# twmitchel/FieldConv

Measured on AMD Instinct MI355X. Metric: FieldConv fwd+bwd Medges/s (20k verts, k=32, C=48, M=2), higher is better.
Workload: dtype f32 (complex64 in/out; contractions on f16 MFMA with every operand split into two halves, fp32 accumulate)

## Files before the change

fieldconv_amd/_env.py:

```python
import os

SWITCHES = {
    'FC_MFMA': 'f32: fp32-MFMA contractions throughout; f16: single halves (reduced precision); default: split halves',
    'FC_RING': '0: frequency-major forward kernels for every mesh size; 2: ring-major ones for every size',
    'FC_GROUP_SPLIT': '0: the backward data kernel never runs the two frequency groups of a tile as separate work items; 2 (development): wherever legal',
    'FC_RING_COMPACT': '0: no compact LDS plans (aliased partials, half-size record chunks) for the ring-major forward kernel',
    'FC_RING_HALVES': '0: no half tiles in the last round of the ring-major forward kernel',
    'FC_HALF_TILES': '0: no half tiles in the frequency-major kernels; 2: half tiles in the backward kernels too',
    'FC_BWD_STREAM': '0: the data / filter kernel pair on large meshes too, instead of the H-streaming arrangement (gather + stream + gx kernels)',
    'FC_GATHER_WPG': '16 / 4: the gather kernel of the H-streaming arrangement as one 16-wavefront workgroup per CU / as five 4-wavefront ones, whatever its registers say',
    'FC_FILTER2': '0: the LDS-staged half-precision filter-gradient kernel instead of the register-fed one',
    'FC_SPLIT_FINISH': '1: partial sums and parameter-gradient chain as two launches',
    'FC_EDGE_PARTS_MAX': 'cap (log2) on the number of workgroups that share a tile on small meshes',
    'FC_ECHO_WPV': 'wavefronts per vertex in the ECHO descriptor kernels (1, 2 or 4)',
    'FC_STAMP_KERNEL': 'data | filter | stream: which backward kernel writes in-kernel time stamps (tools/stamps.py); waits: the walk kernels sum '
                       'the cycles of their explicit vector-memory waits instead (tools/wait_cost.py)',
    'FC_DEBUG': 'forward kernels: skip phases (WRONG RESULTS; refused by bench.py)',
    'FC_DEBUG_BWD': 'backward kernels: skip phases (bit 0 walk, bit 1 gxt product, bit 2 gW product, bit 3 H stores) (WRONG RESULTS; refused by bench.py)',
    'FC_LIN_DIRECT': '0: TangentLin on small meshes through the LDS-staged kernel instead of the direct one',
    'FC_DEBUG_RG': "ECHOBlock head's grouped GEMM: 1 no products, 2 no loads, 4 no staging (WRONG RESULTS; refused by bench.py)",
    'FC_DEBUG_RP': 'finishing launch: 1 no partial loads, 2 no parameter-gradient chain (WRONG RESULTS; refused by bench.py)',
    'FIELDCONV_DEV': '1: load libfieldconv_hip_dev.so (the library switches above exist there only; one of them set without this raises)',
    'FIELDCONV_HIP_LIB': 'path of a prebuilt libfieldconv_hip.so (development variants, fieldconv_amd.build.build_variant)',
    'FIELDCONV_DENSE': '1: FCPrecomp stencils through the dense-stencil kernels',
    'FIELDCONV_NO_GEO': '1: 64-byte factored records in the forward pass instead of geometric ones',
    'FIELDCONV_TORCH_GRAPH': '1: support graph built with torch ops instead of fc_graph_build',
    'FIELDCONV_NO_EDGE_SPLIT': '1: no edge split on small meshes',
    'FIELDCONV_EAGER_STENCIL': '1: FCPrecomp returns the dense (E,R,F) tensor',
    'FIELDCONV_NO_FUSED_EPILOGUE': '1: residual add and modReLU as separate operators',
    'FIELDCONV_SEPARATE_CALLS': '1: one foreign call per kernel instead of fc_forward_params / fc_backward_all',
    'FIELDCONV_CPP_NODES': '0: the block-level autograd nodes in Python (fieldconv_amd/blocks.py) instead of the C++ ones (fc_torch_nodes.so)',
    'FIELDCONV_ECHO_TAIL': "0: ECHOBlock's dense tail as torch's own Linear / ReLU autograd nodes instead of one node; aten: one node composed "
                           "of ATen GEMMs instead of the native head (fc_echo_head_*)",
    'FIELDCONV_BLOCK_CALLS': '0: FCResNetBlock / ECHOBlock / LiftBlock composed of per-operator autograd nodes instead of the block-level entry points',
    'BENCH_BACKEND': 'gloo: several ranks share a device (test rigs); default nccl (= RCCL)',
    'BENCH_FORCE_DIST': '1: run the partitioned / data-parallel code path with one rank',
    'BENCH_FORWARD_OVERLAP': '1: interior targets under the forward halo exchange',
    'BENCH_NO_OVERLAP': '1: gradient halo exchange not overlapped with the filter-gradient kernel',
    'BENCH_GRAPH_STEP': '1: the partitioned step captured in one HIP graph',
}

TEST_SWITCHES = {
    'FC_FULL_MODES': '1: tests/test_gpu_modes.py sweeps every development switch instead of the eight kernel-family / arithmetic modes',
    'FC_FUZZ_SHAPES': 'number of shapes in the seeded sweep against the oracle (default 40)',
    'FC_FUZZ_SEED': 'seed of that sweep',
    'FC_FUZZ_WIDE': '1: the sweep also draws layers wider than 64 channels and (n_rings, band_limit) pairs outside the compiled set',
    'FC_DIST_TEST_DEVICE': 'cuda: the distributed test worker runs the HIP kernels (two gloo ranks on one GPU)',
    'FC_DIST_OVERLAP': '0: the distributed test worker without forward / backward overlap',
    'FC_DIST_PLAN_ONLY': '1: the distributed test worker checks partition and halo plan at config-4 size only',
    'FC_DIST_CONFIG4': '1: the distributed GPU test worker runs config 4\'s per-rank size (20 000 owned vertices per rank)',
}

LIBRARY_SWITCHES = ('FC_BWD_STREAM', 'FC_GATHER_WPG', 'FC_RING', 'FC_GROUP_SPLIT', 'FC_RING_COMPACT', 'FC_RING_HALVES', 'FC_HALF_TILES', 'FC_FILTER2', 'FC_SPLIT_FINISH',
                    'FC_EDGE_PARTS_MAX', 'FC_ECHO_WPV', 'FC_STAMP_KERNEL', 'FC_DEBUG', 'FC_DEBUG_BWD', 'FC_DEBUG_RP', 'FC_DEBUG_RG', 'FC_LIN_DIRECT')

PREFIXES = ('FC_', 'FIELDCONV_', 'BENCH_')
WRONG_RESULTS = ('FC_DEBUG', 'FC_DEBUG_BWD', 'FC_DEBUG_RP', 'FC_DEBUG_RG')


def active(environ=None):
    environ = os.environ if environ is None else environ
    return {k: environ[k] for k in sorted(SWITCHES) if k in environ}


def unknown(environ=None):
    environ = os.environ if environ is None else environ
    return sorted(k for k in environ if k.startswith(PREFIXES) and k not in SWITCHES and k not in TEST_SWITCHES)
```

fieldconv_amd/_lib.py:

```python
import ctypes
import os

from .build import DEV_LIB_PATH, LIB_PATH

_c_int32 = ctypes.c_int32
_vp = ctypes.c_void_p
_sz = ctypes.c_size_t


class FcDims(ctypes.Structure):
    _fields_ = [('N', _c_int32), ('E', _c_int32), ('I', _c_int32), ('O', _c_int32), ('R', _c_int32), ('B', _c_int32), ('mode', _c_int32)]

    def __init__(self, N=0, E=0, I=0, O=0, R=0, B=0, mode=None):
        super().__init__(N, E, I, O, R, B, current_mode() if mode is None else mode)


class FcCsr(ctypes.Structure):
    _fields_ = [('rowptr', _vp), ('nbr', _vp), ('runs', _vp)]


class FcFilterParams(ctypes.Structure):
    _fields_ = [('zonal', ctypes.c_void_p), ('spherical', ctypes.c_void_p), ('phase', ctypes.c_void_p), ('ftype', ctypes.c_int32),
                ('g_zonal', ctypes.c_void_p), ('g_spherical', ctypes.c_void_p), ('g_phase', ctypes.c_void_p),
                ('bias_partials', ctypes.c_void_p), ('bias_nparts', ctypes.c_int32), ('g_bias', ctypes.c_void_p)]


class FcEpilogue(ctypes.Structure):
    _fields_ = [('addend', _vp), ('modrelu_bias', _vp), ('activated', _vp)]


class FcMesh(ctypes.Structure):
    _fields_ = [('N', _c_int32), ('E', _c_int32), ('R', _c_int32), ('B', _c_int32), ('kind', _c_int32),
                ('by_target', ctypes.POINTER(FcCsr)), ('by_source', ctypes.POINTER(FcCsr)), ('fwd', _vp), ('bwd', _vp), ('mode', _c_int32)]

    def __init__(self, N=0, E=0, R=0, B=0, kind=0, by_target=None, by_source=None, fwd=None, bwd=None, mode=None):
        super().__init__(N, E, R, B, kind, by_target, by_source, fwd, bwd, current_mode() if mode is None else mode)


class FcResnetBlockParams(ctypes.Structure):
    _fields_ = [('C_in', _c_int32), ('C_mid', _c_int32), ('C_out', _c_int32), ('conv1', FcFilterParams), ('conv2', FcFilterParams),
                ('bias1', _vp), ('bias2', _vp), ('res_re', _vp), ('res_im', _vp),
                ('g_bias1', _vp), ('g_bias2', _vp), ('g_res_re', _vp), ('g_res_im', _vp)]


class FcEchoBlockParams(ctypes.Structure):
    _fields_ = [('C_in', _c_int32), ('n_des', _c_int32), ('n_bins', _c_int32), ('conv', FcFilterParams), ('bias', _vp), ('g_bias', _vp)]


class FcEchoHeadParams(ctypes.Structure):
    _fields_ = [('D', _c_int32), ('H1', _c_int32), ('H2', _c_int32), ('C_in', _c_int32), ('C_out', _c_int32)] + \
               [(n, _vp) for n in ('w1', 'b1', 'w2', 'b2', 'w3', 'b3', 'wr', 'br', 'g_w1', 'g_b1', 'g_w2', 'g_b2', 'g_w3', 'g_b3', 'g_wr', 'g_br')]


class FcLiftBlockParams(ctypes.Structure):
    _fields_ = [('C_in', _c_int32), ('C_out', _c_int32), ('ftype', _c_int32), ('zonal_ang', _vp), ('zonal_mag', _vp), ('phase', _vp),
                ('bias', _vp), ('g_zonal_ang', _vp), ('g_zonal_mag', _vp), ('g_phase', _vp), ('g_bias', _vp)]


_DP = ctypes.POINTER(FcDims)
_MP = ctypes.POINTER(FcMesh)
_RBP = ctypes.POINTER(FcResnetBlockParams)
_EBP = ctypes.POINTER(FcEchoBlockParams)
_EHP = ctypes.POINTER(FcEchoHeadParams)
_LBP = ctypes.POINTER(FcLiftBlockParams)
_CP = ctypes.POINTER(FcCsr)
_EP = ctypes.POINTER(FcEpilogue)
_FP = ctypes.POINTER(FcFilterParams)

SIGNATURES = {
    'fc_abi_version': (ctypes.c_int, []),
    'fc_dev_switches': (ctypes.c_int, []),
    'fc_debug_stamp_buffer': (None, [_vp]),
    'fc_status_string': (ctypes.c_char_p, [ctypes.c_int]),
    'fc_supported': (ctypes.c_int, [_DP]),
    'fc_describe_kernels': (ctypes.c_int, [_DP, _c_int32, ctypes.c_char_p, ctypes.c_size_t]),
    'fc_shape_compiled': (ctypes.c_int, [_c_int32, _c_int32]),
    'fc_generic_gather': (ctypes.c_int, [_vp, _vp, _CP, _vp, _c_int32, _c_int32, _c_int32, _c_int32, _c_int32, _vp]),
    'fc_wide_workspace_bytes': (ctypes.c_size_t, [_DP, _c_int32, _c_int32, _c_int32]),
    'fc_forward_wide': (ctypes.c_int, [_vp, _vp, _CP, _c_int32, _vp, _vp, _vp, _vp, ctypes.c_size_t, _DP, _c_int32, _c_int32, _vp]),
    'fc_backward_wide': (ctypes.c_int, [_vp, _vp, _vp, _CP, _c_int32, _vp, _vp, _vp, _vp, _vp, ctypes.c_size_t, _DP, _c_int32, _vp]),
    'fc_cgemm_workspace_bytes': (ctypes.c_size_t, [_c_int32, _c_int32, _c_int32, _c_int32]),
    'fc_cgemm': (ctypes.c_int, [_vp, _vp, _vp, _c_int32, _c_int32, _c_int32, ctypes.c_int64, ctypes.c_int64, ctypes.c_int64, ctypes.c_int64,
                                _c_int32, ctypes.c_double, _c_int32, _vp, ctypes.c_size_t, _vp]),
    'fc_tangent_nonlin_forward_f64': (ctypes.c_int, [_vp, _vp, _vp, _c_int32, _c_int32, _vp]),
    'fc_tangent_nonlin_backward_workspace_bytes_f64': (ctypes.c_size_t, [_c_int32, _c_int32]),
    'fc_tangent_nonlin_backward_f64': (ctypes.c_int, [_vp, _vp, _vp, _vp, _vp, _vp, ctypes.c_size_t, _c_int32, _c_int32, _vp]),
    'fc_generic_scatter': (ctypes.c_int, [_vp, _vp, _vp, _CP, _vp, _c_int32, _c_int32, _c_int32, _c_int32, _c_int32, _vp]),
    'fc_packed_filter_floats_fwd': (_sz, [_DP, _c_int32]),
    'fc_packed_filter_floats_bwd': (_sz, [_DP, _c_int32]),
    'fc_pack_filter': (ctypes.c_int, [_vp, _vp, _vp, _DP, _c_int32, _vp]),
    'fc_pack_filter_params': (ctypes.c_int, [_vp, _vp, _vp, _c_int32, _vp, _vp, _DP, _c_int32, _vp]),
    'fc_filter_param_grads': (ctypes.c_int, [_vp, _vp, _vp, _vp, _c_int32, _vp, _vp, _vp, _DP, _vp]),
    'fc_forward': (ctypes.c_int, [_vp, _vp, _CP, _vp, _vp, _DP, _EP, _vp]),
    'fc_factored_record_floats': (ctypes.c_int, [_c_int32]),
    'fc_forward_workspace_bytes': (_sz, [_DP]),
    'fc_forward_factored': (ctypes.c_int, [_vp, _vp, _CP, _vp, _vp, _vp, _sz, _DP, _EP, _vp]),
    'fc_geometric_record_floats': (ctypes.c_int, []),
    'fc_forward_geometric': (ctypes.c_int, [_vp, _vp, _CP, _vp, _vp, _vp, _sz, _DP, _EP, _vp]),
    'fc_records_flags': (_c_int32, [_DP, _c_int32]),
    'fc_backward_workspace_bytes': (_sz, [_DP, _c_int32]),
    'fc_backward_data': (ctypes.c_int, [_vp, _vp, _vp, _CP, _vp, _vp, _vp, _sz, _DP, _vp]),
    'fc_backward_data_factored': (ctypes.c_int, [_vp, _vp, _vp, _CP, _vp, _vp, _vp, _sz, _DP, _c_int32, _vp]),
    'fc_backward_filter': (ctypes.c_int, [_vp, _vp, _sz, _DP, _c_int32, _vp]),
    'fc_backward_streams': (_c_int32, [_DP, _c_int32]),
    'fc_backward_gather': (ctypes.c_int, [_vp, _vp, _CP, _vp, _vp, _sz, _DP, _vp]),
    'fc_backward_stream': (ctypes.c_int, [_vp, _vp, _vp, _vp, _sz, _DP, _vp]),
    'fc_backward_finish': (ctypes.c_int, [_vp, _vp, _sz, _DP, _c_int32, _vp]),
    'fc_backward_finish_params': (ctypes.c_int, [_vp, _vp, _sz, _DP, _c_int32, _FP, _vp]),
    'fc_backward_all': (ctypes.c_int, [_vp, _vp, _vp, _CP, _c_int32, _vp, _vp, _vp, _FP, _vp, _sz, _DP, _vp]),
    'fc_forward_params': (ctypes.c_int, [_vp, _vp, _CP, _c_int32, _FP, _vp, _vp, _vp, _vp, _sz, _DP, _c_int32, _EP, _vp]),
    'fc_echo_hist_dim': (ctypes.c_int, [_c_int32]),
    'fc_echo_channel_block': (ctypes.c_int, [_c_int32]),
    'fc_echo_forward': (ctypes.c_int, [_vp, _vp, _vp, _CP, _vp, _vp, _c_int32, _c_int32, _c_int32, _c_int32, _vp]),
    'fc_echo_backward': (ctypes.c_int, [_vp, _vp, _vp, _CP, _vp, _vp, _vp, _vp, _c_int32, _c_int32, _c_int32, _c_int32, _vp]),
    'fc_adam_step': (ctypes.c_int, [_vp, _vp, _vp, _vp, _vp, _sz] + [ctypes.c_float] * 5 + [_vp]),
    'fc_precomp_workspace_bytes': (_sz, [_c_int32, _c_int32]),
    'fc_precomp_mark': (ctypes.c_int, [_vp, _vp, ctypes.c_float, _c_int32, _c_int32, _vp, _sz, _vp]),
    'fc_precomp_graph': (ctypes.c_int, [_vp] * 5 + [ctypes.c_float] + [_c_int32] * 7 + [_vp] * 16 + [_vp, _sz, _vp, _sz, _vp]),
    'fc_precomp_kept_count_ptr': (_vp, [_vp, _c_int32]),
    'fc_precomp_build': (ctypes.c_int, [_vp, _vp, _vp, _vp, _vp, ctypes.c_float, _c_int32, _c_int32, _c_int32, _c_int32, _vp, _vp, _vp, _vp, _vp, _sz, _vp]),
    'fc_graph_workspace_bytes': (_sz, [_c_int32, _c_int32, _c_int32, _c_int32, _c_int32]),
    'fc_graph_build': (ctypes.c_int, [_vp, _vp, _c_int32, _c_int32, _c_int32, _c_int32] + [_vp] * 12 + [_vp, _sz, _vp]),
    'fc_trans_field_forward': (ctypes.c_int, [_vp, _vp, _CP, _vp, _vp, _vp, _vp, _vp, _vp, _vp, _vp, _c_int32, _c_int32, _c_int32, _c_int32, _c_int32, _c_int32, _vp]),
    'fc_trans_field_backward_workspace_bytes': (_sz, [_c_int32, _c_int32, _c_int32, _c_int32]),
    'fc_trans_field_backward': (ctypes.c_int, [_vp, _CP, _vp, _vp, _vp, _vp, _vp, _vp, _vp, _vp, _vp, _vp, _vp, _vp, _vp, _sz, _c_int32, _c_int32, _c_int32, _c_int32, _c_int32, _c_int32, _c_int32, _vp]),
    'fc_tangent_lin_forward': (ctypes.c_int, [_vp, _vp, _vp, _vp, _c_int32, _c_int32, _c_int32, _vp]),
    'fc_tangent_lin_backward_workspace_bytes': (_sz, [_c_int32, _c_int32, _c_int32]),
    'fc_tangent_lin_backward': (ctypes.c_int, [_vp, _vp, _vp, _vp, _vp, _vp, _vp, _vp, _sz, _c_int32, _c_int32, _c_int32, _vp]),
    'fc_soft_abs_forward': (ctypes.c_int, [_vp, _vp, _sz, _vp]),
    'fc_soft_abs_backward': (ctypes.c_int, [_vp, _vp, _vp, _sz, _vp]),
    'fc_tangent_nonlin_forward': (ctypes.c_int, [_vp, _vp, _vp, _c_int32, _c_int32, _vp]),
    'fc_tangent_nonlin_backward_workspace_bytes': (_sz, [_c_int32, _c_int32]),
    'fc_tangent_nonlin_backward': (ctypes.c_int, [_vp, _vp, _vp, _vp, _vp, _vp, _sz, _c_int32, _c_int32, _vp]),
    'fc_tangent_nonlin_backward_groups': (_c_int32, [_c_int32]),
    'fc_tangent_nonlin_backward_partial': (ctypes.c_int, [_vp, _vp, _vp, _vp, _vp, _sz, _c_int32, _c_int32, _vp]),
    'fc_trans_field_forward_generic': (ctypes.c_int, [_vp, _vp, _CP, _vp, _vp, _vp, _vp, _vp, _vp, _vp, _vp] + [_c_int32] * 7 + [_vp]),
    'fc_trans_field_backward_generic_workspace_bytes': (_sz, [_c_int32] * 5),
    'fc_trans_field_backward_generic': (ctypes.c_int, [_vp, _CP, _vp] + [_vp] * 11 + [_vp, _sz] + [_c_int32] * 8 + [_vp]),
    'fc_echo_hist_dim_generic': (ctypes.c_int, [_c_int32]),
    'fc_echo_generic_workspace_bytes': (_sz, [_c_int32]),
    'fc_echo_forward_generic': (ctypes.c_int, [_vp, _vp, _vp, _CP, _vp, _vp, _vp, _sz] + [_c_int32] * 5 + [_vp]),
    'fc_echo_backward_generic': (ctypes.c_int, [_vp, _vp, _vp, _CP, _vp, _vp, _vp, _vp, _vp, _sz] + [_c_int32] * 5 + [_vp]),
    'fc_resnet_block_saved_bytes': (_sz, [_MP, _RBP]),
    'fc_resnet_block_workspace_bytes': (_sz, [_MP, _RBP, _c_int32]),
    'fc_resnet_block_forward': (ctypes.c_int, [_vp, _MP, _RBP, _vp, _vp, _sz, _vp, _sz, _vp]),
    'fc_resnet_block_backward': (ctypes.c_int, [_vp, _vp, _MP, _RBP, _vp, _sz, _vp, _vp, _sz, _vp]),
    'fc_echo_block_saved_bytes': (_sz, [_MP, _EBP]),
    'fc_echo_block_workspace_bytes': (_sz, [_MP, _EBP, _c_int32]),
    'fc_echo_block_forward': (ctypes.c_int, [_vp, _MP, _vp, _vp, _EBP, _vp, _vp, _sz, _vp, _sz, _vp]),
    'fc_echo_block_backward': (ctypes.c_int, [_vp, _vp, _MP, _vp, _vp, _EBP, _vp, _sz, _vp, _vp, _sz, _vp]),
    'fc_echo_head_forward_workspace_bytes': (_sz, [_c_int32, _EHP]),
    'fc_echo_head_forward': (ctypes.c_int, [_vp, _vp, _EHP, _vp, _vp, _vp, _vp, _sz, _c_int32, _vp]),
    'fc_echo_head_backward_workspace_bytes': (_sz, [_c_int32, _EHP]),
    'fc_echo_head_backward': (ctypes.c_int, [_vp, _vp, _vp, _vp, _vp, _EHP, _vp, _vp, _vp, _vp, _sz, _c_int32, _vp]),
    'fc_lift_block_saved_bytes': (_sz, [_MP, _LBP]),
    'fc_lift_block_workspace_bytes': (_sz, [_MP, _LBP, _c_int32]),
    'fc_lift_block_forward': (ctypes.c_int, [_vp, _vp, _c_int32, _MP, _vp, _LBP, _vp, _vp, _sz, _vp]),
    'fc_lift_block_backward': (ctypes.c_int, [_vp, _vp, _c_int32, _MP, _vp, _LBP, _vp, _sz, _vp, _vp, _sz, _vp]),
    'fc_fps_workspace_bytes': (_sz, [_c_int32]),
    'fc_fps': (ctypes.c_int, [_vp, _c_int32, _c_int32, _c_int32, _vp, _vp, _sz, _vp]),
    'fc_radius_workspace_bytes': (_sz, [_c_int32]),
    'fc_radius_count': (ctypes.c_int, [_vp, _c_int32, ctypes.c_float, _c_int32, _vp, _sz, _vp]),
    'fc_radius_edge_count_ptr': (_vp, [_vp, _c_int32]),
    'fc_radius_fill': (ctypes.c_int, [_vp, _c_int32, ctypes.c_float, _c_int32, ctypes.c_int64, _vp, _vp, _sz, _vp]),
    'fc_pair_sqdist': (ctypes.c_int, [_vp, _c_int32, _vp, _c_int32, _c_int32, _c_int32, _vp, ctypes.c_int64, _vp, _vp]),
    'fc_twin_loss_workspace_bytes': (_sz, [ctypes.c_int64, ctypes.c_int64]),
    'fc_twin_loss_forward': (ctypes.c_int, [_vp, _c_int32, _vp, _c_int32, _c_int32, _c_int32, _vp, ctypes.c_int64, _vp, ctypes.c_int64, _vp,
                                            ctypes.c_double, _vp, _vp, _vp, _sz, _vp]),
    'fc_twin_loss_backward': (ctypes.c_int, [_vp, _c_int32, _vp, _c_int32, _c_int32, _c_int32, _vp, ctypes.c_int64, _vp, ctypes.c_int64, _vp,
                                             ctypes.c_double] + [_vp] * 8 + [_vp]),
    'fc_twin_count_dense': (ctypes.c_int, [_vp, _c_int32, _vp, _c_int32, _c_int32, _c_int32, ctypes.POINTER(ctypes.c_double), _c_int32, _vp, _vp]),
    'fc_label_smoothing_workspace_bytes': (_sz, [ctypes.c_int64, _c_int32]),
    'fc_label_smoothing_forward': (ctypes.c_int, [_vp, _vp, _vp, ctypes.c_int64, _c_int32, _c_int32, ctypes.c_double, ctypes.c_double, _vp, _vp,
                                                  _sz, _vp]),
    'fc_label_smoothing_backward': (ctypes.c_int, [_vp, _vp, _vp, _vp, ctypes.c_int64, _c_int32, _c_int32, ctypes.c_double, ctypes.c_double,
                                                   _vp, _vp]),
    'fc_fps_batched_workspace_bytes': (_sz, [_c_int32]),
    'fc_fps_batched': (ctypes.c_int, [_vp, _vp, _c_int32, _c_int32, _vp, _vp, _vp, ctypes.c_int64, _vp, _vp, _sz, _vp]),
    'fc_radius_count_batched': (ctypes.c_int, [_vp, _vp, _c_int32, _c_int32, ctypes.c_float, _c_int32, _vp, _sz, _vp]),
    'fc_radius_fill_batched': (ctypes.c_int, [_vp, _vp, _c_int32, _c_int32, ctypes.c_float, _c_int32, ctypes.c_int64, _vp, _vp, _sz, _vp]),
    'fc_segment_pool_workspace_bytes': (_sz, [_c_int32] * 4),
    'fc_segment_pool_soft_abs_forward': (ctypes.c_int, [_vp, _vp] + [_c_int32] * 5 + [_vp, _vp, _sz, _vp]),
    'fc_segment_pool_soft_abs_backward': (ctypes.c_int, [_vp, _vp, _vp] + [_c_int32] * 5 + [_vp, _vp]),
    'fc_segment_pool_forward': (ctypes.c_int, [_vp, _vp] + [_c_int32] * 5 + [_vp, _vp, _sz, _vp]),
    'fc_segment_pool_backward': (ctypes.c_int, [_vp, _vp] + [_c_int32] * 5 + [_vp, _vp]),
    'fc_match_workspace_bytes': (_sz, [_c_int32] * 3),
    'fc_match_topk': (ctypes.c_int, [_vp, _c_int32, _vp, _c_int32, _c_int32, _c_int32, _vp, _vp, _c_int32, _vp, _c_int32, _c_int32, _vp, _vp,
                                     _vp, _sz, _vp]),
    'fc_linear_ce_workspace_bytes': (_sz, [_c_int32] * 6),
    'fc_linear_ce_forward': (ctypes.c_int, [_vp, _vp, _vp, _vp, _c_int32, _c_int32, _c_int32, ctypes.c_double, ctypes.c_double, ctypes.c_int64,
                                            _c_int32, _vp, _vp, _vp, _vp, _sz, _vp]),
    'fc_linear_topk': (ctypes.c_int, [_vp, _vp, _vp] + [_c_int32] * 5 + [_vp, _vp, _vp, _sz, _vp]),
    'fc_linear_ce_backward_input': (ctypes.c_int, [_vp] * 6 + [_c_int32] * 3 + [ctypes.c_double, ctypes.c_double, ctypes.c_int64, _vp, _vp]),
    'fc_linear_ce_backward_weight': (ctypes.c_int, [_vp] * 6 + [_c_int32] * 3 + [ctypes.c_double, ctypes.c_double, ctypes.c_int64, _c_int32,
                                                    _vp, _vp, _vp, _sz, _vp]),
    'fc_geodesic_lds_vertices': (_c_int32, []),
    'fc_mesh_edge_lengths': (ctypes.c_int, [_vp, _vp, _vp, _c_int32, _c_int32, _vp, _vp]),
    'fc_geodesic_rows': (ctypes.c_int, [_vp, _vp, _vp, _c_int32, _c_int32, _vp, _c_int32, _vp, _vp, _vp]),
    'fc_geodesic_workspace_bytes': (_sz, [_c_int32, _c_int32]),
    'fc_geodesic_nearest': (ctypes.c_int, [_vp, _vp, _vp, _c_int32, _c_int32, _vp, _vp, _vp, _c_int32, _c_int32, _c_int32, _vp, _vp, _vp, _vp,
                                           _sz, _vp]),
    'fc_face_areas': (ctypes.c_int, [_vp, _vp, _c_int32, _c_int32, _vp, _vp]),
    'fc_segment_sum_f32': (ctypes.c_int, [_vp, _vp, ctypes.c_int64, _c_int32, ctypes.c_float, _vp, _vp]),
    'fc_geodesic_fps_lds_vertices': (_c_int32, []),
    'fc_geodesic_fps_workspace_bytes': (_sz, [_c_int32, _c_int32]),
    'fc_geodesic_fps': (ctypes.c_int, [_vp, _vp, _vp, _c_int32, _c_int32, _vp, _c_int32, _c_int32, _vp, _vp, _vp, ctypes.c_int64, _vp, _vp, _vp,
                                       _vp, _sz, _vp]),
    'fc_geodesic_ball_workspace_bytes': (_sz, [_c_int32, _c_int32]),
    'fc_geodesic_ball_count': (ctypes.c_int, [_vp, _vp, _vp, _c_int32, _c_int32, _vp, _vp, _c_int32, _c_int32, _vp, _c_int32, _c_int32, _c_int32,
                                              ctypes.c_float, _c_int32, _vp, _vp, _sz, _vp]),
    'fc_geodesic_ball_fill': (ctypes.c_int, [_vp, _vp, _vp, _c_int32, _c_int32, _vp, _vp, _c_int32, _c_int32, _vp, _c_int32, _c_int32, _c_int32,
                                             ctypes.c_float, _c_int32, _vp, ctypes.c_int64, _vp, _vp, _vp, _sz, _vp]),
    'fc_logmap_ball_lds_vertices': (_c_int32, []),
    'fc_vertex_frames': (ctypes.c_int, [_vp, _vp, _vp, _vp, _c_int32, _c_int32, _vp, _vp, _vp, _vp]),
    'fc_logmap_workspace_bytes': (_sz, [_c_int32, _c_int32, _c_int32]),
    'fc_logmap': (ctypes.c_int, [_vp, _vp, _vp, _c_int32, _c_int32, _vp, _vp, _c_int32, _c_int32, _vp, _vp, _vp, _vp, _vp, _c_int32, _c_int32,
                                 _c_int32, ctypes.c_float, _vp, _vp, ctypes.c_int64, _vp, _vp, _vp, _vp, _vp, _vp, _c_int32, _vp, _sz, _vp]),
    'fc_mesh_diagonals': (ctypes.c_int, [_vp, _vp, _c_int32, _c_int32, _vp, _vp, _c_int32, _vp, _vp, _vp, _vp]),
    'fc_mesh_graph_merge': (ctypes.c_int, [_vp, _vp, _c_int32, _c_int32, _vp, _vp, _vp, _vp, _vp]),
    'fc_transfer': (ctypes.c_int, [_vp] * 5 + [_c_int32] * 7 + [_vp, _vp]),
}

_LIB = None


def keep_mode(fn_cls):
    fwd, bwd = fn_cls.forward, fn_cls.backward

    def forward(ctx, *args):
        ctx.fc_mode = current_mode()
        return fwd(ctx, *args)

    def backward(ctx, *grads):
        with arithmetic(ctx.fc_mode):
            return bwd(ctx, *grads)
    fn_cls.forward, fn_cls.backward = staticmethod(forward), staticmethod(backward)
    return fn_cls


class FieldConvNativeError(RuntimeError):
    pass


MFMA_MODES = {'': 0, 'split': 0, 'f32': 1, 'f16': 2}

import threading as _threading

_MODE = _threading.local()


def current_mode():
    stack = getattr(_MODE, 'stack', None)
    if stack:
        return stack[-1]
    mode = os.environ.get('FC_MFMA', '')
    if mode not in MFMA_MODES:
        raise FieldConvNativeError(f"FC_MFMA={mode!r}: expected one of 'split' (default), 'f32', 'f16'")
    return MFMA_MODES[mode]


class arithmetic:

    def __init__(self, mode):
        if isinstance(mode, int) and mode in MFMA_MODES.values():
            self.mode = mode
            return
        if mode not in MFMA_MODES:
            raise FieldConvNativeError(f"arithmetic({mode!r}): expected one of 'split', 'f32', 'f16'")
        self.mode = MFMA_MODES[mode]

    def __enter__(self):
        if not hasattr(_MODE, 'stack'):
            _MODE.stack = []
        _MODE.stack.append(self.mode)
        return self

    def __exit__(self, *exc):
        _MODE.stack.pop()


def _pick_library():
    explicit = os.environ.get('FIELDCONV_HIP_LIB')
    if explicit:
        return explicit
    from ._env import LIBRARY_SWITCHES
    wanted = sorted(k for k in LIBRARY_SWITCHES if os.environ.get(k, '') != '')
    dev = os.environ.get('FIELDCONV_DEV', '') == '1'
    if wanted and not dev:
        raise FieldConvNativeError(
            f'{", ".join(wanted)} set, but the product library has no environment switches: set FIELDCONV_DEV=1 to load the development '
            f'build ({DEV_LIB_PATH}), or unset the variable(s)')
    if dev:
        if not os.path.exists(DEV_LIB_PATH):
            raise FieldConvNativeError(
                f'FIELDCONV_DEV=1, but the development library {DEV_LIB_PATH} is not built: '
                'build it with `python -m fieldconv_amd.build --dev` (fieldconv_amd.build.build_dev())')
        return DEV_LIB_PATH
    return LIB_PATH


def load(path=None):
    global _LIB
    if _LIB is not None and path is None:
        return _LIB
    path = path or _pick_library()
    if not os.path.exists(path):
        raise FieldConvNativeError(
            f'{path} not found: build it with `python -m fieldconv_amd.build` '
            '(fieldconv_amd has no CPU or eager fallback for the field-convolution path)')
    lib = ctypes.CDLL(path)
    for name, (res, args) in SIGNATURES.items():
        fn = getattr(lib, name)
        fn.restype = res
        fn.argtypes = args
    current_mode()
    _LIB = lib
    return lib


def check(status, what):
    if status != 0:
        msg = load().fc_status_string(int(status)).decode()
        raise FieldConvNativeError(f'{what} failed: {msg} (status {status})')
```

fieldconv_amd/csrc/fc_api.hip:

```cpp
#include <stdio.h>
#include <stdlib.h>
#include "fc_common.hpp"
#include "fc_kernels.hpp"
#include "fc_tile.hpp"

namespace fc {

bool shape_compiled(int R, int B) {
#define FC_CASE(RR, BB) if (R == RR && B == BB) return true;
    FC_FOR_EACH_SHAPE(FC_CASE)
#undef FC_CASE
    return false;
}

static bool dims_valid(const fc_dims* d) {
    return d && d->N > 0 && d->E >= 0 && d->I > 0 && d->O > 0 && d->R > 0 && d->B >= 0 && d->mode >= FC_MFMA_SPLIT_F16 && d->mode <= FC_MFMA_F16;
}

static bool dims_supported(const fc_dims* d) {
    if (!dims_valid(d)) return false;
    if (!shape_compiled(d->R, d->B)) return false;
    if (d->I > kMaxChannels || d->O > kMaxChannels) return false;
    return forward_fits(d) && backward_fits(d);
}

bool rows_fit_32bit(const fc_dims* d) {
    const uint64_t c = (uint64_t)(d->I > d->O ? d->I : d->O);
    return (uint64_t)d->N * c * 8 < (1ull << 32) && d->N < (1 << 24);
}

static unsigned long long* g_stamps = nullptr;
unsigned long long* debug_stamp_buffer() { return g_stamps; }

}

extern "C" {

void fc_debug_stamp_buffer(void* device_buffer) { fc::g_stamps = static_cast<unsigned long long*>(device_buffer); }

int fc_abi_version(void) { return 11; }

int fc_dev_switches(void) { return fc::kDevSwitches ? 1 : 0; }

const char* fc_status_string(int s) {
    switch (s) {
        case FC_OK: return "ok";
        case FC_ERR_BAD_ARGUMENT: return "bad argument (null pointer or inconsistent dims)";
        case FC_ERR_UNSUPPORTED: return "unsupported (n_rings, band_limit, channels) for the compiled kernels";
        case FC_ERR_LAUNCH: return "HIP kernel launch failed";
        case FC_ERR_WORKSPACE: return "workspace missing or too small";
        default: return "unknown status";
    }
}

int fc_supported(const fc_dims* dims) { return fc::dims_supported(dims) ? 1 : 0; }

int fc_describe_kernels(const fc_dims* dims, int32_t kind, char* buffer, size_t buffer_bytes) {
    if (!buffer || buffer_bytes < 2 || kind < 0 || kind > 2 || !fc::dims_valid(dims)) return FC_ERR_BAD_ARGUMENT;
    if (!fc::dims_supported(dims)) return FC_ERR_UNSUPPORTED;
    char fwd[256], bwd[768];
    fc::describe_forward(dims, kind, fwd, sizeof(fwd));
    fc::describe_backward(dims, kind != 0, bwd, sizeof(bwd));
    snprintf(buffer, buffer_bytes, "%s; %s", fwd, bwd);
    return FC_OK;
}

size_t fc_packed_filter_floats_fwd(const fc_dims* d, int32_t records) {
    if (!fc::dims_valid(d)) return 0;
    return fc::packed_filter_floats_fwd(d, records);
}

size_t fc_packed_filter_floats_bwd(const fc_dims* d, int32_t records) {
    if (!fc::dims_valid(d)) return 0;
    return fc::packed_filter_floats_bwd(d, records);
}

int fc_pack_filter(const float* w_eff, float* wpk_fwd, float* wpk_bwd, const fc_dims* dims, int32_t records, void* stream) {
    if (!w_eff || (!wpk_fwd && !wpk_bwd) || !fc::dims_valid(dims)) return FC_ERR_BAD_ARGUMENT;
    return fc::pack_filter_impl(w_eff, wpk_fwd, wpk_bwd, dims, records, static_cast<hipStream_t>(stream));
}

int fc_pack_filter_params(const float* zonal, const float* spherical, const float* phase, int32_t ftype, float* wpk_fwd,
                          float* wpk_bwd, const fc_dims* dims, int32_t records, void* stream) {
    if (!zonal || !spherical || (!wpk_fwd && !wpk_bwd) || !fc::dims_valid(dims)) return FC_ERR_BAD_ARGUMENT;
    if (ftype < 0 || ftype > 2 || (ftype == 1 && !phase)) return FC_ERR_BAD_ARGUMENT;
    return fc::pack_filter_params_impl(zonal, spherical, phase, ftype, wpk_fwd, wpk_bwd, dims, records,
                                       static_cast<hipStream_t>(stream));
}

int fc_filter_param_grads(const float* gw_eff, const float* zonal, const float* spherical, const float* phase, int32_t ftype,
                          float* g_zonal, float* g_spherical, float* g_phase, const fc_dims* dims, void* stream) {
    if (!gw_eff || !zonal || !spherical || !g_zonal || !g_spherical || !fc::dims_valid(dims)) return FC_ERR_BAD_ARGUMENT;
    if (ftype < 0 || ftype > 2 || (ftype == 1 && (!phase || !g_phase))) return FC_ERR_BAD_ARGUMENT;
    return fc::filter_param_grads_impl(gw_eff, zonal, spherical, phase, ftype, g_zonal, g_spherical, g_phase, dims,
                                       static_cast<hipStream_t>(stream));
}

static bool epilogue_valid(const fc_epilogue* e) { return !e || !e->modrelu_bias || e->activated; }

int fc_forward(const float* x, const float* sten, const fc_csr* by_target, const float* wpk_fwd, float* y,
               const fc_dims* dims, const fc_epilogue* epilogue, void* stream) {
    if (!epilogue_valid(epilogue)) return FC_ERR_BAD_ARGUMENT;
    if (!x || !y || !wpk_fwd || !by_target || !by_target->rowptr || !fc::dims_valid(dims)) return FC_ERR_BAD_ARGUMENT;
    if (dims->E > 0 && (!sten || !by_target->nbr)) return FC_ERR_BAD_ARGUMENT;
    if (!fc::dims_supported(dims)) return FC_ERR_UNSUPPORTED;
    return fc::forward_impl(x, sten, by_target, wpk_fwd, y, dims, 0, nullptr, 0, epilogue, static_cast<hipStream_t>(stream));
}

int fc_factored_record_floats(int32_t band_limit) { return band_limit >= 0 ? fc::factored_record_floats(band_limit) : 0; }

size_t fc_forward_workspace_bytes(const fc_dims* dims) {
    if (!fc::dims_valid(dims) || !fc::dims_supported(dims)) return 0;
    return fc::forward_workspace_bytes(dims, 1);
}

int fc_forward_factored(const float* x, const float* rec_t, const fc_csr* by_target, const float* wpk_fwd, float* y,
                        void* workspace, size_t workspace_bytes, const fc_dims* dims, const fc_epilogue* epilogue, void* stream) {
    if (!epilogue_valid(epilogue)) return FC_ERR_BAD_ARGUMENT;
    if (!x || !y || !wpk_fwd || !by_target || !by_target->rowptr || !fc::dims_valid(dims)) return FC_ERR_BAD_ARGUMENT;
    if (dims->E > 0 && (!rec_t || !by_target->runs)) return FC_ERR_BAD_ARGUMENT;
    if (!fc::dims_supported(dims) || dims->R > 8 || !fc::rows_fit_32bit(dims)) return FC_ERR_UNSUPPORTED;
    return fc::forward_impl(x, rec_t, by_target, wpk_fwd, y, dims, 1, workspace, workspace_bytes, epilogue, static_cast<hipStream_t>(stream));
}

int fc_geometric_record_floats(void) { return fc::kGeoRecordFloats; }

int fc_forward_geometric(const float* x, const float* geo_t, const fc_csr* by_target, const float* wpk_fwd, float* y,
                         void* workspace, size_t workspace_bytes, const fc_dims* dims, const fc_epilogue* epilogue, void* stream) {
    if (!epilogue_valid(epilogue)) return FC_ERR_BAD_ARGUMENT;
    if (!x || !y || !wpk_fwd || !by_target || !by_target->rowptr || !fc::dims_valid(dims)) return FC_ERR_BAD_ARGUMENT;
    if (dims->E > 0 && (!geo_t || !by_target->runs)) return FC_ERR_BAD_ARGUMENT;
    if (!fc::dims_supported(dims) || dims->R > 8 || !fc::rows_fit_32bit(dims)) return FC_ERR_UNSUPPORTED;
    return fc::forward_impl(x, geo_t, by_target, wpk_fwd, y, dims, 2, workspace, workspace_bytes, epilogue, static_cast<hipStream_t>(stream));
}

int32_t fc_records_flags(const fc_dims* dims, int32_t record_driven) {
    if (!record_driven) return 0;
    (void)dims;
    return 1;
}

size_t fc_backward_workspace_bytes(const fc_dims* dims, int32_t records) {
    if (!fc::dims_supported(dims)) return 0;
    (void)records;
    return fc::backward_workspace_bytes(dims);
}

static int check_bwd(const float* x, const float* gy, const float* sten, const fc_csr* by_source, const float* wpk_bwd,
                     float* gx, const fc_dims* dims) {
    if (!x || !gy || !gx || !wpk_bwd || !by_source || !by_source->rowptr || !fc::dims_valid(dims)) return FC_ERR_BAD_ARGUMENT;
    if (dims->E > 0 && !sten) return FC_ERR_BAD_ARGUMENT;
    if (!fc::dims_supported(dims)) return FC_ERR_UNSUPPORTED;
    return FC_OK;
}

int fc_backward_data(const float* x, const float* gy, const float* sten_s, const fc_csr* by_source, const float* wpk_bwd,
                     float* gx, void* workspace, size_t workspace_bytes, const fc_dims* dims, void* stream) {
    const int rc = check_bwd(x, gy, sten_s, by_source, wpk_bwd, gx, dims);
    if (rc != FC_OK) return rc;
    if (dims->E > 0 && !by_source->nbr) return FC_ERR_BAD_ARGUMENT;
    return fc::backward_data_impl(x, gy, sten_s, by_source, wpk_bwd, gx, workspace, workspace_bytes, dims, false,
                                  static_cast<hipStream_t>(stream));
}

int fc_backward_data_factored(const float* x, const float* gy, const float* rec_s, const fc_csr* by_source,
                              const float* wpk_bwd, float* gx, void* workspace, size_t workspace_bytes,
                              const fc_dims* dims, int32_t records, void* stream) {
    const int rc = check_bwd(x, gy, rec_s, by_source, wpk_bwd, gx, dims);
    if (rc != FC_OK) return rc;
    if (dims->E > 0 && !by_source->runs) return FC_ERR_BAD_ARGUMENT;
    if (dims->R > 8 || !fc::rows_fit_32bit(dims)) return FC_ERR_UNSUPPORTED;
    (void)records;
    return fc::backward_data_impl(x, gy, rec_s, by_source, wpk_bwd, gx, workspace, workspace_bytes, dims, true,
                                  static_cast<hipStream_t>(stream));
}

int fc_backward_filter(const float* x, void* workspace, size_t workspace_bytes, const fc_dims* dims, int32_t records, void* stream) {
    if (!x || !fc::dims_valid(dims)) return FC_ERR_BAD_ARGUMENT;
    if (!fc::dims_supported(dims)) return FC_ERR_UNSUPPORTED;
    return fc::backward_filter_impl(x, workspace, workspace_bytes, dims, static_cast<hipStream_t>(stream), records != 0);
}

int32_t fc_backward_streams(const fc_dims* dims, int32_t records) {
    return (fc::dims_supported(dims) && dims->R <= 8 && fc::rows_fit_32bit(dims) && fc::backward_streams(dims, records != 0)) ? 1 : 0;
}

int fc_backward_gather(const float* gy, const float* rec_s, const fc_csr* by_source, const float* wpk_bwd, void* workspace,
                       size_t workspace_bytes, const fc_dims* dims, void* stream) {
    if (!gy || !by_source || !by_source->rowptr || !wpk_bwd || !fc::dims_valid(dims)) return FC_ERR_BAD_ARGUMENT;
    if (dims->E > 0 && (!rec_s || !by_source->runs)) return FC_ERR_BAD_ARGUMENT;
    if (!fc_backward_streams(dims, 1)) return FC_ERR_UNSUPPORTED;
    return fc::backward_stream_impl(nullptr, gy, rec_s, by_source, wpk_bwd, nullptr, workspace, workspace_bytes, dims,
                                    static_cast<hipStream_t>(stream), 1);
}

int fc_backward_stream(const float* x, const float* wpk_bwd, float* gx, void* workspace, size_t workspace_bytes, const fc_dims* dims,
                       void* stream) {
    if (!x || !wpk_bwd || !gx || !fc::dims_valid(dims)) return FC_ERR_BAD_ARGUMENT;
    if (!fc_backward_streams(dims, 1)) return FC_ERR_UNSUPPORTED;
    return fc::backward_stream_impl(x, nullptr, nullptr, nullptr, wpk_bwd, gx, workspace, workspace_bytes, dims,
                                    static_cast<hipStream_t>(stream), 2);
}

int fc_backward_finish(float* gw_eff, void* workspace, size_t workspace_bytes, const fc_dims* dims, int32_t records, void* stream) {
    if (!gw_eff || !fc::dims_valid(dims)) return FC_ERR_BAD_ARGUMENT;
    if (!fc::dims_supported(dims)) return FC_ERR_UNSUPPORTED;
    return fc::backward_finish_impl(gw_eff, workspace, workspace_bytes, dims, static_cast<hipStream_t>(stream), records != 0);
}

static int check_finish_params(const fc_filter_params* params, const fc_dims* dims) {
    if (!params || !fc::dims_valid(dims)) return FC_ERR_BAD_ARGUMENT;
    if (!fc::dims_supported(dims)) return FC_ERR_UNSUPPORTED;
    if (params->ftype < 0 || params->ftype > 2 || !params->zonal || !params->spherical || !params->g_zonal || !params->g_spherical ||
        (params->ftype == 1 && (!params->phase || !params->g_phase)))
        return FC_ERR_BAD_ARGUMENT;
    if (params->bias_partials && (params->bias_nparts <= 0 || !params->g_bias)) return FC_ERR_BAD_ARGUMENT;
    return FC_OK;
}

int fc_backward_finish_params(float* gw_eff, void* workspace, size_t workspace_bytes, const fc_dims* dims, int32_t records,
                              const fc_filter_params* params, void* stream) {
    {
        const int rc = check_finish_params(params, dims);
        if (rc != FC_OK) return rc;
    }
    static const bool split_finish = [] { const char* e = fc::dev_env("FC_SPLIT_FINISH"); return e && atoi(e) != 0; }();
    if (split_finish) {
        if (!gw_eff) return FC_ERR_BAD_ARGUMENT;
        int rc = fc_backward_finish(gw_eff, workspace, workspace_bytes, dims, records, stream);
        if (rc != FC_OK) return rc;
        rc = fc_filter_param_grads(gw_eff, params->zonal, params->spherical, params->phase, params->ftype, params->g_zonal,
                                   params->g_spherical, params->g_phase, dims, stream);
        if (rc != FC_OK || !params->bias_partials) return rc;
        return fc::bias_partials_reduce_impl(params->bias_partials, params->bias_nparts, dims->O, params->g_bias, static_cast<hipStream_t>(stream));
    }
    return fc::backward_finish_params_impl(gw_eff, workspace, workspace_bytes, dims, params, static_cast<hipStream_t>(stream), 0, 0, 0, nullptr,
                                           records != 0);
}

int fc_backward_all(const float* x, const float* gy, const float* sten_or_rec_s, const fc_csr* by_source, int32_t records,
                    const float* wpk_bwd, float* gx, float* gw_eff, const fc_filter_params* params, void* workspace,
                    size_t workspace_bytes, const fc_dims* dims, void* stream) {
    if (!gw_eff && !params) return FC_ERR_BAD_ARGUMENT;
    static const bool split_finish = [] { const char* e = fc::dev_env("FC_SPLIT_FINISH"); return e && atoi(e) != 0; }();
    const bool defer = params != nullptr && !split_finish;
    int rc = check_bwd(x, gy, sten_or_rec_s, by_source, wpk_bwd, gx, dims);
    if (rc != FC_OK) return rc;
    if (params) {
        rc = check_finish_params(params, dims);
        if (rc != FC_OK) return rc;
    }
    if (records) {
        if (dims->E > 0 && !by_source->runs) return FC_ERR_BAD_ARGUMENT;
        if (dims->R > 8 || !fc::rows_fit_32bit(dims)) return FC_ERR_UNSUPPORTED;
    } else if (dims->E > 0 && !by_source->nbr) return FC_ERR_BAD_ARGUMENT;
    rc = fc::backward_data_impl(x, gy, sten_or_rec_s, by_source, wpk_bwd, gx, workspace, workspace_bytes, dims, records != 0,
                                static_cast<hipStream_t>(stream), defer);
    if (rc != FC_OK) return rc;
    rc = fc_backward_filter(x, workspace, workspace_bytes, dims, records, stream);
    if (rc != FC_OK) return rc;
    if (!params) return fc_backward_finish(gw_eff, workspace, workspace_bytes, dims, records, stream);
    if (!defer) return fc_backward_finish_params(gw_eff, workspace, workspace_bytes, dims, records, params, stream);
    return fc::backward_finish_params_impl(gw_eff, workspace, workspace_bytes, dims, params, static_cast<hipStream_t>(stream), 0, 0, 0, gx,
                                           records != 0, x);
}

int fc_forward_params(const float* x, const float* sten_or_records, const fc_csr* by_target, int32_t kind,
                      const fc_filter_params* params, float* wpk_fwd, float* wpk_bwd, float* y, void* workspace,
                      size_t workspace_bytes, const fc_dims* dims, int32_t records, const fc_epilogue* epilogue, void* stream) {
    if (!params || kind < 0 || kind > 2 || ((kind != 0) != ((records & 1) != 0))) return FC_ERR_BAD_ARGUMENT;
    const int rc = fc_pack_filter_params(params->zonal, params->spherical, params->phase, params->ftype, wpk_fwd, wpk_bwd, dims,
                                         records, stream);
    if (rc != FC_OK) return rc;
    if (kind == 2) return fc_forward_geometric(x, sten_or_records, by_target, wpk_fwd, y, workspace, workspace_bytes, dims, epilogue, stream);
    if (kind == 1) return fc_forward_factored(x, sten_or_records, by_target, wpk_fwd, y, workspace, workspace_bytes, dims, epilogue, stream);
    return fc_forward(x, sten_or_records, by_target, wpk_fwd, y, dims, epilogue, stream);
}

}
```

fieldconv_amd/csrc/fc_common.hpp:

```cpp
#pragma once
#include <hip/hip_runtime.h>
#include <stdint.h>
#include <stdlib.h>
#include <type_traits>

namespace fc {

#ifdef FC_DEV_SWITCHES
inline const char* dev_env(const char* name) { return getenv(name); }
constexpr bool kDevSwitches = true;
#else
inline const char* dev_env(const char*) { return nullptr; }
constexpr bool kDevSwitches = false;
#endif

constexpr int kWave = 64;
constexpr int kTile = 16;
constexpr int kWaves = 16;
constexpr int kThreads = kWave * kWaves;
constexpr float kOriginEps = 1e-7f;

typedef float f32x4 __attribute__((ext_vector_type(4)));
typedef float f32x2 __attribute__((ext_vector_type(2)));

__device__ __forceinline__ f32x4 mfma16(float a, float b, f32x4 c) {
    return __builtin_amdgcn_mfma_f32_16x16x4f32(a, b, c, 0, 0, 0);
}

__host__ __device__ constexpr int round_up(int v, int m) { return (v + m - 1) / m * m; }

__device__ __forceinline__ int first_tile_of_block() {
    const int b = blockIdx.x, g = gridDim.x;
    return (g & 7) ? b : (b & 7) * (g >> 3) + (b >> 3);
}

__device__ __forceinline__ float wave_max_nonneg(float v) {
    int x = __float_as_int(v);
    x = max(x, __builtin_amdgcn_update_dpp(0, x, 0x111, 0xF, 0xF, true));
    x = max(x, __builtin_amdgcn_update_dpp(0, x, 0x112, 0xF, 0xF, true));
    x = max(x, __builtin_amdgcn_update_dpp(0, x, 0x114, 0xF, 0xF, true));
    x = max(x, __builtin_amdgcn_update_dpp(0, x, 0x118, 0xF, 0xF, true));
    x = max(x, __builtin_amdgcn_update_dpp(0, x, 0x142, 0xF, 0xF, true));
    x = max(x, __builtin_amdgcn_update_dpp(0, x, 0x143, 0xF, 0xF, true));
    return __int_as_float(__builtin_amdgcn_readlane(x, 63));
}

__device__ __forceinline__ float2 gather_row(const float2* __restrict__ base, int vertex, uint32_t row_bytes, uint32_t lane_bytes) {
    uint32_t off;
    asm("v_mad_u32_u24 %0, %1, %2, %3" : "=v"(off) : "v"(vertex), "s"(row_bytes), "v"(lane_bytes));
    return *reinterpret_cast<const float2*>(reinterpret_cast<const char*>(base) + off);
}

template <int BEGIN, int END, class Fn>
__device__ __forceinline__ void static_for(Fn&& fn) {
    if constexpr (BEGIN < END) {
        fn(std::integral_constant<int, BEGIN>{});
        static_for<BEGIN + 1, END>(fn);
    }
}

__host__ __device__ constexpr int factored_record_floats(int B) { return round_up(4 + 2 * (2 * B + 1), 4); }

typedef __attribute__((address_space(1))) const void* gptr_t;
typedef __attribute__((address_space(3))) void* lptr_t;

__device__ __forceinline__ void lds_dma16_untracked(const void* src_lane, const void* lds_dst_uniform) {
    const uint32_t dst = __builtin_amdgcn_readfirstlane((uint32_t)(uintptr_t)lds_dst_uniform);
    asm volatile("s_mov_b32 m0, %0\n\ts_nop 0\n\tglobal_load_lds_dwordx4 %1, off" : : "s"(dst), "v"(src_lane) : "memory", "m0");
}

__device__ __forceinline__ void lds_dma16_untracked_lanes(const void* src_lane, const void* lds_dst_uniform, unsigned long long mask) {
    const uint32_t dst = __builtin_amdgcn_readfirstlane((uint32_t)(uintptr_t)lds_dst_uniform);
    asm volatile("s_mov_b64 exec, %2\n\ts_mov_b32 m0, %0\n\ts_nop 0\n\tglobal_load_lds_dwordx4 %1, off\n\ts_mov_b64 exec, -1"
                 : : "s"(dst), "v"(src_lane), "s"(mask) : "memory", "m0");
}

__device__ __forceinline__ void lds_dma16_saddr(const void* src_uniform, uint32_t lane_off, const void* lds_dst_uniform) {
    const uint32_t dst = __builtin_amdgcn_readfirstlane((uint32_t)(uintptr_t)lds_dst_uniform);
    const uint64_t base = (uint64_t)(uintptr_t)src_uniform;
    const uint32_t lo = __builtin_amdgcn_readfirstlane((uint32_t)base), hi = __builtin_amdgcn_readfirstlane((uint32_t)(base >> 32));
    const uint64_t sb = ((uint64_t)hi << 32) | lo;
    asm volatile("s_mov_b32 m0, %0\n\ts_nop 0\n\tglobal_load_lds_dwordx4 %1, %2" : : "s"(dst), "v"(lane_off), "s"(sb) : "memory", "m0");
}
__device__ __forceinline__ void lds_dma16_saddr_lanes(const void* src_uniform, uint32_t lane_off, const void* lds_dst_uniform,
                                                      unsigned long long mask) {
    const uint32_t dst = __builtin_amdgcn_readfirstlane((uint32_t)(uintptr_t)lds_dst_uniform);
    const uint64_t base = (uint64_t)(uintptr_t)src_uniform;
    const uint32_t lo = __builtin_amdgcn_readfirstlane((uint32_t)base), hi = __builtin_amdgcn_readfirstlane((uint32_t)(base >> 32));
    const uint64_t sb = ((uint64_t)hi << 32) | lo;
    asm volatile("s_mov_b64 exec, %3\n\ts_mov_b32 m0, %0\n\ts_nop 0\n\tglobal_load_lds_dwordx4 %1, %2\n\ts_mov_b64 exec, -1"
                 : : "s"(dst), "v"(lane_off), "s"(sb), "s"(mask) : "memory", "m0");
}
__device__ __forceinline__ void lds_dma4_saddr(const void* src_uniform, uint32_t lane_off, const void* lds_dst_uniform) {
    const uint32_t dst = __builtin_amdgcn_readfirstlane((uint32_t)(uintptr_t)lds_dst_uniform);
    const uint64_t base = (uint64_t)(uintptr_t)src_uniform;
    const uint32_t lo = __builtin_amdgcn_readfirstlane((uint32_t)base), hi = __builtin_amdgcn_readfirstlane((uint32_t)(base >> 32));
    const uint64_t sb = ((uint64_t)hi << 32) | lo;
    asm volatile("s_mov_b32 m0, %0\n\ts_nop 0\n\tglobal_load_lds_dword %1, %2" : : "s"(dst), "v"(lane_off), "s"(sb) : "memory", "m0");
}

__host__ __device__ constexpr int factored_log_chunk_records(int B) {
    const int per_kib = 256 / factored_record_floats(B);
    return per_kib >= 32 ? 5 : per_kib >= 16 ? 4 : per_kib >= 8 ? 3 : per_kib >= 4 ? 2 : 1;
}
constexpr int kRunStride = 8;
constexpr int kRingChunks = 4;



__host__ __device__ constexpr int slab_stride(int KP) { return KP + 8; }

__device__ __forceinline__ bool is_origin(float2 z) {
    return (fabsf(z.x) < kOriginEps) && (fabsf(z.y) < kOriginEps);
}

__device__ __forceinline__ float2 unit_conj(float2 z) {
    const bool org = is_origin(z);
    const float n2 = z.x * z.x + z.y * z.y;
    const float inv = org ? 0.f : __frsqrt_rn(n2);
    return org ? make_float2(1.f, 0.f) : make_float2(z.x * inv, -z.y * inv);
}

__device__ __forceinline__ float2 cmul(float2 a, float2 b) {
    return make_float2(a.x * b.x - a.y * b.y, a.x * b.y + a.y * b.x);
}
__device__ __forceinline__ float2 cmul_conj(float2 a, float2 b) {
    return make_float2(a.x * b.x + a.y * b.y, a.y * b.x - a.x * b.y);
}

__device__ __forceinline__ f32x2 cmul_pk_step1(f32x2 a, f32x2 b) { return f32x2{a.x, a.x} * b; }
__device__ __forceinline__ f32x2 cmul_pk_step2(f32x2 a, f32x2 b, f32x2 t) {
    f32x2 z;
    asm("v_pk_fma_f32 %0, %1, %2, %3 op_sel:[1,1,0] op_sel_hi:[1,0,1] neg_lo:[1,0,0]" : "=v"(z) : "v"(a), "v"(b), "v"(t));
    return z;
}
__device__ __forceinline__ f32x2 cmul_pk(f32x2 a, f32x2 b) {
    return cmul_pk_step2(a, b, cmul_pk_step1(a, b));
}
__device__ __forceinline__ f32x2 cmul_conj_pk_step1(f32x2 a, f32x2 b) { return f32x2{b.x, b.x} * a; }
__device__ __forceinline__ f32x2 cmul_conj_pk_step2(f32x2 a, f32x2 b, f32x2 t) {
    f32x2 z;
    asm("v_pk_fma_f32 %0, %1, %2, %3 op_sel:[1,1,0] op_sel_hi:[1,0,1] neg_hi:[1,0,0]" : "=v"(z) : "v"(b), "v"(a), "v"(t));
    return z;
}
__device__ __forceinline__ f32x2 cmul_conj_pk(f32x2 a, f32x2 b) {
    return cmul_conj_pk_step2(a, b, cmul_conj_pk_step1(a, b));
}

template <int B>
__device__ __forceinline__ void rotate_all(f32x2 z, f32x2 (&xt)[2 * B + 1]) {
    const bool org = (fabsf(z.x) < kOriginEps) && (fabsf(z.y) < kOriginEps);
    const f32x2 sq = z * z;
    const float n2 = sq.x + sq.y;
    const float inv = __frsqrt_rn(n2);
    const f32x2 u = org ? f32x2{1.f, 0.f} : f32x2{z.x * inv, -z.y * inv};
    xt[B] = z;
    if (B >= 1) {
        xt[B + 1] = org ? z : f32x2{n2 * inv, 0.f};
        xt[B - 1] = cmul_conj_pk(z, u);
    }
#pragma unroll
    for (int m = 2; m <= B; ++m) {
        xt[B + m] = cmul_pk(xt[B + m - 1], u);
        xt[B - m] = cmul_conj_pk(xt[B - m + 1], u);
    }
}

template <int B>
__device__ __forceinline__ void rotate_geometric(f32x2 x, f32x2 c, f32x2 g, f32x2 (&z)[2 * B + 1]) {
    const bool org = (fabsf(x.x) < kOriginEps) && (fabsf(x.y) < kOriginEps);
    const f32x2 sq = x * x;
    const float inv = __frsqrt_rn(sq.x + sq.y);
    const f32x2 u = org ? f32x2{1.f, 0.f} : f32x2{x.x * inv, -x.y * inv};
    const f32x2 v = cmul_pk(g, u);
    z[B] = cmul_pk(c, x);
    if (B >= 1) {
        z[B + 1] = cmul_pk(z[B], v);
        z[B - 1] = cmul_conj_pk(z[B], v);
    }
#pragma unroll
    for (int m = 2; m <= B; ++m) {
        z[B + m] = cmul_pk(z[B + m - 1], v);
        z[B - m] = cmul_conj_pk(z[B - m + 1], v);
    }
}
constexpr int kGeoRecordFloats = 8;
constexpr int kGeoLogChunkRecords = 5;

__device__ __forceinline__ void cmac_sx(f32x2& acc, f32x2 s, f32x2 x, f32x2 xs) {
    acc = __builtin_elementwise_fma(f32x2{s.x, s.x}, x, acc);
    acc = __builtin_elementwise_fma(f32x2{s.y, s.y}, xs, acc);
}
__device__ __forceinline__ void cmac_gconjs(f32x2& acc, f32x2 s, f32x2 g, f32x2 gs) {
    acc = __builtin_elementwise_fma(f32x2{s.x, s.x}, g, acc);
    acc = __builtin_elementwise_fma(f32x2{s.y, s.y}, gs, acc);
}

__device__ __forceinline__ float2 unit_power(float2 u, int m) {
    float2 p = make_float2(1.f, 0.f);
    const int am = m < 0 ? -m : m;
    for (int k = 0; k < am; ++k) p = (m > 0) ? cmul(p, u) : cmul_conj(p, u);
    return p;
}

template <int B>
__device__ __forceinline__ float2 gx_from_slices(const float2 x, const float2* __restrict__ gxt, const size_t idx, const size_t stride,
                                                 const int ks = 1) {
    constexpr int F = 2 * B + 1;
    float2 z[F];
#pragma unroll
    for (int f = 0; f < F; ++f) {
        z[f] = gxt[(size_t)(f * ks) * stride + idx];
        if (ks == 2) {
            const float2 z2 = gxt[(size_t)(f * ks + 1) * stride + idx];
            z[f].x += z2.x;
            z[f].y += z2.y;
        }
    }
    const float2 u1 = unit_conj(x);
    float2 up[B + 1];
    up[0] = make_float2(1.f, 0.f);
#pragma unroll
    for (int q = 1; q <= B; ++q) up[q] = cmul(up[q - 1], u1);
    const float inv2 = is_origin(x) ? 0.f : 1.f / (x.x * x.x + x.y * x.y);
    float2 acc = make_float2(0.f, 0.f);
    float eq = 0.f;
#pragma unroll
    for (int f = 0; f < F; ++f) {
        const int mm = f - B;
        float2 c = up[mm < 0 ? -mm : mm];
        if (mm < 0) c.y = -c.y;
        const float2 xtv = cmul(x, c);
        const float2 out = cmul_conj(z[f], c);
        acc.x += out.x;
        acc.y += out.y;
        eq += (float)mm * (z[f].x * xtv.y - z[f].y * xtv.x);
    }
    acc.x += (-x.y * inv2) * eq;
    acc.y += (x.x * inv2) * eq;
    return acc;
}

struct Stamper {
    unsigned long long* p;
    int n;
    __device__ __forceinline__ void operator()(int label) {
        if (p) {
            if (n < 256 && (threadIdx.x & 63) == 0)
                p[n] = ((unsigned long long)label << 56) | (__builtin_amdgcn_s_memtime() & 0x00ffffffffffffffull);
            ++n;
        }
    }
    __device__ __forceinline__ void realtime(int label) {
        if (p) {
            if (n < 256 && (threadIdx.x & 63) == 0)
                p[n] = ((unsigned long long)label << 56) | (__builtin_amdgcn_s_memrealtime() & 0x00ffffffffffffffull);
            ++n;
        }
    }
};

struct WaitMeter {
    static constexpr int kKinds = 8;
    unsigned long long* p;
    unsigned long long t0, start, cyc[kKinds];
    unsigned n[kKinds];
    __device__ __forceinline__ void open(unsigned long long* q) {
        p = nullptr;
        if constexpr (kDevSwitches) {
            p = q;
            if (p) {
                start = __builtin_amdgcn_s_memtime();
#pragma unroll
                for (int k = 0; k < kKinds; ++k) { cyc[k] = 0; n[k] = 0; }
            }
        }
    }
    __device__ __forceinline__ void begin() {
        if constexpr (kDevSwitches)
            if (p) t0 = __builtin_amdgcn_s_memtime();
    }
    __device__ __forceinline__ void end(const int kind) {
        if constexpr (kDevSwitches)
            if (p) {
                cyc[kind] += __builtin_amdgcn_s_memtime() - t0;
                ++n[kind];
            }
    }
    __device__ __forceinline__ void close() {
        if constexpr (kDevSwitches)
            if (p && (threadIdx.x & 63) == 0) {
#pragma unroll
                for (int k = 0; k < kKinds; ++k) {
                    atomicAdd(p + k, cyc[k]);
                    atomicAdd(p + kKinds + k, (unsigned long long)n[k]);
                }
                atomicAdd(p + 16, __builtin_amdgcn_s_memtime() - start);
                atomicAdd(p + 17, 1ull);
            }
    }
};
constexpr int kMeterForward = 0, kMeterGather = 32;

}
```

fieldconv_amd/csrc/fc_forward.hip:

```cpp
#include "fc_forward_kernels.hpp"

namespace fc {

template int forward_impl_mode<false>(const float*, const float*, const fc_csr*, const float*, float*, const fc_dims*, int,
                                      void*, size_t, const fc_epilogue*, hipStream_t);
extern template int forward_impl_mode<true>(const float*, const float*, const fc_csr*, const float*, float*, const fc_dims*,
                                            int, void*, size_t, const fc_epilogue*, hipStream_t);

int forward_impl(const float* x, const float* sten, const fc_csr* g, const float* wpk, float* y, const fc_dims* d,
                 int kind, void* ws, size_t ws_bytes, const fc_epilogue* epi, hipStream_t stream) {
    if (kind != 0 && forward_ring_fits(d)) return forward_ring_impl(x, sten, g, wpk, y, d, kind, ws, ws_bytes, epi, stream);
    return halves_of(d) ? forward_impl_mode<true>(x, sten, g, wpk, y, d, kind, ws, ws_bytes, epi, stream)
                        : forward_impl_mode<false>(x, sten, g, wpk, y, d, kind, ws, ws_bytes, epi, stream);
}

size_t forward_workspace_bytes(const fc_dims* d, int kind) { return forward_workspace_bytes_impl(d, kind); }

bool forward_fits(const fc_dims* d) {
    const MmaGeom g = make_mma_geom(d->O, d->R, d->I, halves_of(d));
    return forward_lds_floats(g, 1) * sizeof(float) + (size_t)kWaves * kRingChunks * 1024 <= kMaxLds;
}

}
```

fieldconv_amd/csrc/fc_forward_ring.hip:

```cpp
#include <stdio.h>
#include "fc_forward_ring.hpp"
#include "fc_forward_kernels.hpp"

namespace fc {

bool ring_enabled(const fc_dims* d) {
    static const bool on = [] { const char* e = dev_env("FC_RING"); return !(e && atoi(e) == 0); }();
    return on && halves_of(d) == 2;
}

bool forward_ring_fits(const fc_dims* d) {
    static const bool force = [] { const char* e = dev_env("FC_RING"); return e && atoi(e) == 2; }();
    if (!ring_enabled(d) || !plan_ring(d->O, 2 * d->B + 1, d->I, halves_of(d)).ok) return false;
    return force || (d->N + kTile - 1) / kTile > num_cus();
}

void describe_forward(const fc_dims* d, int kind, char* buf, size_t n) {
    const char* mode = halves_of(d) == 2 ? "split-f16" : halves_of(d) == 1 ? "f16" : "f32";
    const char* rec = kind == 2 ? "geometric records" : kind == 1 ? "factored records" : "dense rows";
    if (kind != 0 && forward_ring_fits(d)) {
        const RingPlan p = plan_ring(d->O, 2 * d->B + 1, d->I, halves_of(d));
        snprintf(buf, n, "fc_forward_ring_kernel<%s,%s> (ring-major, 2 workgroups x 8 wavefronts per CU, %zu B LDS, %d %s record chunks%s)",
                 rec, mode, p.lds, p.nr, p.logh ? "half-size" : "1 KiB", p.alias ? ", partials aliased onto the slab" : "");
    } else {
        snprintf(buf, n, "%s<%s,%s> (frequency-major, 16 wavefronts per CU, parts=%d)", kind ? "fc_forward_factored_kernel" : "fc_forward_kernel",
                 rec, mode, 1 << forward_parts_log2(d, kind));
    }
}

size_t packed_ring_image_floats(int M, int F, int channels, int R, int halves) {
    const MmaGeom g = ring_geom(M, F, channels, halves);
    return (size_t)g.MP + (size_t)R * halves * g.MP * g.KP;
}

template <int R, int B, bool GEO, int LOGH>
static int launch_forward_ring(const float2* x, const float* rec, const fc_csr* g, const float* wpk, float2* y, const RingArgs& a,
                               size_t lds, int grid, hipStream_t stream) {
    auto kern = fc_forward_ring_kernel<R, B, GEO, LOGH>;
    static bool lds_ok[kMaxDevices] = {};
    if (!allow_full_lds(reinterpret_cast<const void*>(kern), lds, lds_ok)) return FC_ERR_LAUNCH;
    hipLaunchKernelGGL(kern, dim3(grid), dim3(kDuoThreads), lds, stream, x, rec, g->rowptr, g->runs, wpk, y, a);
    return hipGetLastError() == hipSuccess ? FC_OK : FC_ERR_LAUNCH;
}

int forward_ring_impl(const float* x, const float* rec, const fc_csr* g, const float* wpk, float* y, const fc_dims* d, int kind,
                      void* ws, size_t ws_bytes, const fc_epilogue* epi, hipStream_t stream) {
    const int F = 2 * d->B + 1;
    const RingPlan p = plan_ring(d->O, F, d->I, halves_of(d));
    if (!p.ok) return FC_ERR_UNSUPPORTED;
    RingArgs a;
    a.N = d->N; a.I = d->I; a.O = d->O;
    a.g = p.g;
    a.ntiles = (d->N + kTile - 1) / kTile;
    a.parts_log2 = (ws && ws_bytes >= forward_workspace_bytes_impl(d, kind)) ? forward_parts_log2(d, kind) : 0;
    a.part_stride = (uint32_t)forward_part_stride(d);
    a.epi = make_epi(epi);
    a.nr = p.nr;
    a.alias_part = p.alias;
    a.wpk_bytes = (uint32_t)(packed_ring_image_floats(d->O, F, d->I, d->R, p.g.split) * sizeof(float));
    a.slab_bytes_w = (uint32_t)(2 * p.g.split * p.g.MP * p.g.KP * 2);
    static const int dbg = [] { const char* e = dev_env("FC_DEBUG"); return e ? atoi(e) : 0; }();
    a.dbg = dbg;
    static const bool meter = [] { const char* e = dev_env("FC_STAMP_KERNEL"); return e && e[0] == 'w'; }();
    a.stamps = meter ? nullptr : debug_stamp_buffer();
    a.meter = meter && debug_stamp_buffer() ? debug_stamp_buffer() + kMeterForward : nullptr;
    const int nvt = a.ntiles << a.parts_log2;
    int grid = nvt < 2 * num_cus() ? nvt : 2 * num_cus();
    const int rem = nvt % grid;
    a.nv_full = nvt;
    a.nv_total = nvt;
    a.spread_cus = 0;
    static const bool halves = !(dev_env("FC_RING_HALVES") && atoi(dev_env("FC_RING_HALVES")) == 0);
    if (halves && a.parts_log2 == 0 && rem > 0 && 2 * rem <= grid) {
        a.nv_full = nvt - rem;
        a.nv_total = a.nv_full + 2 * rem;
    }
    const int cus = num_cus();
    if (halves && a.parts_log2 == 0 && nvt > cus && nvt < 2 * cus) {
        a.nv_full = 2 * nvt - 2 * cus;
        a.nv_total = 2 * cus;
        a.spread_cus = cus;
        grid = 2 * cus;
    }
    int rc = FC_ERR_UNSUPPORTED;
    const float2* x2 = reinterpret_cast<const float2*>(x);
    float2* y2 = reinterpret_cast<float2*>(a.parts_log2 ? static_cast<float*>(ws) : y);
#define FC_CASE(RR, BB)                                                                                            \
    if (d->R == RR && d->B == BB) {                                                                                \
        if constexpr (BB >= 2) {                                                                                   \
            if (p.logh)                                                                                            \
                rc = kind == 2 ? launch_forward_ring<RR, BB, true, 1>(x2, rec, g, wpk, y2, a, p.lds, grid, stream)  \
                               : launch_forward_ring<RR, BB, false, 1>(x2, rec, g, wpk, y2, a, p.lds, grid, stream); \
        }                                                                                                          \
        if (!p.logh)                                                                                               \
            rc = kind == 2 ? launch_forward_ring<RR, BB, true, 0>(x2, rec, g, wpk, y2, a, p.lds, grid, stream)      \
                           : launch_forward_ring<RR, BB, false, 0>(x2, rec, g, wpk, y2, a, p.lds, grid, stream);    \
    }
    FC_FOR_EACH_SHAPE(FC_CASE)
#undef FC_CASE
    if (rc != FC_OK || a.parts_log2 == 0) return rc;
    return sum_parts_epilogue(static_cast<const float*>(ws), y, (size_t)d->N * d->O, a.part_stride, 1 << a.parts_log2, d->O, a.epi, stream);
}

}
```

fieldconv_amd/csrc/fc_forward_ring.hpp:

```cpp
#pragma once
#include <stdlib.h>
#include "fc_common.hpp"
#include "fc_kernels.hpp"
#include "fc_tile.hpp"

namespace fc {

constexpr int kDuoWaves = 8;
constexpr int kDuoThreads = kDuoWaves * kWave;
constexpr size_t kDuoMaxLds = 80 * 1024;

struct RingArgs {
    int N, I, O;
    MmaGeom g;
    int ntiles;
    int parts_log2;
    uint32_t part_stride;
    int nr;
    int alias_part;
    int nv_full;
    int nv_total;
    int spread_cus;
    uint32_t wpk_bytes;
    uint32_t slab_bytes_w;
    int dbg;
    FwdEpi epi;
    unsigned long long* stamps;
    unsigned long long* meter;
};

__host__ __device__ inline MmaGeom ring_geom(int M, int F, int channels, int halves) {
    MmaGeom g = make_mma_geom(M, F, channels, halves);
    g.NKP = kDuoWaves / g.NMT;
    if (g.NKP > g.KST) g.NKP = g.KST;
    if (g.NKP < 1) g.NKP = 1;
    return g;
}

__device__ __forceinline__ int ring_item(const RingArgs& a) {
    if (a.spread_cus == 0) return first_tile_of_block();
    const int b = blockIdx.x, C = a.spread_cus, W = a.nv_full;
    if (b >= C) return a.nv_full + (C - W) + (b - C);
    const int w0 = (b * W) / C, w1 = ((b + 1) * W) / C;
    return w1 > w0 ? w0 : a.nv_full + (b - w0);
}

struct RingLds {
    float* slab;
    float* part;
    float* vinv;
    int* runs;
    float* ring;
};
__host__ __device__ inline size_t ring_lds_floats(const MmaGeom& g, int nr, int chunk_floats = 256, bool alias = false) {
    const size_t slab = slab_floats(g), part = partial_floats(g.NKP, g.MP);
    return (alias ? (slab > part ? slab : part) : slab + part) + kTile + kDuoWaves * 32 + (size_t)kDuoWaves * 2 * nr * chunk_floats;
}
__device__ __forceinline__ RingLds ring_lds(char* smem, const MmaGeom& g, bool alias) {
    RingLds l;
    l.slab = reinterpret_cast<float*>(smem);
    l.part = alias ? l.slab : l.slab + slab_floats(g);
    const size_t slab = slab_floats(g), part = partial_floats(g.NKP, g.MP);
    l.vinv = l.slab + (alias ? (slab > part ? slab : part) : slab + part);
    l.runs = reinterpret_cast<int*>(l.vinv + kTile);
    l.ring = reinterpret_cast<float*>(l.runs + kDuoWaves * 32);
    return l;
}

template <int R, int B, bool GEO, int LOGH = 0>
__global__ __launch_bounds__(kDuoThreads, 4) void fc_forward_ring_kernel(
    const float2* __restrict__ gx_, const float* __restrict__ grec, const int32_t* __restrict__ growptr,
    const int32_t* __restrict__ gruns, const float* __restrict__ gwpk, float2* __restrict__ gy_, const RingArgs a) {
    constexpr int F = 2 * B + 1;
    constexpr int RECF = GEO ? kGeoRecordFloats : factored_record_floats(B);
    constexpr int LOG_CR = (GEO ? kGeoLogChunkRecords : factored_log_chunk_records(B)) - LOGH;
    constexpr int CR = 1 << LOG_CR;
    constexpr int CHUNK = 256 >> LOGH;
    static_assert(LOG_CR >= 2, "a record chunk holds at least four records");
    extern __shared__ __attribute__((aligned(16))) char smem[];
    const MmaGeom& g = a.g;
    const RingLds l = ring_lds(smem, g, a.alias_part != 0);
    const int tid = threadIdx.x;
    const int lane = tid & 63;
    const int wave = __builtin_amdgcn_readfirstlane(tid >> 6);
    const int nr = a.nr;
    const int I = a.I;
    const int sfl = slab_floats(g);

    for (int idx = tid; idx < sfl; idx += kDuoThreads) l.slab[idx] = 0.f;
    __syncthreads();

    if (wave >= kDuoWaves / 2 && !(a.dbg & 4)) __builtin_amdgcn_s_setprio(1);
    Stamper stamp{(a.stamps && blockIdx.x == 0) ? a.stamps + wave * 256 : nullptr, 0};
    WaitMeter meter;
    meter.open(a.meter);
    const int cl = lane < I ? lane : 0;
    const int mt = wave % g.NMT, kp = wave / g.NMT;
    const bool mma_active = kp < g.NKP;
    const rsrc_t wimg = make_rsrc(gwpk, a.wpk_bytes);
    const int planes0 = g.MP * 4;
    const int pl = a.parts_log2;
    const int nvt = a.ntiles << pl;

    auto ring_of = [&](const int j) { return l.ring + (wave * 2 + j) * nr * CHUNK; };
    auto dma_chunk = [&](const int j, const int first, const int ch) {
        const float* src = grec + ((size_t)first + (size_t)ch * CR) * RECF + lane * 4;
        if constexpr (LOGH == 0) lds_dma16_untracked(src, ring_of(j) + (ch & (nr - 1)) * CHUNK);
        else lds_dma16_untracked_lanes(src, ring_of(j) + (ch & (nr - 1)) * CHUNK, 0xffffffffull);
    };
    auto slot_range = [&](const int vt, const int j, const int par, int& b, int& e) {
        b = 0;
        e = 0;
        int run[R];
#pragma unroll
        for (int q = 0; q < R; ++q) run[q] = 0;
        int t = (vt >> pl) * kTile + wave + kDuoWaves * j;
        bool live = vt < nvt;
        if (vt >= a.nv_full) {
            const int h = vt - a.nv_full;
            t = (a.nv_full + (h >> 1)) * kTile + (h & 1) * kDuoWaves + wave;
            live = vt < a.nv_total && j == 0;
        }
        if (live && t < a.N) {
            const int rb = growptr[t];
            const int n = growptr[t + 1] - rb;
            const int part = vt & ((1 << pl) - 1);
            const int s0 = (n * part) >> pl, s1 = (n * (part + 1)) >> pl;
            b = rb + s0;
            e = rb + s1;
#pragma unroll
            for (int q = 0; q < R; ++q) run[q] = min(max(gruns[(size_t)t * kRunStride + q], s0), s1) - s0;
        }
        if (lane == 0) {
            int* lro = l.runs + (wave * 2 + j) * 16 + par * 8;
#pragma unroll
            for (int q = 0; q < R; ++q) lro[q] = run[q];
        }
    };
    auto rec_ptr = [&](const float* ring, const int s) {
        if constexpr (CR * RECF == CHUNK) return ring + ((s * RECF) & (nr * CHUNK - 1));
        else return ring + ((s >> LOG_CR) & (nr - 1)) * CHUNK + (s & (CR - 1)) * RECF;
    };
    auto first_rows = [&](const int j, const int nslots, float2& r0, float2& r1) {
        r0 = make_float2(0.f, 0.f);
        r1 = r0;
        if (nslots > 0) {
            const float* ring = ring_of(j);
            const int n0 = __float_as_int(ring[3]);
            const int n1 = __float_as_int(ring[min(1, nslots - 1) * RECF + 3]);
            r0 = gather_row(gx_, n0, 8u * I, 8u * cl);
            r1 = gather_row(gx_, n1, 8u * I, 8u * cl);
        }
    };

    int beg[2], end[2], par = 0;
#pragma unroll
    for (int j = 0; j < 2; ++j) {
        slot_range(ring_item(a), j, 0, beg[j], end[j]);
        const int nch = (end[j] - beg[j] + CR - 1) >> LOG_CR;
        for (int ch = 0; ch < min(nch, nr); ++ch) dma_chunk(j, beg[j], ch);
    }
    meter.begin();
    asm volatile("s_waitcnt vmcnt(0)" ::: "memory");
    meter.end(4);
    float2 px[2][2];
#pragma unroll
    for (int j = 0; j < 2; ++j) first_rows(j, end[j] - beg[j], px[j][0], px[j][1]);

    f32x4 tot_re = {0.f, 0.f, 0.f, 0.f}, tot_im = tot_re;

    const int wv = ((mt * 16 + (lane & 15)) * 32 + 8 * (lane >> 4)) * 2;
    const int wplane = g.MP * g.KP * 2;
    const int wkb = g.MP * 64;
    u32x4 wf0[4], wf1[4];
    auto load_w = [&](const int rq, const int kb, u32x4 (&dst)[4]) {
        const int kc = min(kb, g.KST - 1);
        const int base = planes0 + rq * (int)a.slab_bytes_w + wkb * kc;
#pragma unroll
        for (int pnum = 0; pnum < 4; ++pnum) dst[pnum] = buffer_load16(wimg, wv, base + pnum * wplane);
    };
    auto prefetch_w = [&](const int rq) {
        if (mma_active) {
            load_w(rq, kp, wf0);
            load_w(rq, kp + g.NKP, wf1);
        } else {
            const u32x4 zero = {0u, 0u, 0u, 0u};
#pragma unroll
            for (int pnum = 0; pnum < 4; ++pnum) { wf0[pnum] = zero; wf1[pnum] = zero; }
        }
    };
    auto mma_block = [&](const lds_f16* sp, const int kb, const u32x4 (&w)[4], f32x4& are, f32x4& aim) {
        const int fr = lane & 15, fq = lane >> 4;
        const u32x4 sign = {0x80008000u, 0x80008000u, 0x80008000u, 0x80008000u};
        const lds_f16* s0 = sp + fr * g.KS + 32 * fq + 128 * kb;
        {
            const u32x4 srh = *reinterpret_cast<lds_u32x4*>(s0), srl = *reinterpret_cast<lds_u32x4*>(s0 + 8);
            are = mfma32h(w[1], srh, are); aim = mfma32h(w[3], srh, aim);
            are = mfma32h(w[0], srl, are); aim = mfma32h(w[2], srl, aim);
            are = mfma32h(w[0], srh, are); aim = mfma32h(w[2], srh, aim);
        }
        {
            u32x4 sih = *reinterpret_cast<lds_u32x4*>(s0 + 16), sil = *reinterpret_cast<lds_u32x4*>(s0 + 24);
            aim = mfma32h(w[1], sih, aim);
            aim = mfma32h(w[0], sil, aim);
            aim = mfma32h(w[0], sih, aim);
            sih ^= sign;
            sil ^= sign;
            are = mfma32h(w[3], sih, are);
            are = mfma32h(w[2], sil, are);
            are = mfma32h(w[2], sih, are);
        }
    };
    auto contract = [&](const int rq) {
        if (mma_active && !(a.dbg & 2)) {
            f32x4 tre = {0.f, 0.f, 0.f, 0.f}, tim = tre;
            const lds_f16* sp = (const lds_f16*)l.slab;
            for (int kb = kp; kb < g.KST; kb += 2 * g.NKP) {
                mma_block(sp, kb, wf0, tre, tim);
                if (kb + 2 * g.NKP < g.KST) load_w(rq, kb + 2 * g.NKP, wf0);
                if (kb + g.NKP < g.KST) {
                    mma_block(sp, kb + g.NKP, wf1, tre, tim);
                    if (kb + 3 * g.NKP < g.KST) load_w(rq, kb + 3 * g.NKP, wf1);
                }
            }
            const float inv = l.vinv[lane & 15];
            tot_re += tre * inv;
            tot_im += tim * inv;
        }
    };
    auto flush_row = [&](const f32x2 (&c)[F], const int j) {
        const int row_i = wave + kDuoWaves * j;
        float mx = 0.f;
#pragma unroll
        for (int f = 0; f < F; ++f) mx = fmaxf(mx, fmaxf(fabsf(c[f].x), fabsf(c[f].y)));
        mx = wave_max_nonneg(mx);
        float scale, inv;
        split_scale(mx, scale, inv);
        if (lane == 0) l.vinv[row_i] = inv;
        if (lane < g.KI) {
            lds_u32* const row = (lds_u32*)l.slab + row_i * (g.KS / 2);
            int o0 = split_pair_offset(lane, 2);
#pragma unroll
            for (int f = 0; f < F; ++f) {
                f16x2 hi, lo;
                split_halves2(c[f], scale, hi, lo);
                split_pair_store(row, o0, hi, lo, lane, 2);
                o0 += 2 * g.KI;
                asm volatile("" : "+v"(o0));
            }
        }
    };

    stamp.realtime(29);
    stamp(28);
    for (int vt = ring_item(a); vt < a.nv_total; vt += gridDim.x) {
        int nbeg[2], nend[2];
#pragma unroll
        for (int j = 0; j < 2; ++j) slot_range(vt + gridDim.x, j, par ^ 1, nbeg[j], nend[j]);

        f32x2 clo[2][F], chi[2][F];
#pragma unroll
        for (int j = 0; j < 2; ++j)
#pragma unroll
            for (int f = 0; f < F; ++f) { clo[j][f] = f32x2{0.f, 0.f}; chi[j][f] = clo[j][f]; }
        float2 xq[2][2] = {{px[0][0], px[0][1]}, {px[1][0], px[1][1]}};

        constexpr bool kLookaheadProven = CR - 2 >= 3;
        auto gather_run = [&](const int j, int s, const int run_end, f32x2 (&lo)[F], f32x2 (&hi)[F], float2& xe, float2& xo) {
            const float* const ring = ring_of(j);
            const int nslots = end[j] - beg[j];
            const int nch = (nslots + CR - 1) >> LOG_CR;
            auto slot = [&](const int s_, float2& xcur) {
                const float* rp = rec_ptr(ring, s_);
                const f32x4 head = *reinterpret_cast<const f32x4*>(rp);
                const int n2 = __float_as_int(rec_ptr(ring, min(s_ + 2, nslots - 1))[3]);
                const f32x2 w0v = f32x2{head.y, head.y}, w1v = f32x2{head.z, head.z};
                f32x2 z[F];
                if constexpr (GEO) {
                    const f32x4 cg = *reinterpret_cast<const f32x4*>(rp + 4);
                    rotate_geometric<B>(f32x2{xcur.x, xcur.y}, f32x2{cg.x, cg.y}, f32x2{cg.z, cg.w}, z);
                    xcur = gather_row(gx_, n2, 8u * I, 8u * cl);
                } else {
                    f32x2 xt[F], ph[F];
                    rotate_all<B>(f32x2{xcur.x, xcur.y}, xt);
                    xcur = gather_row(gx_, n2, 8u * I, 8u * cl);
#pragma unroll
                    for (int f = 0; f < F; ++f) {
                        ph[f] = *reinterpret_cast<const f32x2*>(rp + 4 + 2 * f);
                        z[f] = cmul_pk_step1(ph[f], xt[f]);
                    }
#pragma unroll
                    for (int f = 0; f < F; ++f) z[f] = cmul_pk_step2(ph[f], xt[f], z[f]);
                }
#pragma unroll
                for (int f = 0; f < F; ++f) lo[f] = __builtin_elementwise_fma(w0v, z[f], lo[f]);
#pragma unroll
                for (int f = 0; f < F; ++f) hi[f] = __builtin_elementwise_fma(w1v, z[f], hi[f]);
            };
            while (s < run_end) {
                const int m = s & (CR - 1);
                if (m == 0 && s > 0) {
                    const int ch = s >> LOG_CR;
                    if (ch - 1 + nr < nch) dma_chunk(j, beg[j], ch - 1 + nr);
                }
                int stop = min(run_end, s - m + CR);
                if constexpr (!kLookaheadProven) {
                    if (nr == 2) {
                        if (m == CR - 2) {
                            meter.begin();
                            asm volatile("s_waitcnt vmcnt(2)" ::: "memory");
                            meter.end(1);
                        }
                        else if (m < CR - 2) stop = min(stop, s - m + CR - 2);
                    }
                }
                if ((s & 1) && s < stop) {
                    slot(s, xo);
                    ++s;
                }
                for (; s + 1 < stop; s += 2) {
                    slot(s, xe);
                    slot(s + 1, xo);
                }
                if (s < stop) {
                    slot(s, xe);
                    ++s;
                }
            }
        };

        stamp(10);
        for (int q = 0; q < R - 1; ++q) {
            if (!(a.dbg & 1)) {
#pragma unroll
                for (int j = 0; j < 2; ++j) {
                    const int* lro = l.runs + (wave * 2 + j) * 16 + par * 8;
                    const int s = __builtin_amdgcn_readfirstlane(lro[q]);
                    const int run_end = (q + 1 < R - 1) ? __builtin_amdgcn_readfirstlane(lro[q + 1]) : end[j] - beg[j];
                    gather_run(j, s, run_end, clo[j], chi[j], xq[j][0], xq[j][1]);
                }
            }
            stamp(0);
            if (q == R - 2) {
                meter.begin();
                meter.end(7);
#pragma unroll
                for (int j = 0; j < 2; ++j) {
                    const int nnch = (nend[j] - nbeg[j] + CR - 1) >> LOG_CR;
                    for (int ch = 0; ch < min(nnch, nr); ++ch) dma_chunk(j, nbeg[j], ch);
                }
            }
            prefetch_w(q);
            flush_row(clo[0], 0);
            if (vt < a.nv_full) flush_row(clo[1], 1);
            stamp(1);
            __syncthreads();
            stamp(2);
            contract(q);
            stamp(3);
            __syncthreads();
            stamp(4);
#pragma unroll
            for (int j = 0; j < 2; ++j)
#pragma unroll
                for (int f = 0; f < F; ++f) { clo[j][f] = chi[j][f]; chi[j][f] = f32x2{0.f, 0.f}; }
        }
        prefetch_w(R - 1);
        flush_row(clo[0], 0);
        if (vt < a.nv_full) flush_row(clo[1], 1);
        __syncthreads();
        if (!mma_active || (a.dbg & 2)) {
            meter.begin();
            asm volatile("s_waitcnt vmcnt(0)" ::: "memory");
            meter.end(3);
        }
#pragma unroll
        for (int j = 0; j < 2; ++j) {
            beg[j] = nbeg[j];
            end[j] = nend[j];
            first_rows(j, end[j] - beg[j], px[j][0], px[j][1]);
        }
        contract(R - 1);
        if (a.alias_part) __syncthreads();
        if (mma_active) store_partial(l.part, g, mt, kp, lane, tot_re, tot_im);
        tot_re = f32x4{0.f, 0.f, 0.f, 0.f};
        tot_im = tot_re;
        stamp(5);
        __syncthreads();
        {
            const bool half = vt >= a.nv_full;
            const int hh = vt - a.nv_full;
            const int row0 = half ? (a.nv_full + (hh >> 1)) * kTile + (hh & 1) * kDuoWaves : (vt >> pl) * kTile;
            const int nrows = half ? kDuoWaves : kTile;
            float2* const yout = gy_ + (size_t)(half ? 0 : (vt & ((1 << pl) - 1))) * a.part_stride;
            for (int idx = tid; idx < nrows * a.O; idx += kDuoThreads) {
                const int v = idx / a.O, o = idx - v * a.O;
                const int n = row0 + v;
                float2 sm = sum_partials(l.part, g, v, o);
                const float k = gwpk[o];
                sm.x *= k;
                sm.y *= k;
                if (n < a.N) {
                    if (pl == 0) sm = apply_epilogue(sm, (size_t)n * a.O + o, o, a.epi);
                    yout[(size_t)n * a.O + o] = sm;
                }
            }
        }
        if (a.alias_part) {
            __syncthreads();
            for (int idx = tid; idx < partial_floats(g.NKP, g.MP); idx += kDuoThreads) l.slab[idx] = 0.f;
            __syncthreads();
        }
        stamp(6);
        par ^= 1;
    }
    stamp(30);
    stamp.realtime(31);
    meter.close();
}

struct RingPlan {
    MmaGeom g;
    int nr;
    int logh;
    int alias;
    size_t lds;
    bool ok;
};
inline RingPlan plan_ring(int M, int F, int channels, int halves) {
    RingPlan p;
    p.g = ring_geom(M, F, channels, halves);
    p.ok = false;
    p.nr = 0; p.lds = 0; p.logh = 0; p.alias = 0;
    if (halves != 2 || p.g.NMT > kDuoWaves) return p;
    static const bool compact = !(dev_env("FC_RING_COMPACT") && atoi(dev_env("FC_RING_COMPACT")) == 0);
    const int tries[4][3] = {{4, 0, 0}, {2, 0, 0}, {2, 0, 1}, {2, 1, 1}};
    for (int t = 0; t < (compact ? 4 : 2); ++t) {
        if (tries[t][1] && F < 5) continue;
        const size_t lds = ring_lds_floats(p.g, tries[t][0], 256 >> tries[t][1], tries[t][2] != 0) * sizeof(float);
        if (lds <= kDuoMaxLds) {
            p.nr = tries[t][0]; p.logh = tries[t][1]; p.alias = tries[t][2]; p.lds = lds; p.ok = true;
            break;
        }
    }
    return p;
}

}
```

fieldconv_amd/csrc/fc_kernels.hpp:

```cpp
#pragma once
#include <hip/hip_runtime.h>
#include "../../include/fieldconv_hip.h"

#define FC_FOR_EACH_SHAPE(X) \
    X(2, 1) X(3, 1) X(4, 1) X(5, 1) X(6, 1) X(7, 1) X(8, 1) \
    X(2, 2) X(3, 2) X(4, 2) X(5, 2) X(6, 2) X(7, 2) X(8, 2) \
    X(2, 3) X(3, 3) X(4, 3) X(5, 3) X(6, 3) X(7, 3) X(8, 3)

namespace fc {

constexpr size_t kMaxLds = 160 * 1024;
constexpr int kDefaultCUs = 256;
constexpr int kMaxDevices = 16;
inline int num_cus() {
    static int cached[kMaxDevices] = {};
    int dev = 0;
    if (hipGetDevice(&dev) != hipSuccess || dev < 0) return kDefaultCUs;
    if (dev < kMaxDevices && cached[dev] > 0) return cached[dev];
    int n = 0;
    if (hipDeviceGetAttribute(&n, hipDeviceAttributeMultiprocessorCount, dev) != hipSuccess || n <= 0) n = kDefaultCUs;
    if (dev < kMaxDevices) cached[dev] = n;
    return n;
}
constexpr int kMaxChannels = 64;

int forward_impl(const float* x, const float* sten, const fc_csr* g, const float* wpk, float* y,
                 const fc_dims* d, int kind, void* ws, size_t ws_bytes, const fc_epilogue* epi, hipStream_t stream);
size_t forward_workspace_bytes(const fc_dims* d, int kind);
size_t backward_workspace_bytes(const fc_dims* d);
int backward_data_impl(const float* x, const float* gy, const float* sten, const fc_csr* g, const float* wpk, float* gx,
                       void* ws, size_t ws_bytes, const fc_dims* d, bool factored, hipStream_t stream, bool defer_gx_sum = false);
int backward_filter_impl(const float* x, void* ws, size_t ws_bytes, const fc_dims* d, hipStream_t stream, bool factored = false);
bool backward_streams(const fc_dims* d, bool factored);
int backward_stream_impl(const float* x, const float* gy, const float* rec, const fc_csr* g, const float* wpk, float* gx, void* ws,
                         size_t ws_bytes, const fc_dims* d, hipStream_t stream, int stages);
int backward_finish_impl(float* gw_eff, void* ws, size_t ws_bytes, const fc_dims* d, hipStream_t stream, bool factored = false);
int pack_filter_impl(const float* w_eff, float* wpk_fwd, float* wpk_bwd, const fc_dims* d, int records, hipStream_t stream);
int pack_filter_params_impl(const float* zonal, const float* sph, const float* phase, int ftype, float* wpk_fwd,
                            float* wpk_bwd, const fc_dims* d, int records, hipStream_t stream);
int pack_filter_params_pair_impl(const fc_filter_params& f0, float* fwd0, float* bwd0, const fc_dims* d0, const fc_filter_params& f1,
                                 float* fwd1, float* bwd1, const fc_dims* d1, int records, hipStream_t stream);
size_t packed_filter_floats_fwd(const fc_dims* d, int records);
size_t packed_filter_floats_bwd(const fc_dims* d, int records);

bool ring_enabled(const fc_dims* d);
bool forward_ring_fits(const fc_dims* d);
size_t packed_ring_image_floats(int M, int F, int channels, int R, int halves);
int forward_ring_impl(const float* x, const float* rec, const fc_csr* g, const float* wpk, float* y, const fc_dims* d, int kind,
                      void* ws, size_t ws_bytes, const fc_epilogue* epi, hipStream_t stream);
int filter_param_grads_impl(const float* gw_eff, const float* zonal, const float* sph, const float* phase, int ftype,
                            float* g_zonal, float* g_sph, float* g_phase, const fc_dims* d, hipStream_t stream);

int reduce_param_grads_impl(const float* gwp, size_t sp, size_t sr, size_t sf, size_t so, bool ring_pairs, int P, float* gw_eff,
                            const float* zonal, const float* sph, const float* phase, int ftype, float* g_zonal, float* g_sph,
                            float* g_phase, const fc_dims* d, hipStream_t stream, int o0 = 0, int i0 = 0, int Ifull = 0,
                            const float* bias_partials = nullptr, int bias_nparts = 0, float* g_bias = nullptr,
                            const float* gx_parts = nullptr, float* gx = nullptr, size_t gx_count = 0, size_t gx_stride = 0, int gx_nparts = 0,
                            const float* gx_x = nullptr);
int bias_partials_reduce_impl(const float* partials, int nparts, int C, float* g_bias, hipStream_t stream);

__host__ __device__ inline int dump_k(int r, int o, int R, int O, bool pairs) {
    return (pairs && (r | 1) < R) ? (r >> 1) * 2 * O + 2 * o + (r & 1) : r * O + o;
}
int backward_finish_params_impl(float* gw_eff, void* ws, size_t ws_bytes, const fc_dims* d, const fc_filter_params* fp, hipStream_t stream,
                                int o0 = 0, int i0 = 0, int Ifull = 0,
                                float* gx_deferred = nullptr, bool factored = false, const float* x_for_gx = nullptr);
int pack_filter_block_impl(const float* w_eff, float* wpk_fwd, float* wpk_bwd, const fc_dims* d, int records, int o0, int i0, int Ifull,
                           hipStream_t stream);
int pack_filter_params_block_impl(const float* zonal, const float* sph, const float* phase, int ftype, float* wpk_fwd, float* wpk_bwd,
                                  const fc_dims* d, int records, int o0, int i0, int Ifull, hipStream_t stream);

bool shape_compiled(int R, int B);
bool rows_fit_32bit(const fc_dims* d);
void describe_forward(const fc_dims* d, int kind, char* buf, size_t n);
void describe_backward(const fc_dims* d, int records, char* buf, size_t n);

int tangent_lin_backward_impl(const float* x, const float* gy, const float* re_w, const float* im_w, float* gx, const float* gx_addend,
                              float* g_re, float* g_im, void* workspace, size_t workspace_bytes, int N, int I, int O, hipStream_t s);

int precomp_area_sums(const int64_t* edges, const int32_t* keep, const float* w, float* total, int N, int E, hipStream_t s);

unsigned long long* debug_stamp_buffer();

inline bool allow_full_lds(const void* fn, size_t lds_bytes, bool (&done)[kMaxDevices]) {
    if (lds_bytes <= 64 * 1024) return true;
    int dev = 0;
    if (hipGetDevice(&dev) != hipSuccess) return false;
    if (dev >= 0 && dev < kMaxDevices && done[dev]) return true;
    if (hipFuncSetAttribute(fn, hipFuncAttributeMaxDynamicSharedMemorySize, (int)kMaxLds) != hipSuccess) return false;
    if (dev >= 0 && dev < kMaxDevices) done[dev] = true;
    return true;
}
bool forward_fits(const fc_dims* d);
bool backward_fits(const fc_dims* d);

}
```

fieldconv_amd/csrc/fc_pack.hip:

```cpp
#include <stdlib.h>
#include "fc_common.hpp"
#include "fc_kernels.hpp"
#include "fc_tile.hpp"
#include "fc_forward_ring.hpp"

namespace fc {

__device__ __forceinline__ float2 filter_entry(const float* __restrict__ zonal, const float* __restrict__ sph,
                                               const float* __restrict__ phase, int ftype, int B, int R, int I, int o, int i,
                                               int r, int f) {
    const size_t oir = ((size_t)o * I + i) * R + r;
    if (ftype == 2) {
        if (f == B) return make_float2(zonal[oir * 2], zonal[oir * 2 + 1]);
        const int b = f < B ? f : f - 1;
        const float* p = sph + (oir * (2 * B) + b) * 2;
        return make_float2(p[0], p[1]);
    }
    const int q = f >= B ? f - B : B - f;
    const float z = zonal[oir];
    float2 sp = make_float2(0.f, 0.f);
    if (B > 0) sp = *reinterpret_cast<const float2*>(sph + (oir * B + (q > 0 ? q - 1 : 0)) * 2);
    float ph = 0.f;
    if (ftype == 1) ph = phase[((size_t)o * I + i) * (B + 1) + q];
    float2 c = q == 0 ? make_float2(z, 0.f) : make_float2(sp.x, f > B ? sp.y : -sp.y);
    if (ftype == 1) {
        float s, co;
        sincosf(ph, &s, &co);
        c = cmul(c, make_float2(co, s));
    }
    return c;
}

struct PackArgs {
    int O, I, R, F, B, ftype;
    MmaGeom gf, gb;
    unsigned blocks_f;
    int ring_f;
    int o0, i0, Ifull;
};

constexpr int kPackThreads = 256;

template <bool FROM_PARAMS, bool WITH_PHASE>
__device__ __forceinline__ float2 packed_value(const float2* __restrict__ w, const float* __restrict__ zonal,
                                               const float* __restrict__ sph, const float* __restrict__ phase,
                                               const PackArgs& a, bool is_bwd, int m, int k, int slab) {
    const int KI = is_bwd ? a.gb.KI : a.gf.KI;
    const bool ring = !is_bwd && a.ring_f;
    const int kk = k / KI, c = k - kk * KI;
    const int r = ring ? slab : kk, f = ring ? kk : slab;
    if (f >= a.F) return make_float2(0.f, 0.f);
    const int o = is_bwd ? c : m, i = is_bwd ? m : c;
    if (o >= a.O || i >= a.I || r >= a.R) return make_float2(0.f, 0.f);
    const float2 v = FROM_PARAMS ? filter_entry(zonal, sph, phase, (!WITH_PHASE && a.ftype == 1) ? 0 : a.ftype, a.B, a.R, a.Ifull, a.o0 + o,
                                                a.i0 + i, r, f)
                                 : w[(((size_t)(a.o0 + o) * a.Ifull + a.i0 + i) * a.R + r) * a.F + f];
    const float sc = 1.f / (float)a.F;
    return make_float2(v.x * sc, (is_bwd ? -v.y : v.y) * sc);
}

template <bool FROM_PARAMS>
__device__ __forceinline__ float row_max2(const float2* __restrict__ w, const float* __restrict__ zonal, const float* __restrict__ sph,
                                          const PackArgs& a, bool is_bwd, int m) {
    const int M = is_bwd ? a.I : a.O, C = is_bwd ? a.O : a.I;
    float mx = 0.f;
    if (m >= M) return mx;
    if (FROM_PARAMS) {
        for (int idx = threadIdx.x; idx < C * a.R; idx += kPackThreads) {
            const int c = idx / a.R, r = idx - c * a.R;
            const int o = is_bwd ? c : m, i = is_bwd ? m : c;
            const size_t oir = ((size_t)(a.o0 + o) * a.Ifull + a.i0 + i) * a.R + r;
            if (a.ftype == 2) {
                mx = fmaxf(mx, zonal[oir * 2] * zonal[oir * 2] + zonal[oir * 2 + 1] * zonal[oir * 2 + 1]);
                for (int b = 0; b < 2 * a.B; ++b) {
                    const float* p = sph + (oir * (2 * a.B) + b) * 2;
                    mx = fmaxf(mx, p[0] * p[0] + p[1] * p[1]);
                }
            } else {
                mx = fmaxf(mx, zonal[oir] * zonal[oir]);
                for (int b = 0; b < a.B; ++b) {
                    const float* p = sph + (oir * a.B + b) * 2;
                    mx = fmaxf(mx, p[0] * p[0] + p[1] * p[1]);
                }
            }
        }
    } else {
        for (int idx = threadIdx.x; idx < C * a.R * a.F; idx += kPackThreads) {
            const int c = idx / (a.R * a.F), rf = idx - c * (a.R * a.F);
            const int o = is_bwd ? c : m, i = is_bwd ? m : c;
            const float2 v = w[((size_t)(a.o0 + o) * a.Ifull + a.i0 + i) * a.R * a.F + rf];
            mx = fmaxf(mx, v.x * v.x + v.y * v.y);
        }
    }
    const float sc = 1.f / (float)a.F;
    return mx * sc * sc;
}

template <bool FROM_PARAMS>
__device__ __forceinline__ void pack_filter_body(const float2* __restrict__ w, const float* __restrict__ zonal, const float* __restrict__ sph,
                                                 const float* __restrict__ phase, float* __restrict__ fwd, float* __restrict__ bwd,
                                                 const PackArgs& a, const unsigned block) {
    const bool is_bwd = block >= a.blocks_f;
    const unsigned blk = is_bwd ? block - a.blocks_f : block;
    const MmaGeom& g = is_bwd ? a.gb : a.gf;
    float* const img = is_bwd ? bwd : fwd;
    if (!g.split) {
        const size_t j = (size_t)blk * kPackThreads + threadIdx.x;
        if (j >= (size_t)a.F * 2 * g.MP * g.KP) return;
        const int k = j % g.KP;
        const int m = (j / g.KP) % g.MP;
        const int pl = (j / ((size_t)g.KP * g.MP)) % 2;
        const int f = j / ((size_t)g.KP * g.MP * 2);
        const float2 v = packed_value<FROM_PARAMS, true>(w, zonal, sph, phase, a, is_bwd, m, k, f);
        img[j] = pl == 0 ? v.x : v.y;
        return;
    }
    __shared__ float red[kPackThreads / kWave];
    const int nslab = (!is_bwd && a.ring_f) ? a.R : a.F;
    const int m = blk / nslab, f = blk - m * nslab;
    float mx = row_max2<FROM_PARAMS>(w, zonal, sph, a, is_bwd, m);
#pragma unroll
    for (int d = 32; d >= 1; d >>= 1) mx = fmaxf(mx, __shfl_xor(mx, d, 64));
    if ((threadIdx.x & 63) == 0) red[threadIdx.x >> 6] = mx;
    __syncthreads();
    mx = sqrtf(fmaxf(fmaxf(red[0], red[1]), fmaxf(red[2], red[3]))) * 1.0000002f;
    float scale, inv;
    split_scale(mx, scale, inv);
    if (threadIdx.x == 0 && f == 0) img[m] = inv;
    _Float16* const planes = reinterpret_cast<_Float16*>(img + g.MP);
    const size_t plane = (size_t)g.MP * g.KP;
    for (int k = threadIdx.x; k < g.KP; k += kPackThreads) {
        const float2 v = packed_value<FROM_PARAMS, true>(w, zonal, sph, phase, a, is_bwd, m, k, f);
        _Float16 rh, rl, ih, il;
        split_halves(v.x * scale, rh, rl);
        split_halves(v.y * scale, ih, il);
        _Float16* p = planes + (size_t)f * 2 * g.split * plane + ((size_t)(k >> 5) * g.MP + m) * 32 + (k & 31);
        if (g.split == 2) {
            p[0] = rh;
            p[plane] = rl;
            p[2 * plane] = ih;
            p[3 * plane] = il;
        } else {
            p[0] = rh;
            p[plane] = ih;
        }
    }
}

template <bool FROM_PARAMS>
__global__ __launch_bounds__(kPackThreads) void fc_pack_filter_kernel(const float2* __restrict__ w, const float* __restrict__ zonal,
                                                                      const float* __restrict__ sph,
                                                                      const float* __restrict__ phase, float* __restrict__ fwd,
                                                                      float* __restrict__ bwd, const PackArgs a) {
    pack_filter_body<FROM_PARAMS>(w, zonal, sph, phase, fwd, bwd, a, blockIdx.x);
}

struct PackPtrs { const float* zonal; const float* sph; const float* phase; float* fwd; float* bwd; };
__global__ __launch_bounds__(kPackThreads) void fc_pack_filter_pair_kernel(const PackPtrs p0, const PackArgs a0, const PackPtrs p1,
                                                                           const PackArgs a1, const unsigned split) {
    if (blockIdx.x < split) pack_filter_body<true>(nullptr, p0.zonal, p0.sph, p0.phase, p0.fwd, p0.bwd, a0, blockIdx.x);
    else pack_filter_body<true>(nullptr, p1.zonal, p1.sph, p1.phase, p1.fwd, p1.bwd, a1, blockIdx.x - split);
}

static unsigned pack_blocks(const MmaGeom& g, int F) {
    return g.split ? (unsigned)(g.MP * F) : (unsigned)(((size_t)F * 2 * g.MP * g.KP + kPackThreads - 1) / kPackThreads);
}

static bool ring_forward_image(const fc_dims* d, int records) { return (records & 1) && forward_ring_fits(d); }

size_t packed_filter_floats_fwd(const fc_dims* d, int records) {
    if (ring_forward_image(d, records)) return packed_ring_image_floats(d->O, 2 * d->B + 1, d->I, d->R, halves_of(d));
    return packed_image_floats(d->O, d->R, d->I, 2 * d->B + 1, halves_of(d));
}
size_t packed_filter_floats_bwd(const fc_dims* d, int records) {
    (void)records;
    return packed_image_floats(d->I, d->R, d->O, 2 * d->B + 1, halves_of(d));
}

static unsigned pack_args(PackArgs& a, int ftype, bool want_fwd, bool want_bwd, const fc_dims* d, int records, int o0, int i0, int Ifull) {
    a.O = d->O; a.I = d->I; a.R = d->R; a.B = d->B; a.F = 2 * d->B + 1; a.ftype = ftype;
    a.o0 = o0; a.i0 = i0; a.Ifull = Ifull > 0 ? Ifull : d->I;
    a.ring_f = ring_forward_image(d, records & 1) ? 1 : 0;
    a.gf = a.ring_f ? ring_geom(d->O, a.F, d->I, halves_of(d)) : make_mma_geom(d->O, d->R, d->I, halves_of(d));
    a.gb = make_mma_geom(d->I, d->R, d->O, halves_of(d));
    a.blocks_f = want_fwd ? pack_blocks(a.gf, a.ring_f ? a.R : a.F) : 0u;
    const unsigned blocks_b = pack_blocks(a.gb, a.F);
    return a.blocks_f + (want_bwd ? blocks_b : 0u);
}

int pack_filter_params_pair_impl(const fc_filter_params& f0, float* fwd0, float* bwd0, const fc_dims* d0, const fc_filter_params& f1,
                                 float* fwd1, float* bwd1, const fc_dims* d1, int records, hipStream_t stream) {
    PackArgs a0, a1;
    const unsigned n0 = pack_args(a0, f0.ftype, fwd0 != nullptr, bwd0 != nullptr, d0, records, 0, 0, 0);
    const unsigned n1 = pack_args(a1, f1.ftype, fwd1 != nullptr, bwd1 != nullptr, d1, records, 0, 0, 0);
    if (n0 == 0 || n1 == 0) return FC_ERR_BAD_ARGUMENT;
    const PackPtrs p0{f0.zonal, f0.spherical, f0.phase, fwd0, bwd0}, p1{f1.zonal, f1.spherical, f1.phase, fwd1, bwd1};
    hipLaunchKernelGGL(fc_pack_filter_pair_kernel, dim3(n0 + n1), dim3(kPackThreads), 0, stream, p0, a0, p1, a1, n0);
    return hipGetLastError() == hipSuccess ? FC_OK : FC_ERR_LAUNCH;
}

template <bool FROM_PARAMS>
static int launch_pack(const float* w_eff, const float* zonal, const float* sph, const float* phase, int ftype, float* wpk_fwd,
                       float* wpk_bwd, const fc_dims* d, int records, hipStream_t stream, int o0 = 0, int i0 = 0, int Ifull = 0) {
    PackArgs a;
    const unsigned blocks = pack_args(a, ftype, wpk_fwd != nullptr, wpk_bwd != nullptr, d, records, o0, i0, Ifull);
    if (blocks == 0) return FC_ERR_BAD_ARGUMENT;
    hipLaunchKernelGGL(fc_pack_filter_kernel<FROM_PARAMS>, dim3(blocks), dim3(kPackThreads), 0, stream,
                       reinterpret_cast<const float2*>(w_eff), zonal, sph, phase, wpk_fwd, wpk_bwd, a);
    return hipGetLastError() == hipSuccess ? FC_OK : FC_ERR_LAUNCH;
}

int pack_filter_impl(const float* w_eff, float* wpk_fwd, float* wpk_bwd, const fc_dims* d, int records, hipStream_t stream) {
    return launch_pack<false>(w_eff, nullptr, nullptr, nullptr, 0, wpk_fwd, wpk_bwd, d, records, stream);
}

int pack_filter_params_impl(const float* zonal, const float* sph, const float* phase, int ftype, float* wpk_fwd,
                            float* wpk_bwd, const fc_dims* d, int records, hipStream_t stream) {
    return launch_pack<true>(nullptr, zonal, sph, phase, ftype, wpk_fwd, wpk_bwd, d, records, stream);
}

int pack_filter_params_block_impl(const float* zonal, const float* sph, const float* phase, int ftype, float* wpk_fwd, float* wpk_bwd,
                                  const fc_dims* d, int records, int o0, int i0, int Ifull, hipStream_t stream) {
    return launch_pack<true>(nullptr, zonal, sph, phase, ftype, wpk_fwd, wpk_bwd, d, records, stream, o0, i0, Ifull);
}

int pack_filter_block_impl(const float* w_eff, float* wpk_fwd, float* wpk_bwd, const fc_dims* d, int records, int o0, int i0, int Ifull,
                           hipStream_t stream) {
    return launch_pack<false>(w_eff, nullptr, nullptr, nullptr, 0, wpk_fwd, wpk_bwd, d, records, stream, o0, i0, Ifull);
}


constexpr int kGradPairs = 32;
constexpr int kMaxB = 3;

__device__ __forceinline__ void param_grads_entry(const float2* g, const float* __restrict__ zonal, const float* __restrict__ sph,
                                                  const float* __restrict__ phase, int ftype, float* __restrict__ g_zonal,
                                                  float* __restrict__ g_sph, float* gph_row, int I, int R, int B, int o, int i, int r) {
    const size_t oi = (size_t)o * I + i;
    const size_t oir = oi * R + r;
    if (ftype == 2) {
        g_zonal[oir * 2] = g[B].x;
        g_zonal[oir * 2 + 1] = g[B].y;
        for (int b = 0; b < 2 * B; ++b) {
            const float2 v = g[b < B ? b : b + 1];
            g_sph[(oir * (2 * B) + b) * 2] = v.x;
            g_sph[(oir * (2 * B) + b) * 2 + 1] = v.y;
        }
        return;
    }
    for (int q = 0; q <= B; ++q) {
        float s = 0.f, co = 1.f;
        if (ftype == 1) sincosf(phase[oi * (B + 1) + q], &s, &co);
        const float2 P = make_float2(co, s);
        const float2 gp = g[B + q];
        const float2 cp = filter_entry(zonal, sph, phase, 0, B, R, I, o, i, r, B + q);
        float2 gP = cmul_conj(gp, cp);
        const float2 gcp = cmul_conj(gp, P);
        float acc = P.x * gP.y - P.y * gP.x;
        if (q == 0) {
            g_zonal[oir] = gcp.x;
        } else {
            const float2 gm = g[B - q];
            const float2 cm = filter_entry(zonal, sph, phase, 0, B, R, I, o, i, r, B - q);
            gP = cmul_conj(gm, cm);
            const float2 gcm = cmul_conj(gm, P);
            acc += P.x * gP.y - P.y * gP.x;
            g_sph[(oir * B + (q - 1)) * 2] = gcp.x + gcm.x;
            g_sph[(oir * B + (q - 1)) * 2 + 1] = gcp.y - gcm.y;
        }
        gph_row[q] = acc;
    }
}

__global__ void fc_filter_param_grads_kernel(const float2* __restrict__ gw, const float* __restrict__ zonal,
                                             const float* __restrict__ sph, const float* __restrict__ phase, int ftype,
                                             float* __restrict__ g_zonal, float* __restrict__ g_sph,
                                             float* __restrict__ g_phase, int O, int I, int R, int B) {
    __shared__ float gph[kGradPairs * 8 * (kMaxB + 1)];
    const int pair = threadIdx.x / R, r = threadIdx.x - pair * R;
    const int oi = blockIdx.x * kGradPairs + pair;
    const bool valid = oi < O * I;
    const int F = 2 * B + 1;
    const int o = oi / I, i = oi - o * I;
    if (valid)
        param_grads_entry(gw + ((size_t)oi * R + r) * F, zonal, sph, phase, ftype, g_zonal, g_sph, gph + (pair * 8 + r) * (kMaxB + 1), I, R, B,
                          o, i, r);
    __syncthreads();
    if (valid && ftype == 1 && r == 0) {
        for (int q = 0; q <= B; ++q) {
            float acc = 0.f;
            for (int rr = 0; rr < R; ++rr) acc += gph[(pair * 8 + rr) * (kMaxB + 1) + q];
            g_phase[(size_t)oi * (B + 1) + q] = acc;
        }
    }
}

constexpr int kRpPairs = 16;
constexpr int kRpThreads = 1024;
constexpr int kRpGroups = 4;
constexpr int kRpMaxPer = 16;
struct RpStrides { size_t sp, sr, sf, so; int pairs; };

__global__ __launch_bounds__(kRpThreads) void fc_reduce_param_grads_kernel(
    const float2* __restrict__ gwp, const RpStrides st, const int P, float2* __restrict__ gw_out, const float* __restrict__ zonal,
    const float* __restrict__ sph, const float* __restrict__ phase, const int ftype, float* __restrict__ g_zonal,
    float* __restrict__ g_sph, float* __restrict__ g_phase, const int O, const int I, const int R, const int B, const int po0,
    const int pi0, const int Ifull, const float* __restrict__ bias_partials, const int bias_nparts, float* __restrict__ g_bias,
    const int bias_block0, const f32x4* __restrict__ gx_parts, f32x4* __restrict__ gx, const size_t gx_count4, const size_t gx_stride4,
    const int gx_nparts, const size_t gx_tail_floats, const int gx_block0, const float2* __restrict__ gx_x, const int dbg) {
    __shared__ float2 part[kRpGroups][kRpPairs * 8 * 7];
    __shared__ float2 gws[kRpPairs * 8 * 7];
    __shared__ float gph[kRpPairs * 8 * (kMaxB + 1)];
    if ((int)blockIdx.x >= gx_block0 && gx_nparts < 0) {
        const size_t idx = (size_t)((int)blockIdx.x - gx_block0) * kRpThreads + threadIdx.x;
        if (idx >= gx_count4) return;
        const float2* gxt = reinterpret_cast<const float2*>(gx_parts);
        float2* out = reinterpret_cast<float2*>(gx);
        const float2 xv = gx_x[idx];
        const int bl = (-gx_nparts) & 3, ks = 1 + ((-gx_nparts) >> 2);
        out[idx] = bl == 1 ? gx_from_slices<1>(xv, gxt, idx, gx_count4, ks)
                 : bl == 2 ? gx_from_slices<2>(xv, gxt, idx, gx_count4, ks) : gx_from_slices<3>(xv, gxt, idx, gx_count4, ks);
        return;
    }
    if ((int)blockIdx.x >= gx_block0) {
        const size_t idx = (size_t)((int)blockIdx.x - gx_block0) * kRpThreads + threadIdx.x;
        if (idx >= gx_count4) return;
        f32x4 s = gx_parts[idx];
        for (int p = 1; p < gx_nparts; ++p) s += gx_parts[(size_t)p * gx_stride4 + idx];
        if (idx + 1 < gx_count4 || gx_tail_floats == 0) gx[idx] = s;
        else {
            float* dd = reinterpret_cast<float*>(gx + idx);
            for (size_t k = 0; k < gx_tail_floats; ++k) dd[k] = s[k];
        }
        return;
    }
    if ((int)blockIdx.x >= bias_block0) {
        const int lane = threadIdx.x & 63;
        const int c = ((int)blockIdx.x - bias_block0) * (kRpThreads / 64) + (threadIdx.x >> 6);
        if (c >= O) return;
        float s = 0.f;
        for (int p = lane; p < bias_nparts; p += 64) s += bias_partials[(size_t)p * O + c];
#pragma unroll
        for (int d = 32; d >= 1; d >>= 1) s += __shfl_xor(s, d, 64);
        if (lane == 0) g_bias[c] = s;
        return;
    }
    if (dbg & 8) return;
    const int F = 2 * B + 1;
    const int nit = (I + kRpPairs - 1) / kRpPairs;
    const int o = blockIdx.x / nit, i0 = (blockIdx.x - o * nit) * kRpPairs;
    const int nent = kRpPairs * R * F;
    const int per = (P + kRpGroups - 1) / kRpGroups;
    for (int idx = threadIdx.x; idx < nent * kRpGroups; idx += kRpThreads) {
        const int grp = idx / nent, e = idx - grp * nent;
        const int pi = e % kRpPairs, rf = e / kRpPairs;
        const int f = rf % F, r = rf / F;
        const int i = i0 + pi;
        float2 s = make_float2(0.f, 0.f);
        if (i < I && !(dbg & 1)) {
            const size_t ro = st.pairs ? (size_t)dump_k(r, o, R, O, true) * st.so : (size_t)r * st.sr + (size_t)o * st.so;
            const float2* src = gwp + ro + (size_t)f * st.sf + i;
            const int pend = min((grp + 1) * per, P);
            for (int p0 = grp * per; p0 < pend; p0 += kRpMaxPer) {
                float2 v[kRpMaxPer];
#pragma unroll
                for (int u = 0; u < kRpMaxPer; ++u) v[u] = (p0 + u < pend) ? src[(size_t)(p0 + u) * st.sp] : make_float2(0.f, 0.f);
#pragma unroll
                for (int u = 0; u < kRpMaxPer; ++u) { s.x += v[u].x; s.y += v[u].y; }
            }
        }
        part[grp][e] = s;
    }
    __syncthreads();
    if (dbg & 4) { if (threadIdx.x == 0 && g_zonal) g_zonal[blockIdx.x] = part[0][0].x; return; }
    const float sc = 1.f / (float)F;
    for (int e = threadIdx.x; e < nent; e += kRpThreads) {
        const int pi = e % kRpPairs, rf = e / kRpPairs;
        const int f = rf % F, r = rf / F;
        float2 s = part[0][e];
#pragma unroll
        for (int grp = 1; grp < kRpGroups; ++grp) { s.x += part[grp][e].x; s.y += part[grp][e].y; }
        s.x *= sc;
        s.y *= sc;
        gws[(pi * 8 + r) * 7 + f] = s;
    }
    __syncthreads();
    if (gw_out) {
        const int RF = R * F;
        const int npi = min(kRpPairs, I - i0);
        float2* const dst = gw_out + ((size_t)o * I + i0) * RF;
        for (int j = threadIdx.x; j < npi * RF; j += kRpThreads) {
            const int pi = j / RF, rem = j - pi * RF;
            const int r = rem / F, f = rem - r * F;
            dst[j] = gws[(pi * 8 + r) * 7 + f];
        }
    }
    const int pair = threadIdx.x / R, r = threadIdx.x - pair * R;
    const bool valid = pair < kRpPairs && i0 + pair < I;
    if (valid && !(dbg & 2))
        param_grads_entry(gws + (pair * 8 + r) * 7, zonal, sph, phase, ftype, g_zonal, g_sph, gph + (pair * 8 + r) * (kMaxB + 1), Ifull, R, B,
                          po0 + o, pi0 + i0 + pair, r);
    __syncthreads();
    if (valid && ftype == 1 && r == 0) {
        for (int q = 0; q <= B; ++q) {
            float acc = 0.f;
            for (int rr = 0; rr < R; ++rr) acc += gph[(pair * 8 + rr) * (kMaxB + 1) + q];
            g_phase[((size_t)(po0 + o) * Ifull + pi0 + i0 + pair) * (B + 1) + q] = acc;
        }
    }
}

int reduce_param_grads_impl(const float* gwp, size_t sp, size_t sr, size_t sf, size_t so, bool ring_pairs, int P, float* gw_eff,
                            const float* zonal, const float* sph, const float* phase, int ftype, float* g_zonal, float* g_sph,
                            float* g_phase, const fc_dims* d, hipStream_t stream, int o0, int i0, int Ifull, const float* bias_partials,
                            int bias_nparts, float* g_bias, const float* gx_parts, float* gx, size_t gx_count, size_t gx_stride, int gx_nparts,
                            const float* gx_x) {
    if (d->R > 8 || d->B > kMaxB || kRpPairs * d->R > kRpThreads) return FC_ERR_UNSUPPORTED;
    const int nit = (d->I + kRpPairs - 1) / kRpPairs;
    const RpStrides st{sp, sr, sf, so, ring_pairs ? 1 : 0};
    const int main_blocks = d->O * nit;
    static const int dbg = [] { const char* e = dev_env("FC_DEBUG_RP"); return e ? atoi(e) : 0; }();
    const int bias_blocks = (bias_partials && bias_nparts > 0 && g_bias) ? (d->O + kRpThreads / 64 - 1) / (kRpThreads / 64) : 0;
    const bool sum_gx = gx_parts && gx && gx_nparts > 1;
    const bool from_slices = gx_parts && gx && gx_x && gx_nparts < 0;
    const size_t gx_floats = gx_count * 2, gx_count4 = from_slices ? gx_count : sum_gx ? (gx_floats + 3) / 4 : 0;
    const int gx_blocks = (int)((gx_count4 + kRpThreads - 1) / kRpThreads);
    hipLaunchKernelGGL(fc_reduce_param_grads_kernel, dim3(main_blocks + bias_blocks + gx_blocks), dim3(kRpThreads), 0, stream,
                       reinterpret_cast<const float2*>(gwp), st, P, reinterpret_cast<float2*>(gw_eff), zonal, sph, phase, ftype, g_zonal, g_sph,
                       g_phase, d->O, d->I, d->R, d->B, o0, i0, Ifull > 0 ? Ifull : d->I, bias_partials, bias_nparts, g_bias, main_blocks,
                       reinterpret_cast<const f32x4*>(gx_parts), reinterpret_cast<f32x4*>(gx), gx_count4, gx_stride / 2, gx_nparts,
                       gx_floats % 4, main_blocks + bias_blocks, reinterpret_cast<const float2*>(gx_x), dbg);
    return hipGetLastError() == hipSuccess ? FC_OK : FC_ERR_LAUNCH;
}

int filter_param_grads_impl(const float* gw_eff, const float* zonal, const float* sph, const float* phase, int ftype,
                            float* g_zonal, float* g_sph, float* g_phase, const fc_dims* d, hipStream_t stream) {
    if (d->R > 8 || d->B > kMaxB) return FC_ERR_UNSUPPORTED;
    const int total = d->O * d->I;
    hipLaunchKernelGGL(fc_filter_param_grads_kernel, dim3((total + kGradPairs - 1) / kGradPairs), dim3(kGradPairs * d->R), 0, stream,
                       reinterpret_cast<const float2*>(gw_eff), zonal, sph, phase, ftype, g_zonal, g_sph, g_phase, d->O, d->I,
                       d->R, d->B);
    return hipGetLastError() == hipSuccess ? FC_OK : FC_ERR_LAUNCH;
}

}
```

fieldconv_amd/csrc/fc_wide.hip:

```cpp
#include "fc_common.hpp"
#include "fc_kernels.hpp"
#include "fc_tile.hpp"

namespace fc {

struct WidePlan {
    int blk, nib, nob;
    fc_dims db;
    size_t x_blocks, y_block, gy_blocks, gx_parts, gx_block, wpk, gw_block, conv_ws, total_fwd, total_bwd;
};

static size_t align256(size_t v) { return (v + 255) / 256 * 256; }

static bool wide_plan(const fc_dims* d, int blk, int records, WidePlan& p) {
    if (blk <= 0 || blk > kMaxChannels) return false;
    p.blk = blk;
    p.nib = (d->I + blk - 1) / blk;
    p.nob = (d->O + blk - 1) / blk;
    p.db = *d;
    p.db.I = blk;
    p.db.O = blk;
    const size_t rows = (size_t)d->N;
    p.x_blocks = align256(rows * p.nib * blk * 8);
    p.y_block = align256(rows * blk * 8);
    p.gy_blocks = align256(rows * p.nob * blk * 8);
    p.gx_parts = align256(rows * blk * 8) * p.nob;
    p.gx_block = align256(rows * blk * 8);
    const size_t wf = packed_filter_floats_fwd(&p.db, records), wb = packed_filter_floats_bwd(&p.db, records);
    p.wpk = align256((wf > wb ? wf : wb) * sizeof(float));
    p.gw_block = align256((size_t)blk * blk * d->R * (2 * d->B + 1) * 8);
    const size_t fws = records ? forward_workspace_bytes(&p.db, 1) : 0, bws = backward_workspace_bytes(&p.db);
    p.conv_ws = align256(fws > bws ? fws : bws);
    p.total_fwd = p.x_blocks + p.y_block + p.wpk + align256(fws);
    p.total_bwd = p.x_blocks + p.gy_blocks + p.gx_parts + p.gx_block + p.wpk + p.gw_block + align256(bws);
    return true;
}

static int copy_block(float* dst, int ld_dst, const float* src, int ld_src, int rows, int cols, hipStream_t stream) {
    if (rows == 0 || cols == 0) return FC_OK;
    return hipMemcpy2DAsync(dst, (size_t)ld_dst * 8, src, (size_t)ld_src * 8, (size_t)cols * 8, rows, hipMemcpyDeviceToDevice, stream) ==
                   hipSuccess
               ? FC_OK
               : FC_ERR_LAUNCH;
}

}

extern "C" {

size_t fc_wide_workspace_bytes(const fc_dims* dims, int32_t block, int32_t records, int32_t backward) {
    fc::WidePlan p;
    if (!dims || dims->N <= 0 || dims->I <= 0 || dims->O <= 0 || !fc::wide_plan(dims, block, records, p)) return 0;
    return backward ? p.total_bwd : p.total_fwd;
}

int fc_forward_wide(const float* x, const float* sten_or_records, const fc_csr* by_target, int32_t kind, const fc_filter_params* params,
                    const float* w_eff, float* y, void* workspace, size_t workspace_bytes, const fc_dims* dims, int32_t records, int32_t block,
                    void* stream) {
    if (!x || !y || (!params == !w_eff) || !by_target || !dims || kind < 0 || kind > 2 || ((kind != 0) != (records != 0)))
        return FC_ERR_BAD_ARGUMENT;
    fc::WidePlan p;
    if (!fc::wide_plan(dims, block, records, p)) return FC_ERR_BAD_ARGUMENT;
    if (!fc_supported(&p.db)) return FC_ERR_UNSUPPORTED;
    if (!by_target->rowptr || (dims->E > 0 && (!sten_or_records || (records ? !by_target->runs : !by_target->nbr)))) return FC_ERR_BAD_ARGUMENT;
    if (records && (dims->R > 8 || !fc::rows_fit_32bit(&p.db))) return FC_ERR_UNSUPPORTED;
    if (!workspace || workspace_bytes < p.total_fwd) return FC_ERR_WORKSPACE;
    hipStream_t st = static_cast<hipStream_t>(stream);
    char* w = static_cast<char*>(workspace);
    float* xb = reinterpret_cast<float*>(w);
    float* yb = reinterpret_cast<float*>(w + p.x_blocks);
    float* wpk = reinterpret_cast<float*>(w + p.x_blocks + p.y_block);
    void* cws = w + p.x_blocks + p.y_block + p.wpk;
    const size_t cws_bytes = p.total_fwd - (p.x_blocks + p.y_block + p.wpk);
    const int N = dims->N, I = dims->I, O = dims->O, blk = p.blk;
    const size_t xstride = (size_t)N * blk * 2;
    for (int ib = 0; ib < p.nib; ++ib) {
        const int bi = (I - ib * blk) < blk ? (I - ib * blk) : blk;
        const int rc = fc::copy_block(xb + ib * xstride, bi, x + 2 * (size_t)ib * blk, I, N, bi, st);
        if (rc != FC_OK) return rc;
    }
    for (int ob = 0; ob < p.nob; ++ob) {
        const int bo = (O - ob * blk) < blk ? (O - ob * blk) : blk;
        for (int ib = 0; ib < p.nib; ++ib) {
            const int bi = (I - ib * blk) < blk ? (I - ib * blk) : blk;
            fc_dims d = *dims;
            d.I = bi;
            d.O = bo;
            int rc = params ? fc::pack_filter_params_block_impl(params->zonal, params->spherical, params->phase, params->ftype, wpk, nullptr, &d,
                                                                records, ob * blk, ib * blk, I, st)
                            : fc::pack_filter_block_impl(w_eff, wpk, nullptr, &d, records, ob * blk, ib * blk, I, st);
            if (rc != FC_OK) return rc;
            fc_epilogue epi = {ib > 0 ? yb : nullptr, nullptr, nullptr};
            const size_t fws = records ? fc::forward_workspace_bytes(&d, kind) : 0;
            rc = fc::forward_impl(xb + ib * xstride, sten_or_records, by_target, wpk, yb, &d, kind, fws && fws <= cws_bytes ? cws : nullptr,
                                  fws && fws <= cws_bytes ? fws : 0, ib > 0 ? &epi : nullptr, st);
            if (rc != FC_OK) return rc;
        }
        const int rc = fc::copy_block(y + 2 * (size_t)ob * blk, O, yb, bo, N, bo, st);
        if (rc != FC_OK) return rc;
    }
    return FC_OK;
}

int fc_backward_wide(const float* x, const float* gy, const float* sten_or_rec_s, const fc_csr* by_source, int32_t records,
                     const fc_filter_params* params, const float* w_eff, float* gw_eff, float* gx, void* workspace, size_t workspace_bytes,
                     const fc_dims* dims, int32_t block, void* stream) {
    if (!x || !gy || !gx || (!params == !w_eff) || !by_source || !dims) return FC_ERR_BAD_ARGUMENT;
    if (params ? (!params->g_zonal || !params->g_spherical) : !gw_eff) return FC_ERR_BAD_ARGUMENT;
    fc::WidePlan p;
    if (!fc::wide_plan(dims, block, records, p)) return FC_ERR_BAD_ARGUMENT;
    if (!fc_supported(&p.db)) return FC_ERR_UNSUPPORTED;
    if (!by_source->rowptr || (dims->E > 0 && (!sten_or_rec_s || (records ? !by_source->runs : !by_source->nbr)))) return FC_ERR_BAD_ARGUMENT;
    if (records && (dims->R > 8 || !fc::rows_fit_32bit(&p.db))) return FC_ERR_UNSUPPORTED;
    if (!workspace || workspace_bytes < p.total_bwd) return FC_ERR_WORKSPACE;
    hipStream_t st = static_cast<hipStream_t>(stream);
    char* w = static_cast<char*>(workspace);
    float* xb = reinterpret_cast<float*>(w);
    float* gyb = reinterpret_cast<float*>(w + p.x_blocks);
    float* parts = reinterpret_cast<float*>(w + p.x_blocks + p.gy_blocks);
    float* gxb = reinterpret_cast<float*>(w + p.x_blocks + p.gy_blocks + p.gx_parts);
    float* wpk = reinterpret_cast<float*>(w + p.x_blocks + p.gy_blocks + p.gx_parts + p.gx_block);
    float* gwb = reinterpret_cast<float*>(w + p.x_blocks + p.gy_blocks + p.gx_parts + p.gx_block + p.wpk);
    void* cws = w + p.x_blocks + p.gy_blocks + p.gx_parts + p.gx_block + p.wpk + p.gw_block;
    const size_t cws_bytes = p.total_bwd - (p.x_blocks + p.gy_blocks + p.gx_parts + p.gx_block + p.wpk + p.gw_block);
    const int N = dims->N, I = dims->I, O = dims->O, blk = p.blk;
    const size_t bstride = (size_t)N * blk * 2;
    const size_t pstride = p.gx_parts / p.nob / sizeof(float);
    for (int ib = 0; ib < p.nib; ++ib) {
        const int bi = (I - ib * blk) < blk ? (I - ib * blk) : blk;
        const int rc = fc::copy_block(xb + ib * bstride, bi, x + 2 * (size_t)ib * blk, I, N, bi, st);
        if (rc != FC_OK) return rc;
    }
    for (int ob = 0; ob < p.nob; ++ob) {
        const int bo = (O - ob * blk) < blk ? (O - ob * blk) : blk;
        const int rc = fc::copy_block(gyb + ob * bstride, bo, gy + 2 * (size_t)ob * blk, O, N, bo, st);
        if (rc != FC_OK) return rc;
    }
    for (int ib = 0; ib < p.nib; ++ib) {
        const int bi = (I - ib * blk) < blk ? (I - ib * blk) : blk;
        for (int ob = 0; ob < p.nob; ++ob) {
            const int bo = (O - ob * blk) < blk ? (O - ob * blk) : blk;
            fc_dims d = *dims;
            d.I = bi;
            d.O = bo;
            int rc = params ? fc::pack_filter_params_block_impl(params->zonal, params->spherical, params->phase, params->ftype, nullptr, wpk, &d,
                                                                records, ob * blk, ib * blk, I, st)
                            : fc::pack_filter_block_impl(w_eff, nullptr, wpk, &d, records, ob * blk, ib * blk, I, st);
            if (rc != FC_OK) return rc;
            float* part = p.nob == 1 ? gxb : parts + ob * pstride;
            rc = fc::backward_data_impl(xb + ib * bstride, gyb + ob * bstride, sten_or_rec_s, by_source, wpk, part, cws, cws_bytes, &d, records != 0,
                                        st);
            if (rc != FC_OK) return rc;
            rc = fc::backward_filter_impl(xb + ib * bstride, cws, cws_bytes, &d, st, records != 0);
            if (rc != FC_OK) return rc;
            if (params) {
                fc_filter_params block_params = *params;
                block_params.bias_partials = nullptr;
                block_params.bias_nparts = 0;
                block_params.g_bias = nullptr;
                rc = fc::backward_finish_params_impl(gwb, cws, cws_bytes, &d, &block_params, st, ob * blk, ib * blk, I, nullptr, records != 0);
            } else {
                rc = fc::backward_finish_impl(gwb, cws, cws_bytes, &d, st, records != 0);
                const int rf = dims->R * (2 * dims->B + 1);
                if (rc == FC_OK)
                    rc = fc::copy_block(gw_eff + 2 * (((size_t)ob * blk * I + (size_t)ib * blk) * rf), I * rf, gwb, bi * rf, bo, bi * rf, st);
            }
            if (rc != FC_OK) return rc;
        }
        if (p.nob > 1) {
            const int rc = fc::sum_parts(parts, gxb, (size_t)N * bi, pstride / 2, p.nob, st);
            if (rc != FC_OK) return rc;
        }
        const int rc = fc::copy_block(gx + 2 * (size_t)ib * blk, I, gxb, bi, N, bi, st);
        if (rc != FC_OK) return rc;
    }
    if (params && params->bias_partials) {
        if (params->bias_nparts <= 0 || !params->g_bias) return FC_ERR_BAD_ARGUMENT;
        return fc::bias_partials_reduce_impl(params->bias_partials, params->bias_nparts, O, params->g_bias, st);
    }
    return FC_OK;
}

}
```

fieldconv_amd/functional.py:

```python
import ctypes
import math
import os

import torch

from . import _lib
from ._lib import FcCsr, FcDims, FcEpilogue, FcFilterParams, check


class KernelTimer:

    def __init__(self):
        self.enabled = False
        self.stride = 1
        self.events = {}
        self.count = {}
        self.pool = []

    def reset(self, pairs=0):
        self.events = {}
        self.count = {}
        self.pool = [(torch.cuda.Event(enable_timing=True), torch.cuda.Event(enable_timing=True)) for _ in range(pairs)]

    def elapsed_ms(self):
        return {k: [a.elapsed_time(b) for a, b in v] for k, v in self.events.items()}


kernel_timer = KernelTimer()
KEEP_GW_EFF = False
_ONE_CALL = os.environ.get('FIELDCONV_SEPARATE_CALLS', '0') != '1'


class _timed:
    def __init__(self, name):
        self.name = name

    def __enter__(self):
        self.on = False
        if kernel_timer.enabled:
            n = kernel_timer.count.get(self.name, 0)
            kernel_timer.count[self.name] = n + 1
            self.on = n % kernel_timer.stride == 0
        if self.on:
            if kernel_timer.pool:
                self.a, self.b = kernel_timer.pool.pop()
            else:
                self.a = torch.cuda.Event(enable_timing=True)
                self.b = torch.cuda.Event(enable_timing=True)
            self.a.record()

    def __exit__(self, *exc):
        if self.on:
            self.b.record()
            kernel_timer.events.setdefault(self.name, []).append((self.a, self.b))
        return False


def _require_device(t, what):
    if not t.is_cuda:
        raise RuntimeError(f'{what}: fieldconv_amd runs on a ROCm device only (got a {t.device} tensor); '
                           'there is no CPU fallback')


def on_device(t):
    return t.is_cuda


_raw_stream = getattr(torch._C, '_cuda_getCurrentRawStream', None)
_cur_device = getattr(torch._C, '_cuda_getDevice', None)


def _stream():
    if _raw_stream is not None and _cur_device is not None:
        return ctypes.c_void_p(_raw_stream(_cur_device()))
    return ctypes.c_void_p(torch.cuda.current_stream().cuda_stream)


class _NoGuard:
    def __enter__(self):
        return self

    def __exit__(self, *exc):
        return False


_NO_GUARD = _NoGuard()


def _on(device):
    if _cur_device is not None and device.index is not None and _cur_device() == device.index:
        return _NO_GUARD
    return torch.cuda.device(device)


def _p(t):
    return ctypes.c_void_p(t.data_ptr())


def _dp(t):
    return t.data_ptr() if t is not None else None


def _po(t):
    return ctypes.c_void_p(t.data_ptr()) if t is not None else None


def _csr(rowptr, nbr, runs=None):
    return FcCsr(rowptr.data_ptr(), nbr.data_ptr() if nbr.numel() else None, _dp(runs))


def _by_target(csr):
    return _csr(csr.rowptr_t, csr.nbr_t, None)


def _by_source(csr):
    return _csr(csr.rowptr_s, csr.nbr_s, None)


def _records(graph):
    if graph.geo_t is not None:
        return 2, graph.geo_t, graph.rec_s
    if graph.factored:
        return 1, graph.rec_t, graph.rec_s
    return 0, graph.sten_t, graph.sten_s


def _scratch(nbytes, device, floor=0):
    if floor is None:
        if not nbytes:
            return None
        floor = 0
    return torch.empty(max(int(nbytes), floor), dtype=torch.uint8, device=device)


def _carve(shapes, device, zero=False, extra=None):
    counts = [math.prod(shp) for shp in shapes if shp is not None]
    sizes = [(n + 3) // 4 * 4 for n in counts]
    flat = (torch.zeros if zero else torch.empty)(sum(sizes) + (extra or 0), dtype=torch.float32, device=device)
    parts = iter(flat.split(sizes if extra is None else sizes + [extra]))
    counts = iter(counts)
    out = []
    for shp in shapes:
        if shp is None:
            out.append(None)
        else:
            n = next(counts)
            out.append(next(parts)[:n].view(shp) if n % 4 else next(parts).view(shp))
    if extra is not None:
        out.append(next(parts))
    return out


def _edge_split():
    return os.environ.get('FIELDCONV_NO_EDGE_SPLIT', '0') != '1'


def _split_finish():
    return os.environ.get('FC_SPLIT_FINISH', '0') not in ('', '0')


def _epilogue(addend, bias, act):
    if addend is None and bias is None:
        return None
    return FcEpilogue(_dp(addend), _dp(bias), _dp(act))


def _filter_params(params, grads=None, bias_sum=None):
    zonal, spherical, phase, ftype = params
    g_z, g_s, g_p = grads if grads is not None else (None, None, None)
    fp = FcFilterParams(zonal.data_ptr(), spherical.data_ptr(), phase.data_ptr(), ftype, _dp(g_z), _dp(g_s), _dp(g_p))
    if bias_sum is not None:
        fp.bias_partials, fp.bias_nparts, fp.g_bias = bias_sum[0].data_ptr(), bias_sum[1], bias_sum[2].data_ptr()
    return fp


def make_dims(graph, I, O, B):
    return FcDims(graph.N, graph.E, int(I), int(O), graph.R, int(B))


def supported(graph, I, O, B):
    return bool(_lib.load().fc_supported(ctypes.byref(make_dims(graph, I, O, B))))


@_lib.keep_mode
class _FieldConvFn(torch.autograd.Function):

    @staticmethod
    def forward(ctx, x, w_eff, graph):
        lib = _lib.load()
        x = x.contiguous()
        w_eff = w_eff.contiguous()
        O, I, R, F = w_eff.shape
        B = (F - 1) // 2
        plan = _conv_plan(lib, graph, I, O, B)
        with _on(x.device):
            st = _stream()

            def pack(pl, wpk_f, wpk_b):
                check(lib.fc_pack_filter(_p(w_eff), _p(wpk_f), _po(wpk_b), pl.dref, pl.records, st), 'fc_pack_filter')
            y, wpk_b = _run_forward(lib, x, graph, plan, O, st, pack)
        ctx.save_for_backward(x, wpk_b)
        ctx.graph = graph
        ctx.wshape = (O, I, R, F)
        return y

    @staticmethod
    def backward(ctx, gy):
        lib = _lib.load()
        x, wpk_b = ctx.saved_tensors
        O, I, R, F = ctx.wshape
        plan = _conv_plan(lib, ctx.graph, I, O, (F - 1) // 2)
        gy = gy.contiguous()
        with _on(x.device):
            gx, gw, _ = _launch_backward(lib, x, gy, ctx.graph, wpk_b, plan, ctx.wshape, _stream())
        return gx, gw, None


class _ConvPlan:
    __slots__ = ('dims', 'dref', 'n_fwd', 'n_bwd', 'ws_fwd', 'ws_bwd', 'csr_t', 'csr_s', 'cref_t', 'cref_s', 'records')


def _conv_plan(lib, graph, I, O, B):
    key = (int(I), int(O), int(B))
    plan = graph._plans.get(key)
    if plan is not None:
        return plan
    plan = _ConvPlan()
    plan.dims = make_dims(graph, I, O, B)
    plan.dref = ctypes.byref(plan.dims)
    if not lib.fc_supported(plan.dref):
        raise _lib.FieldConvNativeError(
            f'FieldConv(in={I}, out={O}, n_rings={graph.R}, band_limit={B}) is outside the compiled HIP kernels '
            '(channels <= 64; (n_rings, band_limit) as listed in csrc/fc_kernels.hpp)')
    plan.records = lib.fc_records_flags(plan.dref, 1 if graph.factored else 0)
    plan.n_fwd = lib.fc_packed_filter_floats_fwd(plan.dref, plan.records)
    plan.n_bwd = lib.fc_packed_filter_floats_bwd(plan.dref, plan.records)
    plan.ws_bwd = lib.fc_backward_workspace_bytes(plan.dref, plan.records)
    plan.ws_fwd = 0
    if graph.factored and _edge_split():
        plan.ws_fwd = lib.fc_forward_workspace_bytes(plan.dref)
    plan.csr_t = _csr(graph.rowptr_t, graph.nbr_t, graph.runs_t)
    plan.csr_s = _csr(graph.rowptr_s, graph.nbr_s, graph.runs_s)
    plan.cref_t, plan.cref_s = ctypes.byref(plan.csr_t), ctypes.byref(plan.csr_s)
    graph._plans[key] = plan
    return plan


def _forward_buffers(x, plan, O, addend, bias, out=None, row0=0):
    n = plan.dims.N
    if out is None:
        y = torch.empty((n, O), dtype=torch.complex64, device=x.device)
        act = torch.empty_like(y) if bias is not None else None
    else:
        y, act = out[0][row0:row0 + n], (out[1][row0:row0 + n] if out[1] is not None else None)
        addend = addend[row0:row0 + n] if addend is not None else None
    epi = _epilogue(addend, bias, act)
    return y, act, (ctypes.byref(epi) if epi is not None else None), _scratch(plan.ws_fwd, x.device, None)


def _launch_forward(lib, x, graph, wpk_f, plan, O, st, addend=None, bias=None, out=None, row0=0):
    y, act, epi, ws = _forward_buffers(x, plan, O, addend, bias, out, row0)
    kind, recs, _ = _records(graph)
    with _timed('fc_forward'):
        if kind == 0:
            check(lib.fc_forward(_p(x), _p(recs), plan.cref_t, _p(wpk_f), _p(y), plan.dref, epi, st), 'fc_forward')
        else:
            name = 'fc_forward_geometric' if kind == 2 else 'fc_forward_factored'
            check(getattr(lib, name)(_p(x), _p(recs), plan.cref_t, _p(wpk_f), _p(y), _po(ws), plan.ws_fwd, plan.dref, epi, st), name)
    return y if bias is None else (y, act)


def _row_plan(lib, graph, whole, row0, nrows):
    key = ('rows', whole.dims.I, whole.dims.O, whole.dims.B, int(row0), int(nrows))
    plan = graph._plans.get(key)
    if plan is not None:
        return plan
    plan = _ConvPlan()
    ends = graph.rowptr_t[[row0, row0 + nrows]].tolist()
    plan.dims = FcDims(int(nrows), int(ends[1] - ends[0]), whole.dims.I, whole.dims.O, graph.R, whole.dims.B)
    plan.dref = ctypes.byref(plan.dims)
    plan.records = whole.records
    plan.n_fwd = lib.fc_packed_filter_floats_fwd(plan.dref, plan.records)
    plan.n_bwd = whole.n_bwd
    plan.ws_bwd = whole.ws_bwd
    plan.ws_fwd = 0
    if _edge_split():
        plan.ws_fwd = lib.fc_forward_workspace_bytes(plan.dref)
    plan.csr_t = _csr(graph.rowptr_t[row0:], graph.nbr_t, graph.runs_t[row0:] if graph.runs_t is not None else None)
    plan.csr_s, plan.cref_s = whole.csr_s, whole.cref_s
    plan.cref_t = ctypes.byref(plan.csr_t)
    graph._plans[key] = plan
    return plan


def _run_forward(lib, x, graph, plan, O, st, pack, addend=None, bias=None, params=None):
    dev = x.device
    wpk_b = torch.empty(plan.n_bwd, dtype=torch.float32, device=dev)
    split, nt = graph.forward_split, graph.n_targets
    between = split[1] if split is not None else None
    if split is not None and graph.factored and 0 < split[0] < nt:
        ranges = ((0, split[0]), (split[0], nt - split[0]))
    elif nt < graph.N and graph.factored:
        ranges = ((0, nt),)
    else:
        if nt < graph.N:
            raise _lib.FieldConvNativeError('restrict_targets needs a graph with factored records')
        wpk_f = torch.empty(plan.n_fwd, dtype=torch.float32, device=dev)
        if params is not None and between is None and _ONE_CALL and not kernel_timer.enabled:
            y, act, epi, ws = _forward_buffers(x, plan, O, addend, bias)
            kind, recs, _ = _records(graph)
            check(lib.fc_forward_params(_p(x), _p(recs), plan.cref_t, kind, ctypes.byref(_filter_params(params)), _p(wpk_f), _p(wpk_b), _p(y),
                                        _po(ws), plan.ws_fwd, plan.dref, plan.records, epi, st), 'fc_forward_params')
            return (y if bias is None else (y, act)), wpk_b
        pack(plan, wpk_f, wpk_b)
        if between is not None:
            between()
        return _launch_forward(lib, x, graph, wpk_f, plan, O, st, addend=addend, bias=bias), wpk_b
    y = torch.empty((nt, O), dtype=torch.complex64, device=dev)
    act = torch.empty_like(y) if bias is not None else None
    if len(ranges) == 1 and between is not None:
        between()
    for row0, nrows in ranges:
        sub = _row_plan(lib, graph, plan, row0, nrows)
        wpk_f = torch.empty(sub.n_fwd, dtype=torch.float32, device=dev)
        pack(sub, wpk_f, wpk_b if row0 == 0 else None)
        _launch_forward(lib, x, graph, wpk_f, sub, O, st, addend=addend, bias=bias, out=(y, act), row0=row0)
        if row0 == 0 and len(ranges) == 2:
            between()
    return (y if bias is None else (y, act)), wpk_b


def _param_grads(params):
    zonal, spherical, phase, ftype = params
    return torch.empty_like(zonal), torch.empty_like(spherical), (torch.empty_like(phase) if ftype == 1 else None)


def _launch_backward(lib, x, gy, graph, wpk_b, plan, wshape, st, params=None, bias_sum=None):
    O, I, R, F = wshape
    gx = torch.empty_like(x)
    want_gw = params is None or KEEP_GW_EFF or _split_finish()
    gw = torch.empty((O, I, R, F), dtype=torch.complex64, device=x.device) if want_gw else None
    nbytes = plan.ws_bwd
    ws = _scratch(nbytes, x.device)
    wsp = _p(ws)
    sten = _records(graph)[2]
    pgrads = fp = None
    if params is not None:
        pgrads = _param_grads(params)
        fp = _filter_params(params, pgrads, bias_sum)
    gwp = _po(gw)
    if graph.on_gx is None and _ONE_CALL and not kernel_timer.enabled:
        check(lib.fc_backward_all(_p(x), _p(gy), _p(sten), plan.cref_s, plan.records, _p(wpk_b), _p(gx), gwp,
                                  ctypes.byref(fp) if fp is not None else None, wsp, nbytes, plan.dref, st), 'fc_backward_all')
        return gx, gw, pgrads
    if kernel_timer.enabled and graph.on_gx is None and graph.factored and lib.fc_backward_streams(plan.dref, plan.records):
        with _timed('fc_backward_data'):
            check(lib.fc_backward_gather(_p(gy), _p(sten), plan.cref_s, _p(wpk_b), wsp, nbytes, plan.dref, st), 'fc_backward_gather')
        with _timed('fc_backward_filter'):
            check(lib.fc_backward_stream(_p(x), _p(wpk_b), _p(gx), wsp, nbytes, plan.dref, st), 'fc_backward_stream')
        if fp is not None:
            check(lib.fc_backward_finish_params(gwp, wsp, nbytes, plan.dref, plan.records, ctypes.byref(fp), st), 'fc_backward_finish_params')
        else:
            check(lib.fc_backward_finish(_p(gw), wsp, nbytes, plan.dref, plan.records, st), 'fc_backward_finish')
        return gx, gw, pgrads
    with _timed('fc_backward_data'):
        if graph.factored:
            check(lib.fc_backward_data_factored(_p(x), _p(gy), _p(sten), plan.cref_s, _p(wpk_b), _p(gx), wsp, nbytes, plan.dref,
                                                plan.records, st), 'fc_backward_data_factored')
        else:
            check(lib.fc_backward_data(_p(x), _p(gy), _p(sten), plan.cref_s, _p(wpk_b), _p(gx), wsp, nbytes, plan.dref, st),
                  'fc_backward_data')
    if graph.on_gx is not None:
        graph.on_gx(gx)
    with _timed('fc_backward_filter'):
        check(lib.fc_backward_filter(_p(x), wsp, nbytes, plan.dref, plan.records, st), 'fc_backward_filter')
    if fp is not None:
        check(lib.fc_backward_finish_params(gwp, wsp, nbytes, plan.dref, plan.records, ctypes.byref(fp), st), 'fc_backward_finish_params')
    else:
        check(lib.fc_backward_finish(_p(gw), wsp, nbytes, plan.dref, plan.records, st), 'fc_backward_finish')
    return gx, gw, pgrads


def _param_packer(lib, params, st):
    zonal, spherical, phase, ftype = params

    def pack(pl, wpk_f, wpk_b):
        check(lib.fc_pack_filter_params(_p(zonal), _p(spherical), _p(phase), ftype, _p(wpk_f), _po(wpk_b), pl.dref, pl.records, st),
              'fc_pack_filter_params')
    return pack


@_lib.keep_mode
class _FieldConvParamFn(torch.autograd.Function):

    @staticmethod
    def forward(ctx, x, zonal, spherical, phase, ftype, B, graph):
        lib = _lib.load()
        x = x.contiguous()
        zonal, spherical, phase = zonal.contiguous(), spherical.contiguous(), phase.contiguous()
        O, I, R = zonal.shape[0], zonal.shape[1], zonal.shape[2]
        F = 2 * B + 1
        plan = _conv_plan(lib, graph, I, O, B)
        with _on(x.device):
            st = _stream()
            params = (zonal, spherical, phase, ftype)
            y, wpk_b = _run_forward(lib, x, graph, plan, O, st, _param_packer(lib, params, st), params=params)
        ctx.save_for_backward(x, wpk_b, zonal, spherical, phase)
        ctx.graph, ctx.ftype, ctx.wshape = graph, ftype, (O, I, R, F)
        return y

    @staticmethod
    def backward(ctx, gy):
        lib = _lib.load()
        x, wpk_b, zonal, spherical, phase = ctx.saved_tensors
        O, I, R, F = ctx.wshape
        plan = _conv_plan(lib, ctx.graph, I, O, (F - 1) // 2)
        gy = gy.contiguous()
        with _on(x.device):
            st = _stream()
            gx, _, (g_z, g_s, g_p) = _launch_backward(lib, x, gy, ctx.graph, wpk_b, plan, ctx.wshape, st,
                                                      params=(zonal, spherical, phase, ctx.ftype))
        return gx, g_z, g_s, g_p, None, None, None


@_lib.keep_mode
class _FieldConvActFn(torch.autograd.Function):

    @staticmethod
    def forward(ctx, x, zonal, spherical, phase, bias, addend, ftype, B, graph):
        lib = _lib.load()
        x = x.contiguous()
        zonal, spherical, phase = zonal.contiguous(), spherical.contiguous(), phase.contiguous()
        bias = bias.contiguous()
        addend = addend.contiguous() if addend is not None else None
        O, I, R = zonal.shape[0], zonal.shape[1], zonal.shape[2]
        F = 2 * B + 1
        plan = _conv_plan(lib, graph, I, O, B)
        with _on(x.device):
            st = _stream()
            params = (zonal, spherical, phase, ftype)
            (pre, act), wpk_b = _run_forward(lib, x, graph, plan, O, st, _param_packer(lib, params, st), addend=addend, bias=bias, params=params)
        ctx.save_for_backward(x, wpk_b, zonal, spherical, phase, bias, pre)
        ctx.graph, ctx.ftype, ctx.wshape, ctx.has_addend = graph, ftype, (O, I, R, F), addend is not None
        return act

    @staticmethod
    def backward(ctx, g_act):
        lib = _lib.load()
        x, wpk_b, zonal, spherical, phase, bias, pre = ctx.saved_tensors
        O, I, R, F = ctx.wshape
        plan = _conv_plan(lib, ctx.graph, I, O, (F - 1) // 2)
        g_act = g_act.contiguous()
        N = pre.shape[0]
        with _on(x.device):
            st = _stream()
            g_pre = torch.empty_like(pre)
            g_bias = torch.empty_like(bias)
            nbytes = lib.fc_tangent_nonlin_backward_workspace_bytes(N, O)
            ws = _scratch(nbytes, x.device)
            check(lib.fc_tangent_nonlin_backward_partial(_p(pre), _p(bias), _p(g_act), _p(g_pre), _p(ws), nbytes, N, O, st),
                  'fc_tangent_nonlin_backward_partial')
            gx, _, (g_z, g_s, g_p) = _launch_backward(lib, x, g_pre, ctx.graph, wpk_b, plan, ctx.wshape, st,
                                                      params=(zonal, spherical, phase, ctx.ftype),
                                                      bias_sum=(ws, lib.fc_tangent_nonlin_backward_groups(N), g_bias))
        return gx, g_z, g_s, g_p, g_bias, (g_pre if ctx.has_addend else None), None, None, None


def field_conv_act(x, zonal, spherical, phase, ftype, band_limit, graph, bias, addend=None):
    _require_device(x, 'field_conv')
    O, I = zonal.shape[0], zonal.shape[1]
    if _run_time_path(x, graph) or max(I, O) > _channel_block(graph, I, O, band_limit) or \
            os.environ.get('FIELDCONV_NO_FUSED_EPILOGUE', '0') == '1':
        h = field_conv_params(x, zonal, spherical, phase, ftype, band_limit, graph)
        if addend is not None:
            h = h + addend
        return tangent_nonlin(h, bias)
    _check_conv(x, graph, I, zonal.shape[2], 2 * band_limit + 1)
    if bias.numel() != O:
        raise ValueError(f'bias has {bias.numel()} channels, the convolution {O}')
    if addend is not None and (addend.dtype != torch.complex64 or tuple(addend.shape) != (graph.n_targets, O)):
        raise ValueError(f'addend must be complex64 of shape ({graph.n_targets}, {O})')
    return _FieldConvActFn.apply(x, zonal, spherical, phase, bias.reshape(-1), addend, int(ftype), int(band_limit), graph)


def _dtype_code(t):
    return 1 if t.dtype in (torch.complex128, torch.float64) else 0


def _cgemm(lib, A, B, C, M, N, K, sam, sak, sbk, sbn, conj_b, alpha):
    dt = _dtype_code(C)
    nbytes = lib.fc_cgemm_workspace_bytes(M, N, K, dt)
    ws = _scratch(nbytes, C.device, None)
    check(lib.fc_cgemm(_p(A), _p(B), _p(C), M, N, K, sam, sak, sbk, sbn, 1 if conj_b else 0, float(alpha), dt, _po(ws), nbytes, _stream()),
          'fc_cgemm')
    return C


@_lib.keep_mode
class _GenericFieldConvFn(torch.autograd.Function):

    @staticmethod
    def forward(ctx, x, w_eff, graph):
        lib = _lib.load()
        x = x.contiguous()
        O, I, R, F = w_eff.shape
        B = (F - 1) // 2
        nt, K = graph.n_targets, I * R * F
        with _on(x.device):
            contrib = _GenericFieldConvFn._gather(lib, x, graph, I, R, B)
            y = torch.empty((nt, O), dtype=x.dtype, device=x.device)
            _cgemm(lib, contrib, w_eff, y, nt, O, K, K, 1, 1, K, False, 1.0 / F)
        ctx.save_for_backward(x, w_eff)
        ctx.graph = graph
        return y

    @staticmethod
    def _gather(lib, x, graph, I, R, B):
        F = 2 * B + 1
        contrib = torch.empty((graph.n_targets, I, R, F), dtype=x.dtype, device=x.device)
        check(lib.fc_generic_gather(_p(x), _p(graph.sten_t), ctypes.byref(_by_target(graph)), _p(contrib), graph.n_targets, I, R, B, _dtype_code(x),
                                    _stream()), 'fc_generic_gather')
        return contrib

    @staticmethod
    def backward(ctx, gy):
        lib = _lib.load()
        x, w_eff = ctx.saved_tensors
        graph = ctx.graph
        O, I, R, F = w_eff.shape
        B = (F - 1) // 2
        nt, K = graph.n_targets, I * R * F
        gy = gy.contiguous()
        with _on(x.device):
            contrib = _GenericFieldConvFn._gather(lib, x, graph, I, R, B)
            g_contrib = torch.empty((nt, K), dtype=x.dtype, device=x.device)
            _cgemm(lib, gy, w_eff, g_contrib, nt, K, O, O, 1, K, 1, True, 1.0 / F)
            gw = torch.empty((O, I, R, F), dtype=x.dtype, device=x.device)
            _cgemm(lib, gy, contrib, gw, O, K, nt, 1, O, K, 1, True, 1.0 / F)
            gx = torch.empty_like(x)
            check(lib.fc_generic_scatter(_p(x), _p(g_contrib), _p(graph.sten_s), ctypes.byref(_by_source(graph)), _p(gx), graph.N, I, R, B, _dtype_code(x),
                                         _stream()), 'fc_generic_scatter')
        return gx, gw, None

# ... 549 lines not shown
```

include/fieldconv_hip.h:

```cpp
#ifndef FIELDCONV_HIP_H
#define FIELDCONV_HIP_H

#include <stddef.h>
#include <stdint.h>

#ifdef __cplusplus
extern "C" {
#endif

typedef enum fc_status {
    FC_OK = 0,
    FC_ERR_BAD_ARGUMENT = -1,
    FC_ERR_UNSUPPORTED = -2,
    FC_ERR_LAUNCH = -3,
    FC_ERR_WORKSPACE = -4
} fc_status;

typedef struct fc_dims {
    int32_t N;
    int32_t E;
    int32_t I;
    int32_t O;
    int32_t R;
    int32_t B;
    int32_t mode;
} fc_dims;

typedef struct fc_csr {
    const int32_t* rowptr;
    const int32_t* nbr;
    const int32_t* runs;
} fc_csr;

int fc_abi_version(void);
typedef enum fc_mfma_mode { FC_MFMA_SPLIT_F16 = 0, FC_MFMA_F32 = 1, FC_MFMA_F16 = 2 } fc_mfma_mode;
int fc_dev_switches(void);
void fc_debug_stamp_buffer(void* device_buffer);
const char* fc_status_string(int status);

int fc_supported(const fc_dims* dims);
int fc_describe_kernels(const fc_dims* dims, int32_t kind, char* buffer, size_t buffer_bytes);

int32_t fc_records_flags(const fc_dims* dims, int32_t record_driven);
size_t fc_packed_filter_floats_fwd(const fc_dims* dims, int32_t records);
size_t fc_packed_filter_floats_bwd(const fc_dims* dims, int32_t records);
int fc_pack_filter(const float* w_eff, float* wpk_fwd, float* wpk_bwd, const fc_dims* dims, int32_t records, void* stream);
int fc_pack_filter_params(const float* zonal, const float* spherical, const float* phase, int32_t ftype,
                          float* wpk_fwd, float* wpk_bwd, const fc_dims* dims, int32_t records, void* stream);
int fc_filter_param_grads(const float* gw_eff, const float* zonal, const float* spherical, const float* phase,
                          int32_t ftype, float* g_zonal, float* g_spherical, float* g_phase,
                          const fc_dims* dims, void* stream);

typedef struct fc_epilogue {
    const float* addend;
    const float* modrelu_bias;
    float* activated;
} fc_epilogue;

int fc_forward(const float* x, const float* sten_t, const fc_csr* by_target, const float* wpk_fwd,
               float* y, const fc_dims* dims, const fc_epilogue* epilogue, void* stream);

int fc_factored_record_floats(int32_t band_limit);
size_t fc_forward_workspace_bytes(const fc_dims* dims);
int fc_forward_factored(const float* x, const float* rec_t, const fc_csr* by_target, const float* wpk_fwd,
                        float* y, void* workspace, size_t workspace_bytes, const fc_dims* dims, const fc_epilogue* epilogue,
                        void* stream);

int fc_geometric_record_floats(void);
int fc_forward_geometric(const float* x, const float* geo_t, const fc_csr* by_target, const float* wpk_fwd,
                         float* y, void* workspace, size_t workspace_bytes, const fc_dims* dims, const fc_epilogue* epilogue,
                         void* stream);

size_t fc_backward_workspace_bytes(const fc_dims* dims, int32_t records);
int fc_backward_data(const float* x, const float* gy, const float* sten_s, const fc_csr* by_source,
                     const float* wpk_bwd, float* gx, void* workspace, size_t workspace_bytes,
                     const fc_dims* dims, void* stream);
int fc_backward_data_factored(const float* x, const float* gy, const float* rec_s, const fc_csr* by_source,
                              const float* wpk_bwd, float* gx, void* workspace, size_t workspace_bytes,
                              const fc_dims* dims, int32_t records, void* stream);
int fc_backward_filter(const float* x, void* workspace, size_t workspace_bytes, const fc_dims* dims, int32_t records, void* stream);
int32_t fc_backward_streams(const fc_dims* dims, int32_t records);
int fc_backward_gather(const float* gy, const float* rec_s, const fc_csr* by_source, const float* wpk_bwd, void* workspace,
                       size_t workspace_bytes, const fc_dims* dims, void* stream);
int fc_backward_stream(const float* x, const float* wpk_bwd, float* gx, void* workspace, size_t workspace_bytes, const fc_dims* dims,
                       void* stream);
int fc_backward_finish(float* gw_eff, void* workspace, size_t workspace_bytes, const fc_dims* dims, int32_t records, void* stream);

typedef struct fc_filter_params {
    const float* zonal;
    const float* spherical;
    const float* phase;
    int32_t ftype;
    float* g_zonal;
    float* g_spherical;
    float* g_phase;
    const float* bias_partials;
    int32_t bias_nparts;
    float* g_bias;
} fc_filter_params;
int fc_forward_params(const float* x, const float* sten_or_records, const fc_csr* by_target, int32_t kind,
                      const fc_filter_params* params, float* wpk_fwd, float* wpk_bwd, float* y, void* workspace,
                      size_t workspace_bytes, const fc_dims* dims, int32_t records, const fc_epilogue* epilogue, void* stream);
int fc_backward_all(const float* x, const float* gy, const float* sten_or_rec_s, const fc_csr* by_source, int32_t records,
                    const float* wpk_bwd, float* gx, float* gw_eff, const fc_filter_params* params, void* workspace,
                    size_t workspace_bytes, const fc_dims* dims, void* stream);
int fc_backward_finish_params(float* gw_eff, void* workspace, size_t workspace_bytes, const fc_dims* dims, int32_t records,
                              const fc_filter_params* params, void* stream);

size_t fc_wide_workspace_bytes(const fc_dims* dims, int32_t block, int32_t records, int32_t backward);
int fc_forward_wide(const float* x, const float* sten_or_records, const fc_csr* by_target, int32_t kind, const fc_filter_params* params,
                    const float* w_eff, float* y, void* workspace, size_t workspace_bytes, const fc_dims* dims, int32_t records,
                    int32_t block, void* stream);
int fc_backward_wide(const float* x, const float* gy, const float* sten_or_rec_s, const fc_csr* by_source, int32_t records,
                     const fc_filter_params* params, const float* w_eff, float* gw_eff, float* gx, void* workspace,
                     size_t workspace_bytes, const fc_dims* dims, int32_t block, void* stream);

typedef enum fc_dtype { FC_F32 = 0, FC_F64 = 1 } fc_dtype;
int fc_shape_compiled(int32_t n_rings, int32_t band_limit);
int fc_generic_gather(const void* x, const void* sten_t, const fc_csr* by_target, void* contrib, int32_t n_targets, int32_t I,
                      int32_t R, int32_t B, int32_t dtype, void* stream);
int fc_generic_scatter(const void* x, const void* g_contrib, const void* sten_s, const fc_csr* by_source, void* gx, int32_t N,
                       int32_t I, int32_t R, int32_t B, int32_t dtype, void* stream);
size_t fc_cgemm_workspace_bytes(int32_t M, int32_t N, int32_t K, int32_t dtype);
int fc_cgemm(const void* A, const void* B, void* C, int32_t M, int32_t N, int32_t K, int64_t sam, int64_t sak, int64_t sbk, int64_t sbn,
             int32_t conj_b, double alpha, int32_t dtype, void* workspace, size_t workspace_bytes, void* stream);

int fc_tangent_lin_forward(const float* x, const float* re_w, const float* im_w, float* y,
                           int32_t N, int32_t I, int32_t O, void* stream);
size_t fc_tangent_lin_backward_workspace_bytes(int32_t N, int32_t I, int32_t O);
int fc_tangent_lin_backward(const float* x, const float* gy, const float* re_w, const float* im_w,
                            float* gx, float* g_re, float* g_im, void* workspace, size_t workspace_bytes,
                            int32_t N, int32_t I, int32_t O, void* stream);

int fc_tangent_nonlin_forward(const float* x, const float* bias, float* y, int32_t N, int32_t C, void* stream);
size_t fc_tangent_nonlin_backward_workspace_bytes(int32_t N, int32_t C);
int fc_tangent_nonlin_backward(const float* x, const float* bias, const float* gy, float* gx, float* gbias,
                               void* workspace, size_t workspace_bytes, int32_t N, int32_t C, void* stream);
int32_t fc_tangent_nonlin_backward_groups(int32_t N);
int fc_tangent_nonlin_backward_partial(const float* x, const float* bias, const float* gy, float* gx, void* workspace,
                                       size_t workspace_bytes, int32_t N, int32_t C, void* stream);

int fc_soft_abs_forward(const float* x, float* y, size_t count, void* stream);
int fc_soft_abs_backward(const float* x, const float* gy, float* gx, size_t count, void* stream);

int fc_tangent_nonlin_forward_f64(const double* x, const double* bias, double* y, int32_t N, int32_t C, void* stream);
size_t fc_tangent_nonlin_backward_workspace_bytes_f64(int32_t N, int32_t C);
int fc_tangent_nonlin_backward_f64(const double* x, const double* bias, const double* gy, double* gx, double* gbias,
                                   void* workspace, size_t workspace_bytes, int32_t N, int32_t C, void* stream);

int fc_echo_hist_dim(int32_t n_bins);
int fc_echo_channel_block(int32_t n_bins);
int fc_echo_forward(const float* x, const float* ln_t, const float* wxp_t, const fc_csr* by_target, float* hist,
                    float* desc, int32_t N, int32_t E, int32_t C, int32_t n_bins, void* stream);
int fc_echo_backward(const float* x, const float* ln_s, const float* wxp_s, const fc_csr* by_source, const float* hist,
                     const float* g_desc, float* gx, float* hist_grad_workspace, int32_t N, int32_t E, int32_t C,
                     int32_t n_bins, void* stream);

int fc_trans_field_forward(const float* x, const float* lift_sten, const fc_csr* by_target, const int64_t* slot_to_edge,
                           const float* zonal_ang, const float* zonal_mag, const float* phase, float* y, float* ang,
                           float* mag, float* s1sum, int32_t N, int32_t E, int32_t Cin, int32_t O, int32_t R, int32_t sten_stride,
                           void* stream);
size_t fc_trans_field_backward_workspace_bytes(int32_t N, int32_t Cin, int32_t O, int32_t R);
int fc_trans_field_backward(const float* lift_sten, const fc_csr* by_source, const int64_t* slot_to_edge_s,
                            const float* zonal_ang, const float* zonal_mag, const float* phase, const float* ang,
                            const float* mag, const float* s1sum, const float* gy, float* gx, float* g_zonal_ang,
                            float* g_zonal_mag, float* g_phase, void* workspace, size_t workspace_bytes, int32_t N,
                            int32_t E, int32_t Cin, int32_t O, int32_t R, int32_t sten_stride, int32_t ftype, void* stream);

typedef struct fc_mesh {
    int32_t N, E, R, B;
    int32_t kind;
    const fc_csr* by_target;
    const fc_csr* by_source;
    const float* fwd;
    const float* bwd;
    int32_t mode;
} fc_mesh;

typedef struct fc_resnet_block_params {
    int32_t C_in, C_mid, C_out;
    fc_filter_params conv1, conv2;
    const float* bias1;
    const float* bias2;
    const float* res_re;
    const float* res_im;
    float* g_bias1;
    float* g_bias2;
    float* g_res_re;
    float* g_res_im;
} fc_resnet_block_params;
size_t fc_resnet_block_saved_bytes(const fc_mesh* mesh, const fc_resnet_block_params* p);
size_t fc_resnet_block_workspace_bytes(const fc_mesh* mesh, const fc_resnet_block_params* p, int32_t backward);
int fc_resnet_block_forward(const float* x, const fc_mesh* mesh, const fc_resnet_block_params* p, float* out, void* saved,
                            size_t saved_bytes, void* workspace, size_t workspace_bytes, void* stream);
int fc_resnet_block_backward(const float* x, const float* g_out, const fc_mesh* mesh, const fc_resnet_block_params* p, const void* saved,
                             size_t saved_bytes, float* gx, void* workspace, size_t workspace_bytes, void* stream);

typedef struct fc_echo_block_params {
    int32_t C_in, n_des, n_bins;
    fc_filter_params conv;
    const float* bias;
    float* g_bias;
} fc_echo_block_params;
size_t fc_echo_block_saved_bytes(const fc_mesh* mesh, const fc_echo_block_params* p);
size_t fc_echo_block_workspace_bytes(const fc_mesh* mesh, const fc_echo_block_params* p, int32_t backward);
int fc_echo_block_forward(const float* x, const fc_mesh* mesh, const float* ln_t, const float* wxp_t, const fc_echo_block_params* p,
                          float* desc, void* saved, size_t saved_bytes, void* workspace, size_t workspace_bytes, void* stream);
int fc_echo_block_backward(const float* x, const float* g_desc, const fc_mesh* mesh, const float* ln_s, const float* wxp_s,
                           const fc_echo_block_params* p, const void* saved, size_t saved_bytes, float* gx, void* workspace,
                           size_t workspace_bytes, void* stream);

typedef struct fc_echo_head_params {
    int32_t D, H1, H2, C_in, C_out;
    const float *w1, *b1, *w2, *b2, *w3, *b3, *wr, *br;
    float *g_w1, *g_b1, *g_w2, *g_b2, *g_w3, *g_b3, *g_wr, *g_br;
} fc_echo_head_params;
size_t fc_echo_head_forward_workspace_bytes(int32_t N, const fc_echo_head_params* p);
int fc_echo_head_forward(const float* d, const float* x, const fc_echo_head_params* p, float* h1, float* h2, float* y, void* workspace,
                         size_t workspace_bytes, int32_t N, void* stream);
size_t fc_echo_head_backward_workspace_bytes(int32_t N, const fc_echo_head_params* p);
int fc_echo_head_backward(const float* d, const float* x, const float* h1, const float* h2, const float* g, const fc_echo_head_params* p,
                          float* g_d, float* gx, float* g_h1, void* workspace, size_t workspace_bytes, int32_t N, void* stream);

typedef struct fc_lift_block_params {
    int32_t C_in, C_out, ftype;
    const float* zonal_ang;
    const float* zonal_mag;
    const float* phase;
    const float* bias;
    float* g_zonal_ang;
    float* g_zonal_mag;
    float* g_phase;
    float* g_bias;
} fc_lift_block_params;
size_t fc_lift_block_saved_bytes(const fc_mesh* mesh, const fc_lift_block_params* p);
size_t fc_lift_block_workspace_bytes(const fc_mesh* mesh, const fc_lift_block_params* p, int32_t backward);
int fc_lift_block_forward(const float* x, const float* lift_sten, int32_t sten_stride, const fc_mesh* mesh, const int64_t* slot_to_edge_t,
                          const fc_lift_block_params* p, float* out, void* saved, size_t saved_bytes, void* stream);
int fc_lift_block_backward(const float* g_out, const float* lift_sten, int32_t sten_stride, const fc_mesh* mesh, const int64_t* slot_to_edge_s,
                           const fc_lift_block_params* p, const void* saved, size_t saved_bytes, float* gx, void* workspace,
                           size_t workspace_bytes, void* stream);

int fc_trans_field_forward_generic(const void* x, const void* lift_sten, const fc_csr* by_target, const int64_t* slot_to_edge,
                                   const void* zonal_ang, const void* zonal_mag, const void* phase, void* y, void* ang, void* mag,
                                   void* s1sum, int32_t N, int32_t E, int32_t Cin, int32_t O, int32_t R, int32_t sten_stride, int32_t dtype,
                                   void* stream);
size_t fc_trans_field_backward_generic_workspace_bytes(int32_t N, int32_t Cin, int32_t O, int32_t R, int32_t dtype);
int fc_trans_field_backward_generic(const void* lift_sten, const fc_csr* by_source, const int64_t* slot_to_edge_s, const void* zonal_ang,
                                    const void* zonal_mag, const void* phase, const void* ang, const void* mag, const void* s1sum,
                                    const void* gy, void* gx, void* g_zonal_ang, void* g_zonal_mag, void* g_phase, void* workspace,
                                    size_t workspace_bytes, int32_t N, int32_t E, int32_t Cin, int32_t O, int32_t R, int32_t sten_stride,
                                    int32_t ftype, int32_t dtype, void* stream);
int fc_echo_hist_dim_generic(int32_t n_bins);
size_t fc_echo_generic_workspace_bytes(int32_t n_bins);
int fc_echo_forward_generic(const void* x, const void* ln_t, const void* wxp_t, const fc_csr* by_target, void* hist, void* desc,
                            void* workspace, size_t workspace_bytes, int32_t N, int32_t E, int32_t C, int32_t n_bins, int32_t dtype,
                            void* stream);
int fc_echo_backward_generic(const void* x, const void* ln_s, const void* wxp_s, const fc_csr* by_source, const void* hist,
                             const void* g_desc, void* gx, void* hist_grad_workspace, void* workspace, size_t workspace_bytes, int32_t N,
                             int32_t E, int32_t C, int32_t n_bins, int32_t dtype, void* stream);

size_t fc_graph_workspace_bytes(int32_t N, int32_t E, int32_t R, int32_t F, int32_t with_stencil);
int fc_graph_build(const int64_t* supp_edges, const float* supp_sten, int32_t N, int32_t E, int32_t R, int32_t F,
                   int32_t* rowptr_t, int32_t* nbr_t, int32_t* runs_t, int64_t* perm_t, int32_t* rowptr_s,
                   int32_t* nbr_s, int32_t* runs_s, int64_t* perm_s, float* rec_t, float* rec_s, float* geo_t,
                   int32_t* flags, void* workspace, size_t workspace_bytes, void* stream);

size_t fc_precomp_workspace_bytes(int32_t N, int32_t E);
int fc_precomp_mark(const float* log_mag, const int64_t* supp_edges, float epsilon, int32_t N, int32_t E, void* workspace,
                    size_t workspace_bytes, void* stream);
const int32_t* fc_precomp_kept_count_ptr(const void* workspace, int32_t E);
int fc_precomp_build(const float* log_mag, const float* log_ang, const float* xp, const float* w, const int64_t* supp_edges,
                     float epsilon, int32_t N, int32_t E, int32_t R, int32_t F, int64_t* supp_edges_out, float* supp_sten,
                     float* ln, float* wxp, void* workspace, size_t workspace_bytes, void* stream);
int fc_precomp_graph(const float* log_mag, const float* log_ang, const float* xp, const float* w, const int64_t* supp_edges,
                     float epsilon, int32_t N, int32_t E, int32_t E_kept, int32_t R, int32_t F, int32_t rec_pad_rows,
                     int32_t geo_pad_rows, int64_t* supp_edges_out, float* ln, float* wxp, float* factors, int32_t* rowptr_t, int32_t* nbr_t, int32_t* runs_t, int64_t* perm_t,
                     int32_t* rowptr_s, int32_t* nbr_s, int32_t* runs_s, int64_t* perm_s, float* rec_t, float* rec_s, float* geo_t,
                     int32_t* flags, void* precomp_workspace, size_t precomp_workspace_bytes, void* graph_workspace,
                     size_t graph_workspace_bytes, void* stream);

int fc_adam_step(float* params, const float* grads, float* exp_avg, float* exp_avg_sq, float* step, size_t n, float lr,
                 float beta1, float beta2, float eps, float weight_decay, void* stream);

size_t fc_fps_workspace_bytes(int32_t N);
int fc_fps(const float* pos, int32_t N, int32_t n_samples, int32_t start, int64_t* idx, void* workspace, size_t workspace_bytes,
           void* stream);
size_t fc_radius_workspace_bytes(int32_t N);
int fc_radius_count(const float* pos, int32_t N, float epsilon, int32_t max_num_neighbors, void* workspace, size_t workspace_bytes,
                    void* stream);
const int64_t* fc_radius_edge_count_ptr(const void* workspace, int32_t N);
int fc_radius_fill(const float* pos, int32_t N, float epsilon, int32_t max_num_neighbors, int64_t E, int64_t* supp_edges,
                   void* workspace, size_t workspace_bytes, void* stream);

size_t fc_fps_batched_workspace_bytes(int32_t N);
int fc_fps_batched(const float* pos, const int64_t* pos_ptr, int32_t N, int32_t B, const int64_t* n_samples, const int64_t* start,
                   const int64_t* out_ptr, int64_t S_total, int64_t* idx, void* workspace, size_t workspace_bytes, void* stream);
int fc_radius_count_batched(const float* pos, const int64_t* ptr, int32_t N, int32_t B, float epsilon, int32_t max_num_neighbors,
                            void* workspace, size_t workspace_bytes, void* stream);
int fc_radius_fill_batched(const float* pos, const int64_t* ptr, int32_t N, int32_t B, float epsilon, int32_t max_num_neighbors, int64_t E,
                           int64_t* supp_edges, void* workspace, size_t workspace_bytes, void* stream);

int fc_pair_sqdist(const void* xS, int32_t N_S, const void* xT, int32_t N_T, int32_t C, int32_t dtype, const int64_t* pairs, int64_t K,
                   void* d2, void* stream);
size_t fc_twin_loss_workspace_bytes(int64_t P, int64_t M);
int fc_twin_loss_forward(const void* xS, int32_t N_S, const void* xT, int32_t N_T, int32_t C, int32_t dtype, const int64_t* p_, int64_t P,
                         const int64_t* n_, int64_t M, const void* yN, double mu, void* d2, void* loss, void* workspace,
                         size_t workspace_bytes, void* stream);
int fc_twin_loss_backward(const void* xS, int32_t N_S, const void* xT, int32_t N_T, int32_t C, int32_t dtype, const int64_t* p_, int64_t P,
                          const int64_t* n_, int64_t M, const void* yN, double mu, const void* d2, const void* grad_loss,
                          const int64_t* rowptr_T, const int64_t* order_T, const int64_t* rowptr_S, const int64_t* order_S, void* grad_xT,
                          void* grad_xS, void* stream);
int fc_twin_count_dense(const void* xS, int32_t N_S, const void* xT, int32_t N_T, int32_t C, int32_t dtype, const double* thresholds,
                        int32_t n_thresholds, int64_t* counts, void* stream);
size_t fc_label_smoothing_workspace_bytes(int64_t N, int32_t K);
int fc_label_smoothing_forward(const void* pred, const int64_t* target, const void* weight, int64_t N, int32_t K, int32_t dtype,
                               double confidence, double off_value, void* loss, void* workspace, size_t workspace_bytes, void* stream);
int fc_label_smoothing_backward(const void* pred, const int64_t* target, const void* weight, const void* grad_loss, int64_t N, int32_t K,
                                int32_t dtype, double confidence, double off_value, void* grad_pred, void* stream);


size_t fc_segment_pool_workspace_bytes(int32_t N, int32_t B, int32_t C, int32_t dtype);
int fc_segment_pool_soft_abs_forward(const void* x, const int64_t* ptr, int32_t N, int32_t B, int32_t C, int32_t dtype, int32_t reduce,
                                     void* out, void* workspace, size_t workspace_bytes, void* stream);
int fc_segment_pool_soft_abs_backward(const void* x, const void* grad_out, const int64_t* ptr, int32_t N, int32_t B, int32_t C,
                                      int32_t dtype, int32_t reduce, void* grad_x, void* stream);
int fc_segment_pool_forward(const void* x, const int64_t* ptr, int32_t N, int32_t B, int32_t C, int32_t dtype, int32_t reduce, void* out,
                            void* workspace, size_t workspace_bytes, void* stream);
int fc_segment_pool_backward(const void* grad_out, const int64_t* ptr, int32_t N, int32_t B, int32_t C, int32_t dtype, int32_t reduce,
                             void* grad_x, void* stream);

size_t fc_match_workspace_bytes(int32_t N_T, int32_t k, int32_t parts);
int fc_match_topk(const void* xS, int32_t N_S, const void* xT, int32_t N_T, int32_t C, int32_t dtype, const int64_t* ptr_S,
                  const int64_t* ptr_T, int32_t B, const int64_t* exclude, int32_t k, int32_t parts, int64_t* idx, void* d2,
                  void* workspace, size_t workspace_bytes, void* stream);

size_t fc_linear_ce_workspace_bytes(int32_t N, int32_t H, int32_t K, int32_t parts, int32_t pass, int32_t k);
int fc_linear_ce_forward(const float* h, const float* weight, const float* bias, const int64_t* target, int32_t N, int32_t H, int32_t K,
                         double confidence, double off_value, int64_t ignore_index, int32_t parts, float* lse, float* loss_rows,
                         float* total, void* workspace, size_t workspace_bytes, void* stream);
int fc_linear_topk(const float* h, const float* weight, const float* bias, int32_t N, int32_t H, int32_t K, int32_t k, int32_t parts,
                   int64_t* idx, float* z, void* workspace, size_t workspace_bytes, void* stream);
int fc_linear_ce_backward_input(const float* h, const float* weight, const float* bias, const int64_t* target, const float* lse,
                                const float* row_scale, int32_t N, int32_t H, int32_t K, double confidence, double off_value,
                                int64_t ignore_index, float* grad_h, void* stream);
int fc_linear_ce_backward_weight(const float* h, const float* weight, const float* bias, const int64_t* target, const float* lse,
                                 const float* row_scale, int32_t N, int32_t H, int32_t K, double confidence, double off_value,
                                 int64_t ignore_index, int32_t parts, float* grad_weight, float* grad_bias, void* workspace,
                                 size_t workspace_bytes, void* stream);

int32_t fc_geodesic_lds_vertices(void);
int fc_mesh_edge_lengths(const float* pos, const int32_t* src, const int32_t* nbr, int32_t V, int32_t E, float* length, void* stream);
int fc_geodesic_rows(const int32_t* rowptr, const int32_t* nbr, const float* length, int32_t V, int32_t E, const int64_t* sources, int32_t S,
                     float* dist, int32_t* sweeps, void* stream);
size_t fc_geodesic_workspace_bytes(int32_t V, int32_t max_range);
int fc_geodesic_nearest(const int32_t* rowptr, const int32_t* nbr, const float* length, int32_t V, int32_t E, const int64_t* pos_ptr,
                        const int64_t* sources, const int64_t* src_ptr, int32_t S, int32_t B, int32_t max_range, float* dist,
                        int64_t* label, int32_t* sweeps, void* workspace, size_t workspace_bytes, void* stream);
int fc_face_areas(const float* pos, const int64_t* face, int32_t V, int32_t F, float* area, void* stream);
int fc_segment_sum_f32(const float* x, const int64_t* ptr, int64_t N, int32_t K, float divisor, float* out, void* stream);

int32_t fc_geodesic_fps_lds_vertices(void);
size_t fc_geodesic_fps_workspace_bytes(int32_t V, int32_t max_range);
int fc_geodesic_fps(const int32_t* rowptr, const int32_t* nbr, const float* length, int32_t V, int32_t E, const int64_t* pos_ptr, int32_t B,
                    int32_t max_range, const int64_t* n_samples, const int64_t* start, const int64_t* out_ptr, int64_t total_out,
                    int64_t* idx, float* dist, int64_t* sweeps, void* workspace, size_t workspace_bytes, void* stream);
// ... 32 lines not shown
```

Baseline: 1848.

## Precompute 16-byte (x, unit phase) rows for the ring-major geometric forward kernel

Adds a pass that writes each input element together with its unit phase as a 16-byte row in the forward workspace. The ring-major geometric forward kernel then gathers these rows instead of recomputing the rsqrt-based phase for every edge. The pass rides as extra workgroups on the filter-packing launch, so it adds no separate launch. The cost is doubled gather bytes per row and extra workspace, and the path only applies when a matching XU variant is compiled.

After: 1869, median of 6. +1.2%, better.

```diff
diff --git a/fieldconv_amd/_env.py b/fieldconv_amd/_env.py
--- a/fieldconv_amd/_env.py
+++ b/fieldconv_amd/_env.py
@@ -6,6 +6,7 @@
     'FC_GROUP_SPLIT': '0: the backward data kernel never runs the two frequency groups of a tile as separate work items; 2 (development): wherever legal',
     'FC_RING_COMPACT': '0: no compact LDS plans (aliased partials, half-size record chunks) for the ring-major forward kernel',
     'FC_RING_HALVES': '0: no half tiles in the last round of the ring-major forward kernel',
+    'FC_RING_XU': '0: the ring-major forward kernel fetches rows of x and forms the unit phase per edge, instead of 16-byte (x, u) rows from the workspace',
     'FC_HALF_TILES': '0: no half tiles in the frequency-major kernels; 2: half tiles in the backward kernels too',
     'FC_BWD_STREAM': '0: the data / filter kernel pair on large meshes too, instead of the H-streaming arrangement (gather + stream + gx kernels)',
     'FC_GATHER_WPG': '16 / 4: the gather kernel of the H-streaming arrangement as one 16-wavefront workgroup per CU / as five 4-wavefront ones, whatever its registers say',
@@ -51,7 +52,7 @@
     'FC_DIST_CONFIG4': '1: the distributed GPU test worker runs config 4\'s per-rank size (20 000 owned vertices per rank)',
 }
 
-LIBRARY_SWITCHES = ('FC_BWD_STREAM', 'FC_GATHER_WPG', 'FC_RING', 'FC_GROUP_SPLIT', 'FC_RING_COMPACT', 'FC_RING_HALVES', 'FC_HALF_TILES', 'FC_FILTER2', 'FC_SPLIT_FINISH',
+LIBRARY_SWITCHES = ('FC_BWD_STREAM', 'FC_GATHER_WPG', 'FC_RING', 'FC_GROUP_SPLIT', 'FC_RING_COMPACT', 'FC_RING_HALVES', 'FC_RING_XU', 'FC_HALF_TILES', 'FC_FILTER2', 'FC_SPLIT_FINISH',
                     'FC_EDGE_PARTS_MAX', 'FC_ECHO_WPV', 'FC_STAMP_KERNEL', 'FC_DEBUG', 'FC_DEBUG_BWD', 'FC_DEBUG_RP', 'FC_DEBUG_RG', 'FC_LIN_DIRECT')
 
 PREFIXES = ('FC_', 'FIELDCONV_', 'BENCH_')
diff --git a/fieldconv_amd/_lib.py b/fieldconv_amd/_lib.py
--- a/fieldconv_amd/_lib.py
+++ b/fieldconv_amd/_lib.py
@@ -94,6 +94,7 @@
     'fc_forward': (ctypes.c_int, [_vp, _vp, _CP, _vp, _vp, _DP, _EP, _vp]),
     'fc_factored_record_floats': (ctypes.c_int, [_c_int32]),
     'fc_forward_workspace_bytes': (_sz, [_DP]),
+    'fc_forward_rows_workspace_bytes': (_sz, [_DP]),
     'fc_forward_factored': (ctypes.c_int, [_vp, _vp, _CP, _vp, _vp, _vp, _sz, _DP, _EP, _vp]),
     'fc_geometric_record_floats': (ctypes.c_int, []),
     'fc_forward_geometric': (ctypes.c_int, [_vp, _vp, _CP, _vp, _vp, _vp, _sz, _DP, _EP, _vp]),
diff --git a/fieldconv_amd/csrc/fc_api.hip b/fieldconv_amd/csrc/fc_api.hip
--- a/fieldconv_amd/csrc/fc_api.hip
+++ b/fieldconv_amd/csrc/fc_api.hip
@@ -112,6 +112,11 @@
 size_t fc_forward_workspace_bytes(const fc_dims* dims) {
     if (!fc::dims_valid(dims) || !fc::dims_supported(dims)) return 0;
     return fc::forward_workspace_bytes(dims, 1);
+}
+
+size_t fc_forward_rows_workspace_bytes(const fc_dims* dims) {
+    if (!fc::dims_valid(dims) || !fc::dims_supported(dims)) return 0;
+    return fc::forward_workspace_bytes_any(dims);
 }
 
 int fc_forward_factored(const float* x, const float* rec_t, const fc_csr* by_target, const float* wpk_fwd, float* y,
@@ -269,6 +274,21 @@
                       const fc_filter_params* params, float* wpk_fwd, float* wpk_bwd, float* y, void* workspace,
                       size_t workspace_bytes, const fc_dims* dims, int32_t records, const fc_epilogue* epilogue, void* stream) {
     if (!params || kind < 0 || kind > 2 || ((kind != 0) != ((records & 1) != 0))) return FC_ERR_BAD_ARGUMENT;
+    if (kind == 2 && x && dims && fc::dims_valid(dims) && fc::dims_supported(dims) && dims->R <= 8 && fc::rows_fit_32bit(dims)) {
+        const fc::UnitRows rows = fc::forward_unit_rows(x, dims, kind, workspace, workspace_bytes);
+        if (rows.xu) {
+            if (!params->zonal || !params->spherical || (!wpk_fwd && !wpk_bwd)) return FC_ERR_BAD_ARGUMENT;
+            if (params->ftype < 0 || params->ftype > 2 || (params->ftype == 1 && !params->phase)) return FC_ERR_BAD_ARGUMENT;
+            if (!epilogue_valid(epilogue)) return FC_ERR_BAD_ARGUMENT;
+            if (!y || !wpk_fwd || !by_target || !by_target->rowptr) return FC_ERR_BAD_ARGUMENT;
+            if (dims->E > 0 && (!sten_or_records || !by_target->runs)) return FC_ERR_BAD_ARGUMENT;
+            const int prc = fc::pack_filter_params_impl(params->zonal, params->spherical, params->phase, params->ftype, wpk_fwd, wpk_bwd, dims,
+                                                        records, static_cast<hipStream_t>(stream), &rows);
+            if (prc != FC_OK) return prc;
+            return fc::forward_impl(x, sten_or_records, by_target, wpk_fwd, y, dims, 2, workspace, workspace_bytes, epilogue,
+                                    static_cast<hipStream_t>(stream), true);
+        }
+    }
     const int rc = fc_pack_filter_params(params->zonal, params->spherical, params->phase, params->ftype, wpk_fwd, wpk_bwd, dims,
                                          records, stream);
     if (rc != FC_OK) return rc;
diff --git a/fieldconv_amd/csrc/fc_common.hpp b/fieldconv_amd/csrc/fc_common.hpp
--- a/fieldconv_amd/csrc/fc_common.hpp
+++ b/fieldconv_amd/csrc/fc_common.hpp
@@ -51,6 +51,12 @@
     return *reinterpret_cast<const float2*>(reinterpret_cast<const char*>(base) + off);
 }
 
+__device__ __forceinline__ f32x4 gather_row16(const void* __restrict__ base, int vertex, uint32_t row_bytes, uint32_t lane_bytes) {
+    uint32_t off;
+    asm("v_mad_u32_u24 %0, %1, %2, %3" : "=v"(off) : "v"(vertex), "s"(row_bytes), "v"(lane_bytes));
+    return *reinterpret_cast<const f32x4*>(reinterpret_cast<const char*>(base) + off);
+}
+
 template <int BEGIN, int END, class Fn>
 __device__ __forceinline__ void static_for(Fn&& fn) {
     if constexpr (BEGIN < END) {
@@ -145,6 +151,14 @@
 }
 __device__ __forceinline__ f32x2 cmul_conj_pk(f32x2 a, f32x2 b) {
     return cmul_conj_pk_step2(a, b, cmul_conj_pk_step1(a, b));
+}
+
+__device__ __forceinline__ f32x2 unit_phase_pk(f32x2 z) {
+#pragma clang fp contract(off)
+    const bool org = (fabsf(z.x) < kOriginEps) && (fabsf(z.y) < kOriginEps);
+    const f32x2 sq = z * z;
+    const float inv = __frsqrt_rn(sq.x + sq.y);
+    return org ? f32x2{1.f, 0.f} : f32x2{z.x * inv, -z.y * inv};
 }
 
 template <int B>
@@ -167,11 +181,7 @@
 }
 
 template <int B>
-__device__ __forceinline__ void rotate_geometric(f32x2 x, f32x2 c, f32x2 g, f32x2 (&z)[2 * B + 1]) {
-    const bool org = (fabsf(x.x) < kOriginEps) && (fabsf(x.y) < kOriginEps);
-    const f32x2 sq = x * x;
-    const float inv = __frsqrt_rn(sq.x + sq.y);
-    const f32x2 u = org ? f32x2{1.f, 0.f} : f32x2{x.x * inv, -x.y * inv};
+__device__ __forceinline__ void rotate_geometric(f32x2 x, f32x2 u, f32x2 c, f32x2 g, f32x2 (&z)[2 * B + 1]) {
     const f32x2 v = cmul_pk(g, u);
     z[B] = cmul_pk(c, x);
     if (B >= 1) {
@@ -183,6 +193,10 @@
         z[B + m] = cmul_pk(z[B + m - 1], v);
         z[B - m] = cmul_conj_pk(z[B - m + 1], v);
     }
+}
+template <int B>
+__device__ __forceinline__ void rotate_geometric(f32x2 x, f32x2 c, f32x2 g, f32x2 (&z)[2 * B + 1]) {
+    rotate_geometric<B>(x, unit_phase_pk(x), c, g, z);
 }
 constexpr int kGeoRecordFloats = 8;
 constexpr int kGeoLogChunkRecords = 5;
diff --git a/fieldconv_amd/csrc/fc_forward.hip b/fieldconv_amd/csrc/fc_forward.hip
--- a/fieldconv_amd/csrc/fc_forward.hip
+++ b/fieldconv_amd/csrc/fc_forward.hip
@@ -8,13 +8,20 @@
                                             int, void*, size_t, const fc_epilogue*, hipStream_t);
 
 int forward_impl(const float* x, const float* sten, const fc_csr* g, const float* wpk, float* y, const fc_dims* d,
-                 int kind, void* ws, size_t ws_bytes, const fc_epilogue* epi, hipStream_t stream) {
-    if (kind != 0 && forward_ring_fits(d)) return forward_ring_impl(x, sten, g, wpk, y, d, kind, ws, ws_bytes, epi, stream);
+                 int kind, void* ws, size_t ws_bytes, const fc_epilogue* epi, hipStream_t stream, bool unit_rows_ready) {
+    if (kind != 0 && forward_ring_fits(d)) return forward_ring_impl(x, sten, g, wpk, y, d, kind, ws, ws_bytes, epi, stream, unit_rows_ready);
     return halves_of(d) ? forward_impl_mode<true>(x, sten, g, wpk, y, d, kind, ws, ws_bytes, epi, stream)
                         : forward_impl_mode<false>(x, sten, g, wpk, y, d, kind, ws, ws_bytes, epi, stream);
 }
 
-size_t forward_workspace_bytes(const fc_dims* d, int kind) { return forward_workspace_bytes_impl(d, kind); }
+size_t forward_workspace_bytes(const fc_dims* d, int kind) {
+    const size_t parts = forward_workspace_bytes_impl(d, kind), rows = unit_rows_bytes(d, kind);
+    return rows ? unit_rows_offset(parts) + rows : parts;
+}
+size_t forward_workspace_bytes_any(const fc_dims* d) {
+    const size_t a = forward_workspace_bytes(d, 1), b = forward_workspace_bytes(d, 2);
+    return a > b ? a : b;
+}
 
 bool forward_fits(const fc_dims* d) {
     const MmaGeom g = make_mma_geom(d->O, d->R, d->I, halves_of(d));
diff --git a/fieldconv_amd/csrc/fc_forward_ring.hip b/fieldconv_amd/csrc/fc_forward_ring.hip
--- a/fieldconv_amd/csrc/fc_forward_ring.hip
+++ b/fieldconv_amd/csrc/fc_forward_ring.hip
@@ -15,13 +15,33 @@
     return force || (d->N + kTile - 1) / kTile > num_cus();
 }
 
+static bool unit_rows_apply(const fc_dims* d, int kind) {
+    static const bool off = [] { const char* e = dev_env("FC_RING_XU"); return e && atoi(e) == 0; }();
+    if (off || kind != 2 || !forward_ring_fits(d) || (uint64_t)d->N * d->I * 16 >= (1ull << 32)) return false;
+    return ring_xu_compiled(d->R, d->B, true, plan_ring(d->O, 2 * d->B + 1, d->I, halves_of(d)).logh);
+}
+size_t unit_rows_bytes(const fc_dims* d, int kind) { return unit_rows_apply(d, kind) ? (((size_t)d->N * d->I * 16 + 255) & ~(size_t)255) : 0; }
+UnitRows forward_unit_rows(const float* x, const fc_dims* d, int kind, void* ws, size_t ws_bytes) {
+    UnitRows r{x, nullptr, (size_t)d->N * d->I};
+    const size_t bytes = unit_rows_bytes(d, kind), off = unit_rows_offset(forward_workspace_bytes_impl(d, kind));
+    if (bytes && ws && ws_bytes >= off + bytes && (reinterpret_cast<uintptr_t>(ws) & 15) == 0) r.xu = static_cast<char*>(ws) + off;
+    return r;
+}
+int unit_rows_impl(const UnitRows& r, hipStream_t stream) {
+    if (!r.xu || r.count == 0) return FC_OK;
+    hipLaunchKernelGGL(fc_unit_rows_kernel, dim3(unit_rows_blocks(r.count)), dim3(kUnitRowsThreads), 0, stream,
+                       reinterpret_cast<const float2*>(r.x), static_cast<f32x4*>(r.xu), r.count);
+    return hipGetLastError() == hipSuccess ? FC_OK : FC_ERR_LAUNCH;
+}
+
 void describe_forward(const fc_dims* d, int kind, char* buf, size_t n) {
     const char* mode = halves_of(d) == 2 ? "split-f16" : halves_of(d) == 1 ? "f16" : "f32";
     const char* rec = kind == 2 ? "geometric records" : kind == 1 ? "factored records" : "dense rows";
     if (kind != 0 && forward_ring_fits(d)) {
         const RingPlan p = plan_ring(d->O, 2 * d->B + 1, d->I, halves_of(d));
-        snprintf(buf, n, "fc_forward_ring_kernel<%s,%s> (ring-major, 2 workgroups x 8 wavefronts per CU, %zu B LDS, %d %s record chunks%s)",
-                 rec, mode, p.lds, p.nr, p.logh ? "half-size" : "1 KiB", p.alias ? ", partials aliased onto the slab" : "");
+        snprintf(buf, n, "fc_forward_ring_kernel<%s,%s> (ring-major, 2 workgroups x 8 wavefronts per CU, %zu B LDS, %d %s record chunks%s%s)",
+                 rec, mode, p.lds, p.nr, p.logh ? "half-size" : "1 KiB", p.alias ? ", partials aliased onto the slab" : "",
+                 unit_rows_apply(d, kind) ? ", 16-byte (x, u) rows from the workspace" : "");
     } else {
         snprintf(buf, n, "%s<%s,%s> (frequency-major, 16 wavefronts per CU, parts=%d)", kind ? "fc_forward_factored_kernel" : "fc_forward_kernel",
                  rec, mode, 1 << forward_parts_log2(d, kind));
@@ -33,18 +53,40 @@
     return (size_t)g.MP + (size_t)R * halves * g.MP * g.KP;
 }
 
-template <int R, int B, bool GEO, int LOGH>
+template <int R, int B, bool GEO, int LOGH, bool XU = false>
 static int launch_forward_ring(const float2* x, const float* rec, const fc_csr* g, const float* wpk, float2* y, const RingArgs& a,
                                size_t lds, int grid, hipStream_t stream) {
-    auto kern = fc_forward_ring_kernel<R, B, GEO, LOGH>;
+    auto kern = fc_forward_ring_kernel<R, B, GEO, LOGH, XU>;
     static bool lds_ok[kMaxDevices] = {};
     if (!allow_full_lds(reinterpret_cast<const void*>(kern), lds, lds_ok)) return FC_ERR_LAUNCH;
     hipLaunchKernelGGL(kern, dim3(grid), dim3(kDuoThreads), lds, stream, x, rec, g->rowptr, g->runs, wpk, y, a);
     return hipGetLastError() == hipSuccess ? FC_OK : FC_ERR_LAUNCH;
 }
 
+template <int R, int B>
+static int launch_ring_shape(bool geo, bool logh, const float2* x, const float2* xu, const float* rec, const fc_csr* g, const float* wpk,
+                             float2* y, const RingArgs& a, size_t lds, int grid, hipStream_t stream) {
+    if (logh && B < 2) return FC_ERR_UNSUPPORTED;
+    if (geo && xu) {
+        if constexpr (B >= 2 && ring_xu_compiled(R, B, true, 1)) {
+            if (logh) return launch_forward_ring<R, B, true, 1, true>(xu, rec, g, wpk, y, a, lds, grid, stream);
+        }
+        if constexpr (ring_xu_compiled(R, B, true, 0)) {
+            if (!logh) return launch_forward_ring<R, B, true, 0, true>(xu, rec, g, wpk, y, a, lds, grid, stream);
+        }
+        return FC_ERR_UNSUPPORTED;
+    }
+    if constexpr (B >= 2) {
+        if (logh)
+            return geo ? launch_forward_ring<R, B, true, 1>(x, rec, g, wpk, y, a, lds, grid, stream)
+                       : launch_forward_ring<R, B, false, 1>(x, rec, g, wpk, y, a, lds, grid, stream);
+    }
+    return geo ? launch_forward_ring<R, B, true, 0>(x, rec, g, wpk, y, a, lds, grid, stream)
+               : launch_forward_ring<R, B, false, 0>(x, rec, g, wpk, y, a, lds, grid, stream);
+}
+
 int forward_ring_impl(const float* x, const float* rec, const fc_csr* g, const float* wpk, float* y, const fc_dims* d, int kind,
-                      void* ws, size_t ws_bytes, const fc_epilogue* epi, hipStream_t stream) {
+                      void* ws, size_t ws_bytes, const fc_epilogue* epi, hipStream_t stream, bool unit_rows_ready) {
     const int F = 2 * d->B + 1;
     const RingPlan p = plan_ring(d->O, F, d->I, halves_of(d));
     if (!p.ok) return FC_ERR_UNSUPPORTED;
@@ -83,19 +125,17 @@
         grid = 2 * cus;
     }
     int rc = FC_ERR_UNSUPPORTED;
+    const UnitRows rows = forward_unit_rows(x, d, kind, ws, ws_bytes);
+    if (rows.xu && !unit_rows_ready) {
+        rc = unit_rows_impl(rows, stream);
+        if (rc != FC_OK) return rc;
+        rc = FC_ERR_UNSUPPORTED;
+    }
+    const float2* xu2 = static_cast<const float2*>(rows.xu);
     const float2* x2 = reinterpret_cast<const float2*>(x);
     float2* y2 = reinterpret_cast<float2*>(a.parts_log2 ? static_cast<float*>(ws) : y);
-#define FC_CASE(RR, BB)                                                                                            \
-    if (d->R == RR && d->B == BB) {                                                                                \
-        if constexpr (BB >= 2) {                                                                                   \
-            if (p.logh)                                                                                            \
-                rc = kind == 2 ? launch_forward_ring<RR, BB, true, 1>(x2, rec, g, wpk, y2, a, p.lds, grid, stream)  \
-                               : launch_forward_ring<RR, BB, false, 1>(x2, rec, g, wpk, y2, a, p.lds, grid, stream); \
-        }                                                                                                          \
-        if (!p.logh)                                                                                               \
-            rc = kind == 2 ? launch_forward_ring<RR, BB, true, 0>(x2, rec, g, wpk, y2, a, p.lds, grid, stream)      \
-                           : launch_forward_ring<RR, BB, false, 0>(x2, rec, g, wpk, y2, a, p.lds, grid, stream);    \
-    }
+#define FC_CASE(RR, BB) \
+    if (d->R == RR && d->B == BB) rc = launch_ring_shape<RR, BB>(kind == 2, p.logh != 0, x2, xu2, rec, g, wpk, y2, a, p.lds, grid, stream);
     FC_FOR_EACH_SHAPE(FC_CASE)
 #undef FC_CASE
     if (rc != FC_OK || a.parts_log2 == 0) return rc;
diff --git a/fieldconv_amd/csrc/fc_forward_ring.hpp b/fieldconv_amd/csrc/fc_forward_ring.hpp
--- a/fieldconv_amd/csrc/fc_forward_ring.hpp
+++ b/fieldconv_amd/csrc/fc_forward_ring.hpp
@@ -1,5 +1,6 @@
 #pragma once
 #include <stdlib.h>
+#include <type_traits>
 #include "fc_common.hpp"
 #include "fc_kernels.hpp"
 #include "fc_tile.hpp"
@@ -67,7 +68,25 @@
     return l;
 }
 
-template <int R, int B, bool GEO, int LOGH = 0>
+constexpr int kUnitRowsThreads = 256;
+__device__ __forceinline__ void unit_rows_body(const float2* __restrict__ x, f32x4* __restrict__ xu, const size_t count, const size_t idx) {
+    if (idx >= count) return;
+    const float2 v = x[idx];
+    const f32x2 u = unit_phase_pk(f32x2{v.x, v.y});
+    xu[idx] = f32x4{v.x, v.y, u.x, u.y};
+}
+__global__ __launch_bounds__(kUnitRowsThreads) static void fc_unit_rows_kernel(const float2* __restrict__ x, f32x4* __restrict__ xu, const size_t count) {
+    unit_rows_body(x, xu, count, (size_t)blockIdx.x * kUnitRowsThreads + threadIdx.x);
+}
+inline unsigned unit_rows_blocks(size_t count) { return (unsigned)((count + kUnitRowsThreads - 1) / kUnitRowsThreads); }
+__host__ __device__ constexpr bool ring_xu_compiled(int R, int B, bool geo, int logh) {
+    if (!geo || B > 2) return false;
+    if (B == 2 && R == 3) return false;
+    if (B == 2 && logh == 1 && (R == 4 || R == 5 || R == 8)) return false;
+    return true;
+}
+
+template <int R, int B, bool GEO, int LOGH = 0, bool XU = false>
 __global__ __launch_bounds__(kDuoThreads, 4) void fc_forward_ring_kernel(
     const float2* __restrict__ gx_, const float* __restrict__ grec, const int32_t* __restrict__ growptr,
     const int32_t* __restrict__ gruns, const float* __restrict__ gwpk, float2* __restrict__ gy_, const RingArgs a) {
@@ -77,6 +96,12 @@
     constexpr int CR = 1 << LOG_CR;
     constexpr int CHUNK = 256 >> LOGH;
     static_assert(LOG_CR >= 2, "a record chunk holds at least four records");
+    static_assert(GEO || !XU, "row entries with their unit phase: geometric records only");
+    using row_t = std::conditional_t<XU, f32x4, float2>;
+    auto fetch_row = [&](const int n, const uint32_t lane_ch) {
+        if constexpr (XU) return gather_row16(gx_, n, 16u * a.I, 16u * lane_ch);
+        else return gather_row(gx_, n, 8u * a.I, 8u * lane_ch);
+    };
     extern __shared__ __attribute__((aligned(16))) char smem[];
     const MmaGeom& g = a.g;
     const RingLds l = ring_lds(smem, g, a.alias_part != 0);
@@ -141,15 +166,15 @@
         if constexpr (CR * RECF == CHUNK) return ring + ((s * RECF) & (nr * CHUNK - 1));
         else return ring + ((s >> LOG_CR) & (nr - 1)) * CHUNK + (s & (CR - 1)) * RECF;
     };
-    auto first_rows = [&](const int j, const int nslots, float2& r0, float2& r1) {
-        r0 = make_float2(0.f, 0.f);
+    auto first_rows = [&](const int j, const int nslots, row_t& r0, row_t& r1) {
+        r0 = row_t{};
         r1 = r0;
         if (nslots > 0) {
             const float* ring = ring_of(j);
             const int n0 = __float_as_int(ring[3]);
             const int n1 = __float_as_int(ring[min(1, nslots - 1) * RECF + 3]);
-            r0 = gather_row(gx_, n0, 8u * I, 8u * cl);
-            r1 = gather_row(gx_, n1, 8u * I, 8u * cl);
+            r0 = fetch_row(n0, cl);
+            r1 = fetch_row(n1, cl);
         }
     };
 
@@ -163,7 +188,7 @@
     meter.begin();
     asm volatile("s_waitcnt vmcnt(0)" ::: "memory");
     meter.end(4);
-    float2 px[2][2];
+    row_t px[2][2];
 #pragma unroll
     for (int j = 0; j < 2; ++j) first_rows(j, end[j] - beg[j], px[j][0], px[j][1]);
 
@@ -263,14 +288,14 @@
         for (int j = 0; j < 2; ++j)
 #pragma unroll
             for (int f = 0; f < F; ++f) { clo[j][f] = f32x2{0.f, 0.f}; chi[j][f] = clo[j][f]; }
-        float2 xq[2][2] = {{px[0][0], px[0][1]}, {px[1][0], px[1][1]}};
+        row_t xq[2][2] = {{px[0][0], px[0][1]}, {px[1][0], px[1][1]}};
 
         constexpr bool kLookaheadProven = CR - 2 >= 3;
-        auto gather_run = [&](const int j, int s, const int run_end, f32x2 (&lo)[F], f32x2 (&hi)[F], float2& xe, float2& xo) {
+        auto gather_run = [&](const int j, int s, const int run_end, f32x2 (&lo)[F], f32x2 (&hi)[F], row_t& xe, row_t& xo) {
             const float* const ring = ring_of(j);
             const int nslots = end[j] - beg[j];
             const int nch = (nslots + CR - 1) >> LOG_CR;
-            auto slot = [&](const int s_, float2& xcur) {
+            auto slot = [&](const int s_, row_t& xcur) {
                 const float* rp = rec_ptr(ring, s_);
                 const f32x4 head = *reinterpret_cast<const f32x4*>(rp);
                 const int n2 = __float_as_int(rec_ptr(ring, min(s_ + 2, nslots - 1))[3]);
@@ -278,12 +303,13 @@
                 f32x2 z[F];
                 if constexpr (GEO) {
                     const f32x4 cg = *reinterpret_cast<const f32x4*>(rp + 4);
-                    rotate_geometric<B>(f32x2{xcur.x, xcur.y}, f32x2{cg.x, cg.y}, f32x2{cg.z, cg.w}, z);
-                    xcur = gather_row(gx_, n2, 8u * I, 8u * cl);
+                    if constexpr (XU) rotate_geometric<B>(f32x2{xcur.x, xcur.y}, f32x2{xcur.z, xcur.w}, f32x2{cg.x, cg.y}, f32x2{cg.z, cg.w}, z);
+                    else rotate_geometric<B>(f32x2{xcur.x, xcur.y}, f32x2{cg.x, cg.y}, f32x2{cg.z, cg.w}, z);
+                    xcur = fetch_row(n2, cl);
                 } else {
                     f32x2 xt[F], ph[F];
                     rotate_all<B>(f32x2{xcur.x, xcur.y}, xt);
-                    xcur = gather_row(gx_, n2, 8u * I, 8u * cl);
+                    xcur = fetch_row(n2, cl);
 #pragma unroll
                     for (int f = 0; f < F; ++f) {
                         ph[f] = *reinterpret_cast<const f32x2*>(rp + 4 + 2 * f);
@@ -382,7 +408,11 @@
         }
         contract(R - 1);
         if (a.alias_part) __syncthreads();
-        if (mma_active) store_partial(l.part, g, mt, kp, lane, tot_re, tot_im);
+        if (mma_active) {
+            int ln = lane;
+            asm volatile("" : "+v"(ln));
+            store_partial(l.part, g, mt, kp, ln, tot_re, tot_im);
+        }
         tot_re = f32x4{0.f, 0.f, 0.f, 0.f};
         tot_im = tot_re;
         stamp(5);
diff --git a/fieldconv_amd/csrc/fc_kernels.hpp b/fieldconv_amd/csrc/fc_kernels.hpp
--- a/fieldconv_amd/csrc/fc_kernels.hpp
+++ b/fieldconv_amd/csrc/fc_kernels.hpp
@@ -25,8 +25,20 @@
 constexpr int kMaxChannels = 64;
 
 int forward_impl(const float* x, const float* sten, const fc_csr* g, const float* wpk, float* y,
-                 const fc_dims* d, int kind, void* ws, size_t ws_bytes, const fc_epilogue* epi, hipStream_t stream);
+                 const fc_dims* d, int kind, void* ws, size_t ws_bytes, const fc_epilogue* epi, hipStream_t stream,
+                 bool unit_rows_ready = false);
 size_t forward_workspace_bytes(const fc_dims* d, int kind);
+size_t forward_workspace_bytes_any(const fc_dims* d);
+
+struct UnitRows {
+    const float* x;
+    void* xu;
+    size_t count;
+};
+inline size_t unit_rows_offset(size_t parts_bytes) { return (parts_bytes + 255) & ~(size_t)255; }
+UnitRows forward_unit_rows(const float* x, const fc_dims* d, int kind, void* ws, size_t ws_bytes);
+size_t unit_rows_bytes(const fc_dims* d, int kind);
+int unit_rows_impl(const UnitRows& r, hipStream_t stream);
 size_t backward_workspace_bytes(const fc_dims* d);
 int backward_data_impl(const float* x, const float* gy, const float* sten, const fc_csr* g, const float* wpk, float* gx,
                        void* ws, size_t ws_bytes, const fc_dims* d, bool factored, hipStream_t stream, bool defer_gx_sum = false);
@@ -37,7 +49,7 @@
 int backward_finish_impl(float* gw_eff, void* ws, size_t ws_bytes, const fc_dims* d, hipStream_t stream, bool factored = false);
 int pack_filter_impl(const float* w_eff, float* wpk_fwd, float* wpk_bwd, const fc_dims* d, int records, hipStream_t stream);
 int pack_filter_params_impl(const float* zonal, const float* sph, const float* phase, int ftype, float* wpk_fwd,
-                            float* wpk_bwd, const fc_dims* d, int records, hipStream_t stream);
+                            float* wpk_bwd, const fc_dims* d, int records, hipStream_t stream, const UnitRows* rider = nullptr);
 int pack_filter_params_pair_impl(const fc_filter_params& f0, float* fwd0, float* bwd0, const fc_dims* d0, const fc_filter_params& f1,
                                  float* fwd1, float* bwd1, const fc_dims* d1, int records, hipStream_t stream);
 size_t packed_filter_floats_fwd(const fc_dims* d, int records);
@@ -47,7 +59,7 @@
 bool forward_ring_fits(const fc_dims* d);
 size_t packed_ring_image_floats(int M, int F, int channels, int R, int halves);
 int forward_ring_impl(const float* x, const float* rec, const fc_csr* g, const float* wpk, float* y, const fc_dims* d, int kind,
-                      void* ws, size_t ws_bytes, const fc_epilogue* epi, hipStream_t stream);
+                      void* ws, size_t ws_bytes, const fc_epilogue* epi, hipStream_t stream, bool unit_rows_ready = false);
 int filter_param_grads_impl(const float* gw_eff, const float* zonal, const float* sph, const float* phase, int ftype,
                             float* g_zonal, float* g_sph, float* g_phase, const fc_dims* d, hipStream_t stream);
 
diff --git a/fieldconv_amd/csrc/fc_pack.hip b/fieldconv_amd/csrc/fc_pack.hip
--- a/fieldconv_amd/csrc/fc_pack.hip
+++ b/fieldconv_amd/csrc/fc_pack.hip
@@ -37,7 +37,12 @@
     unsigned blocks_f;
     int ring_f;
     int o0, i0, Ifull;
+    unsigned rows_block0;
+    const float2* rows_x;
+    f32x4* rows_xu;
+    size_t rows_count;
 };
+static_assert(kUnitRowsThreads == 256, "the rider's workgroups are the packing kernel's");
 
 constexpr int kPackThreads = 256;
 
@@ -152,6 +157,10 @@
                                                                       const float* __restrict__ sph,
                                                                       const float* __restrict__ phase, float* __restrict__ fwd,
                                                                       float* __restrict__ bwd, const PackArgs a) {
+    if (blockIdx.x >= a.rows_block0) {
+        unit_rows_body(a.rows_x, a.rows_xu, a.rows_count, (size_t)(blockIdx.x - a.rows_block0) * kPackThreads + threadIdx.x);
+        return;
+    }
     pack_filter_body<FROM_PARAMS>(w, zonal, sph, phase, fwd, bwd, a, blockIdx.x);
 }
 
@@ -185,6 +194,7 @@
     a.gb = make_mma_geom(d->I, d->R, d->O, halves_of(d));
     a.blocks_f = want_fwd ? pack_blocks(a.gf, a.ring_f ? a.R : a.F) : 0u;
     const unsigned blocks_b = pack_blocks(a.gb, a.F);
+    a.rows_block0 = ~0u; a.rows_x = nullptr; a.rows_xu = nullptr; a.rows_count = 0;
     return a.blocks_f + (want_bwd ? blocks_b : 0u);
 }
 
@@ -201,10 +211,18 @@
 
 template <bool FROM_PARAMS>
 static int launch_pack(const float* w_eff, const float* zonal, const float* sph, const float* phase, int ftype, float* wpk_fwd,
-                       float* wpk_bwd, const fc_dims* d, int records, hipStream_t stream, int o0 = 0, int i0 = 0, int Ifull = 0) {
+                       float* wpk_bwd, const fc_dims* d, int records, hipStream_t stream, int o0 = 0, int i0 = 0, int Ifull = 0,
+                       const UnitRows* rider = nullptr) {
     PackArgs a;
-    const unsigned blocks = pack_args(a, ftype, wpk_fwd != nullptr, wpk_bwd != nullptr, d, records, o0, i0, Ifull);
+    unsigned blocks = pack_args(a, ftype, wpk_fwd != nullptr, wpk_bwd != nullptr, d, records, o0, i0, Ifull);
     if (blocks == 0) return FC_ERR_BAD_ARGUMENT;
+    if (rider && rider->xu && rider->count) {
+        a.rows_block0 = blocks;
+        a.rows_x = reinterpret_cast<const float2*>(rider->x);
+        a.rows_xu = static_cast<f32x4*>(rider->xu);
+        a.rows_count = rider->count;
+        blocks += unit_rows_blocks(rider->count);
+    }
     hipLaunchKernelGGL(fc_pack_filter_kernel<FROM_PARAMS>, dim3(blocks), dim3(kPackThreads), 0, stream,
                        reinterpret_cast<const float2*>(w_eff), zonal, sph, phase, wpk_fwd, wpk_bwd, a);
     return hipGetLastError() == hipSuccess ? FC_OK : FC_ERR_LAUNCH;
@@ -215,8 +233,8 @@
 }
 
 int pack_filter_params_impl(const float* zonal, const float* sph, const float* phase, int ftype, float* wpk_fwd,
-                            float* wpk_bwd, const fc_dims* d, int records, hipStream_t stream) {
-    return launch_pack<true>(nullptr, zonal, sph, phase, ftype, wpk_fwd, wpk_bwd, d, records, stream);
+                            float* wpk_bwd, const fc_dims* d, int records, hipStream_t stream, const UnitRows* rider) {
+    return launch_pack<true>(nullptr, zonal, sph, phase, ftype, wpk_fwd, wpk_bwd, d, records, stream, 0, 0, 0, rider);
 }
 
 int pack_filter_params_block_impl(const float* zonal, const float* sph, const float* phase, int ftype, float* wpk_fwd, float* wpk_bwd,
diff --git a/fieldconv_amd/csrc/fc_wide.hip b/fieldconv_amd/csrc/fc_wide.hip
--- a/fieldconv_amd/csrc/fc_wide.hip
+++ b/fieldconv_amd/csrc/fc_wide.hip
@@ -29,7 +29,7 @@
     const size_t wf = packed_filter_floats_fwd(&p.db, records), wb = packed_filter_floats_bwd(&p.db, records);
     p.wpk = align256((wf > wb ? wf : wb) * sizeof(float));
     p.gw_block = align256((size_t)blk * blk * d->R * (2 * d->B + 1) * 8);
-    const size_t fws = records ? forward_workspace_bytes(&p.db, 1) : 0, bws = backward_workspace_bytes(&p.db);
+    const size_t fws = records ? forward_workspace_bytes_any(&p.db) : 0, bws = backward_workspace_bytes(&p.db);
     p.conv_ws = align256(fws > bws ? fws : bws);
     p.total_fwd = p.x_blocks + p.y_block + p.wpk + align256(fws);
     p.total_bwd = p.x_blocks + p.gy_blocks + p.gx_parts + p.gx_block + p.wpk + p.gw_block + align256(bws);
diff --git a/fieldconv_amd/functional.py b/fieldconv_amd/functional.py
--- a/fieldconv_amd/functional.py
+++ b/fieldconv_amd/functional.py
@@ -239,6 +239,8 @@
     plan.ws_fwd = 0
     if graph.factored and _edge_split():
         plan.ws_fwd = lib.fc_forward_workspace_bytes(plan.dref)
+        if graph.n_targets == graph.N == plan.dims.N:
+            plan.ws_fwd = lib.fc_forward_rows_workspace_bytes(plan.dref)
     plan.csr_t = _csr(graph.rowptr_t, graph.nbr_t, graph.runs_t)
     plan.csr_s = _csr(graph.rowptr_s, graph.nbr_s, graph.runs_s)
     plan.cref_t, plan.cref_s = ctypes.byref(plan.csr_t), ctypes.byref(plan.csr_s)
diff --git a/include/fieldconv_hip.h b/include/fieldconv_hip.h
--- a/include/fieldconv_hip.h
+++ b/include/fieldconv_hip.h
@@ -62,6 +62,7 @@
 
 int fc_factored_record_floats(int32_t band_limit);
 size_t fc_forward_workspace_bytes(const fc_dims* dims);
+size_t fc_forward_rows_workspace_bytes(const fc_dims* dims);
 int fc_forward_factored(const float* x, const float* rec_t, const fc_csr* by_target, const float* wpk_fwd,
                         float* y, void* workspace, size_t workspace_bytes, const fc_dims* dims, const fc_epilogue* epilogue,
                         void* stream);
```
